# philres/ngmlr

Hardware: AMD Instinct MI355X
Metric: aligned Gbp/hour (PacBio 10kb synthetic, convex-gap SW hot path, host buffers in -> results out, CIGAR bit-exact) (higher is better)
Workload: dtype f32

## Files before the change

include/cvx_align.h:

```cpp
#ifndef CVX_ALIGN_H
#define CVX_ALIGN_H

#include <stdint.h>
#include <stddef.h>

#ifdef __cplusplus
extern "C" {
#endif

#define CVX_ABI_VERSION 9

enum {
	CVX_OK = 0,
	CVX_ERR_NO_DEVICE = -1,
	CVX_ERR_PARAMS = -2,
	CVX_ERR_ARG = -3,
	CVX_ERR_OOM = -4,
	CVX_ERR_HIP = -5,
	CVX_ERR_CAPACITY = -6
};

enum {
	CVX_TILE_OK = 0,
	CVX_TILE_INVALID_ROW0 = 1,
	CVX_TILE_INVALID_EDGE = 2,
	CVX_TILE_INVALID_LENGTH = 3,
	CVX_TILE_TOO_LARGE = 4,
	CVX_TILE_EMPTY = 5,
	CVX_TILE_UNSUPPORTED = -1
};

enum { CVX_OP_I = 1, CVX_OP_D = 2, CVX_OP_EQ = 7, CVX_OP_X = 8 };

typedef struct {
	float match;
	float mismatch;
	float gap_open;
	float gap_extend;
	float gap_extend_min;
	float gap_decay;
} cvx_params;

enum { CVX_CORRIDOR_ROWS = 0, CVX_CORRIDOR_AFFINE = 1, CVX_CORRIDOR_CONST = 2 };

typedef struct {
	const char *ref;
	const char *qry;
	const int32_t *row_offset;
	const int32_t *row_length;
	int32_t ref_len;
	int32_t qry_len;
	int32_t row_stride_bytes;
	int32_t corridor_kind;
	float corridor_k;
	float corridor_d;
	float corridor_right;
	int32_t corridor_offset;
	int32_t corridor_width;
	int32_t reserved;
} cvx_tile;

int cvx_corridor_fit(const int32_t *row_offset, const int32_t *row_length, int32_t row_stride_bytes, int32_t n_rows,
		int32_t ref_len, int32_t qry_len, cvx_tile *form);
int cvx_corridor_fit_batch(int32_t n_tiles, cvx_tile *tiles, int32_t n_threads, int32_t *n_fitted);

typedef struct {
	float score;
	int32_t status;
	int32_t best_ref_index;
	int32_t best_read_index;
	int32_t ref_position;
	int32_t qstart;
	int32_t qend;
	int32_t n_ops;
	uint64_t ops_begin;
	uint64_t cells;
} cvx_result;

typedef struct cvx_context *cvx_handle;
typedef struct cvx_batch_s *cvx_batch;
typedef struct cvx_batch_s *cvx_job;

typedef struct {
	float plan_ms;
	float fill_ms;
	float backtrack_ms;
	float total_ms;
	uint64_t cells;
	uint64_t active_cells;
	uint64_t dir_bytes;
	int32_t n_fill_launches;
	int32_t n_tiles_fast;
	int32_t n_tiles_redone;
	int32_t n_tiles_chained;
	uint64_t chain_task_ticks, chain_poll_ticks;
} cvx_timing;

enum { CVX_LAUNCH_WHOLE = 0, CVX_LAUNCH_GANG = 1, CVX_LAUNCH_CHAINED = 2, CVX_LAUNCH_CATCH_ALL = 3 };
typedef struct {
	int32_t slots_per_lane;
	int32_t waves;
	int32_t wrap16;
	int32_t n_tiles;
	float ms;
	int32_t kind;
	uint64_t cells;
	uint64_t active_cells;
	uint64_t alg_bytes;
	uint64_t read_bases;
} cvx_launch_info;

const char *cvx_last_error(void);
int cvx_abi_version(void);
int cvx_device_count(void);
const char *cvx_build_id(void);
const char *cvx_source_id(const char *family);
int cvx_device_synchronize(int device_id);

int cvx_create(int device_id, const cvx_params *params, uint64_t max_matrix_mb, cvx_handle *out);
enum { CVX_CREATE_SERVICE = 1, CVX_CREATE_SCALAR_TWIN = 2 };
typedef struct {
	int32_t hw_queues_env, hw_queues_set_by_library;
	int32_t blocking_sync, blocking_sync_why;
	int32_t service_streams;
	int32_t runtime_up_at_load;
	int32_t reserved[2];
} cvx_regime;
int cvx_runtime_regime(int device_id, cvx_regime *out);
int cvx_create_ex(int device_id, const cvx_params *params, uint64_t max_matrix_mb, uint32_t flags, cvx_handle *out);
void cvx_destroy(cvx_handle h);

int cvx_align_batch(cvx_handle h, int32_t n_tiles, const cvx_tile *tiles, cvx_result *results,
		uint32_t *ops_arena, uint64_t ops_capacity, uint64_t *ops_used);

int cvx_batch_upload(cvx_handle h, int32_t n_tiles, const cvx_tile *tiles, cvx_batch *out);
int cvx_batch_run(cvx_handle h, cvx_batch b);
int cvx_batch_timing(cvx_batch b, cvx_timing *t);
int cvx_batch_ops_total(cvx_batch b, uint64_t *n_ops);
int cvx_batch_launch_info(cvx_batch b, int32_t i, cvx_launch_info *info);
int cvx_batch_download(cvx_handle h, cvx_batch b, cvx_result *results,
		uint32_t *ops_arena, uint64_t ops_capacity, uint64_t *ops_used);
void cvx_batch_free(cvx_handle h, cvx_batch b);

int cvx_submit(cvx_handle h, int32_t n_tiles, const cvx_tile *tiles, cvx_job *out);
int cvx_wait(cvx_handle h, cvx_job job, const cvx_result **results, const uint32_t **ops, uint64_t *n_ops);
int cvx_job_poll(cvx_handle h, cvx_job job, int32_t *done);
int cvx_job_timing(cvx_job job, cvx_timing *t);
int cvx_job_launch_info(cvx_job job, int32_t i, cvx_launch_info *info);
void cvx_job_release(cvx_handle h, cvx_job job);

int cvx_host_alloc(uint64_t bytes, void **out);
void cvx_host_free(void *p);

int cvx_corridor_rows(cvx_handle h, const cvx_tile *tile, int32_t *offset, int32_t *length);

int cvx_pack_probe(int32_t n_tiles, const cvx_tile *tiles, int32_t iters, int32_t assume_page_locked, double *ms_per_iter, uint64_t *bytes_touched);

typedef struct cvx_genome_s *cvx_genome;
uint64_t cvx_genome_encoded_bytes(int32_t n, const uint64_t *lengths);
int cvx_genome_encode(int32_t n, const char *const *seqs, const uint64_t *lengths, uint8_t *bin_ref,
		uint64_t *n_nibbles, uint64_t *start_table, int32_t *n_starts);
int cvx_genome_upload(cvx_handle h, const uint8_t *bin_ref, uint64_t n_nibbles, const uint64_t *start_table,
		int32_t n_starts, cvx_genome *out);
void cvx_genome_free(cvx_handle h, cvx_genome g);
int cvx_genome_decode(cvx_handle h, cvx_genome g, int32_t n, const uint64_t *position, const int32_t *length,
		const uint64_t *out_offset, char *out);
int cvx_submit_windows(cvx_handle h, cvx_genome g, int32_t n_tiles, const cvx_tile *tiles,
		const uint64_t *ref_position, cvx_job *out);
int cvx_job_window_refs(cvx_handle h, cvx_job job, const char **refs);

typedef struct cvx_index_s *cvx_index;
typedef struct {
	uint64_t location;
	float score;
	int32_t reverse;
} cvx_candidate;
int cvx_index_upload(cvx_handle h, int32_t kmer_len, const void *ref_table_index, const uint32_t *ref_table, uint32_t n_locations,
		uint64_t unit_offset, cvx_index *out);
void cvx_index_free(cvx_handle h, cvx_index ix);
int cvx_index_build(const uint8_t *bin_ref, uint64_t n_nibbles, const uint64_t *start_table, const uint64_t *seq_lengths, int32_t n_seqs,
		int32_t kmer_len, int32_t ref_skip, int32_t bin_shift, void *ref_table_index, uint32_t *ref_table, uint64_t ref_table_capacity,
		uint64_t *n_locations);
#define CVX_INDEX_KEEP_RESIDENT 1u
int cvx_index_build_device(int32_t device_id, const uint8_t *bin_ref, uint64_t n_nibbles, const uint64_t *start_table, const uint64_t *seq_lengths,
		int32_t n_seqs, int32_t kmer_len, int32_t ref_skip, int32_t bin_shift, void *ref_table_index, uint32_t *ref_table,
		uint64_t ref_table_capacity, uint64_t *n_locations, uint32_t flags);
int cvx_search_batch(cvx_handle h, cvx_index ix, int32_t n, const char *const *seqs, const int32_t *lens,
		float sensitivity, float min_kmer_hits, int32_t bin_shift,
		int32_t *n_candidates, uint64_t *cand_begin, cvx_candidate *cands, uint64_t cand_capacity, uint64_t *cand_used);
int cvx_search_batch_ex(cvx_handle h, cvx_index ix, int32_t n, const char *const *seqs, const int32_t *lens,
		float sensitivity, float min_kmer_hits, int32_t bin_shift, int32_t first_bits,
		int32_t *n_candidates, uint64_t *cand_begin, cvx_candidate *cands, uint64_t cand_capacity, uint64_t *cand_used,
		float *max_hit, int32_t *kmer_misses);
int cvx_search_batch_arena(cvx_handle h, cvx_index ix, int32_t n, const uint8_t *arena, const uint64_t *offsets,
		float sensitivity, float min_kmer_hits, int32_t bin_shift, int32_t first_bits,
		int32_t *n_candidates, uint64_t *cand_begin, cvx_candidate *cands, uint64_t cand_capacity, uint64_t *cand_used,
		float *max_hit, int32_t *kmer_misses);

int cvx_search_last_attempts(cvx_handle h, int32_t n, int32_t *attempts);

int cvx_score_batch(cvx_handle h, int32_t n, const char *const *refs, const char *const *qrys, float *scores);
int cvx_score_kernel_ms(cvx_handle h, float *ms);
enum { CVX_STAGE_SCORE = 0, CVX_STAGE_DECODE = 1, CVX_STAGE_SEARCH = 2,
	CVX_STAGE_SCORE_WINDOWS = 3  };
int cvx_stage_kernel_ms(cvx_handle h, int32_t stage, float *ms);

typedef struct cvx_score_job_s *cvx_score_job;
int cvx_score_submit(cvx_handle h, int32_t n, const char *const *refs, const char *const *qrys, cvx_score_job *job);
int cvx_score_poll(cvx_score_job job);
int cvx_score_wait(cvx_score_job job, float *scores);

typedef struct { uint64_t position; int32_t buffer_len; int32_t read; int32_t reverse; } cvx_score_window;
int cvx_score_windows_submit(cvx_handle h, cvx_genome g, int32_t n_reads, const uint8_t *arena, const uint64_t *offsets,
		int32_t n, const cvx_score_window *pairs, cvx_score_job *job);
int cvx_score_windows(cvx_handle h, cvx_genome g, int32_t n_reads, const uint8_t *arena, const uint64_t *offsets,
		int32_t n, const cvx_score_window *pairs, float *scores, int32_t *status );
int cvx_stage_windows(cvx_handle h, cvx_genome g, int32_t n_reads, const uint8_t *arena, const uint64_t *offsets,
		int32_t n, const cvx_score_window *pairs, uint8_t *out, uint64_t cap, uint64_t *ref_off, uint64_t *qry_off,
		int32_t *status, uint64_t *used);
int cvx_stage_windows_host(const uint8_t *bin_ref, uint64_t n_nibbles, const uint64_t *start_table, int32_t n_starts,
		int32_t n_reads, const uint8_t *arena, const uint64_t *offsets, int32_t n, const cvx_score_window *pairs,
		uint8_t *out, uint64_t cap, uint64_t *ref_off, uint64_t *qry_off, int32_t *status, uint64_t *used);
int cvx_genome_concat_len(uint64_t n_nibbles, const uint64_t *start_table, int32_t n_starts, uint64_t *concat_len);

typedef struct {
	int32_t ret;
	float score;
	int32_t position_offset;
	int32_t qstart, qend;
	int32_t nm;
	float identity;
	int32_t alignment_length;
	int32_t cigar_op_count;
	int32_t sv_type;
	int32_t first_ref, first_read, last_ref, last_read;
	int32_t nm_count;
	int32_t cigar_len, md_len;
} cvx_alignment_text;

enum { CVX_FORMAT_SCALAR_TWIN = 1 };
enum { CVX_NOT_WRITTEN = -1 };
int cvx_format_alignment_ex(const cvx_result *r, const uint32_t *ops_arena,
		const char *ref, int32_t ref_len, int32_t qry_len,
		int32_t ext_qstart, int32_t ext_qend,
		char *cigar, int32_t cigar_cap, char *md, int32_t md_cap,
		int32_t *nm_triples, int32_t nm_cap, uint32_t flags, cvx_alignment_text *out);
int cvx_format_alignment(const cvx_result *r, const uint32_t *ops_arena,
		const char *ref, int32_t ref_len, int32_t qry_len,
		int32_t ext_qstart, int32_t ext_qend,
		char *cigar, int32_t cigar_cap, char *md, int32_t md_cap,
		int32_t *nm_triples, int32_t nm_cap, cvx_alignment_text *out);

typedef struct {
	char *cigar;
	char *md;
	int32_t *nm_triples;
	int32_t cigar_cap, md_cap, nm_cap;
	int32_t ext_qstart, ext_qend;
} cvx_text_buffers;

int cvx_format_batch(int32_t n, const cvx_result *results, const uint32_t *ops_arena,
		const cvx_tile *tiles, const cvx_text_buffers *bufs, cvx_alignment_text *out,
		int32_t n_threads);
int cvx_format_batch_ex(int32_t n, const cvx_result *results, const uint32_t *ops_arena,
		const cvx_tile *tiles, const cvx_text_buffers *bufs, cvx_alignment_text *out,
		int32_t n_threads, uint32_t flags);

int cvx_job_text(cvx_handle h, cvx_job job, const int32_t *ext_qstart, const int32_t *ext_qend,
		cvx_alignment_text *out, uint64_t *text_off, const char **text, uint64_t *text_bytes);

int cvx_job_nm_profile(cvx_handle h, cvx_job job, int32_t first, int32_t count, uint64_t *entry_off,
		int32_t *triples, uint64_t cap_entries, double *kernel_ms);
int cvx_job_nm_profile_resident(cvx_handle h, cvx_job job, int32_t first, int32_t count, uint64_t *entry_off,
		const int32_t **triples, double *kernel_ms);
int cvx_job_text_all(cvx_handle h, cvx_job job, const int32_t *ext_qstart, const int32_t *ext_qend,
		cvx_alignment_text *out, uint64_t *text_off, const char **text, uint64_t *text_bytes,
		uint64_t *nm_entry_off, const int32_t **triples);
int cvx_job_nm_sizes(cvx_handle h, cvx_job job, int32_t first, int32_t count, uint64_t *entry_off);

int cvx_nm_profile_ops(cvx_handle h, int32_t n, const cvx_result *results, const uint32_t *ops_arena, uint64_t ops_total,
		uint64_t *entry_off, int32_t *triples, uint64_t cap_entries);

typedef struct {
	int32_t ref_start, ref_stop;
	int32_t read_start, read_stop;
} cvx_nm_region;
typedef struct {
	int32_t open, distance;
	cvx_nm_region r;
} cvx_nm_open;

int cvx_job_nm_regions(cvx_handle h, cvx_job job, int32_t first, int32_t count, uint64_t *region_off,
		const cvx_nm_region **regions, cvx_nm_open *open, double *kernel_ms);
int cvx_nm_regions_ops(cvx_handle h, int32_t n, const cvx_result *results, const uint32_t *ops_arena, uint64_t ops_total,
		uint64_t *region_off, cvx_nm_region *regions, uint64_t cap_regions, cvx_nm_open *open);
int cvx_nm_regions_host(const int32_t *triples, int64_t n_entries, int64_t scan_len, cvx_nm_region *regions, int64_t cap,
		int64_t *n_regions, cvx_nm_open *open);

typedef struct {
	const char *ref_name;
	int32_t ref_name_len;
	uint32_t location;
	int32_t reverse;
	const char *cigar;
	int32_t mq, nm;
} cvx_sam_other;

typedef struct {
	const char *read_name;
	const char *seq;
	char *qual;
	int32_t read_length;
	int32_t flags;
	int32_t primary;
	int32_t reverse;
	const char *ref_name;
	int32_t ref_name_len;
	uint32_t location;
	int32_t mq;
	const char *cigar;
	const char *md;
	int32_t cigar_op_count;
	const char *mate_ref_name;
	int32_t mate_location;
	int32_t template_length;
	float score;
	int32_t nm;
	float identity;
	int32_t qstart, qend;
	int32_t sv_type;
	int32_t n_others;
	const cvx_sam_other *others;
	const char *rg_id;
	int32_t hard_clip;
	int32_t bam_cigar_fix;
	int32_t skip;
} cvx_sam_record;

typedef struct {
	const char *read_name, *seq;
	const char *qual;
	int32_t read_length, flags;
	const char *ref_name;
	int32_t ref_name_len;
	int32_t location;
	char mate_ref;
	int32_t mate_location, template_length;
	const char *rg_id;
} cvx_sam_unmapped;

int cvx_sam_record_text(cvx_sam_record *r, char *out, uint64_t cap, uint64_t *len);
int cvx_sam_unmapped_text(const cvx_sam_unmapped *r, char *out, uint64_t cap, uint64_t *len);

int cvx_sam_batch(int32_t n, cvx_sam_record *recs, char *out, uint64_t cap, uint64_t *offsets);

#ifdef __cplusplus
}
#endif
#endif
```

ngmlr_amd/capi.py:

```python
from __future__ import annotations

import ctypes as C
import os

HERE = os.path.dirname(os.path.abspath(__file__))
LIB_PATH = os.environ.get("CVX_LIB") or os.path.join(HERE, "libcvxalign.so")

CVX_OK = 0
CREATE_SERVICE, CREATE_SCALAR_TWIN = 1, 2
FORMAT_SCALAR_TWIN = 1
NOT_WRITTEN = -1
STAGE_SCORE, STAGE_DECODE, STAGE_SEARCH, STAGE_SCORE_WINDOWS = 0, 1, 2, 3
ERR_NAMES = {0: "CVX_OK", -1: "CVX_ERR_NO_DEVICE", -2: "CVX_ERR_PARAMS", -3: "CVX_ERR_ARG",
             -4: "CVX_ERR_OOM", -5: "CVX_ERR_HIP", -6: "CVX_ERR_CAPACITY"}
TILE_STATUS = {0: "ok", 1: "invalid-row0", 2: "invalid-edge", 3: "invalid-length", 4: "too-large",
               5: "empty", -1: "unsupported"}

EXPORTS = ("cvx_last_error", "cvx_abi_version", "cvx_source_id", "cvx_device_count", "cvx_device_synchronize", "cvx_create", "cvx_destroy",
           "cvx_align_batch", "cvx_batch_upload", "cvx_batch_run", "cvx_batch_timing",
           "cvx_batch_ops_total", "cvx_batch_launch_info", "cvx_batch_download", "cvx_batch_free",
           "cvx_submit", "cvx_wait", "cvx_job_timing", "cvx_job_launch_info", "cvx_job_release",
           "cvx_format_alignment", "cvx_format_batch", "cvx_score_batch",
           "cvx_genome_encoded_bytes", "cvx_genome_encode", "cvx_genome_upload", "cvx_genome_free",
           "cvx_genome_decode", "cvx_submit_windows", "cvx_job_text",
           "cvx_host_alloc", "cvx_host_free", "cvx_corridor_rows", "cvx_pack_probe", "cvx_build_id", "cvx_job_poll", "cvx_score_kernel_ms",
           "cvx_index_upload", "cvx_index_free", "cvx_search_batch", "cvx_search_batch_ex", "cvx_job_nm_profile", "cvx_job_nm_profile_resident", "cvx_job_text_all", "cvx_job_window_refs", "cvx_job_nm_sizes", "cvx_nm_profile_ops",
           "cvx_job_nm_regions", "cvx_nm_regions_ops", "cvx_nm_regions_host",
           "cvx_sam_record_text", "cvx_sam_unmapped_text", "cvx_sam_batch", "cvx_stage_kernel_ms", "cvx_search_last_attempts", "cvx_index_build", "cvx_index_build_device",
           "cvx_corridor_fit", "cvx_corridor_fit_batch", "cvx_create_ex", "cvx_runtime_regime", "cvx_search_batch_arena",
           "cvx_score_submit", "cvx_score_poll", "cvx_score_wait", "cvx_format_alignment_ex", "cvx_format_batch_ex",
           "cvx_score_windows_submit", "cvx_score_windows", "cvx_stage_windows", "cvx_stage_windows_host", "cvx_genome_concat_len")


class CvxParams(C.Structure):
    _fields_ = [("match", C.c_float), ("mismatch", C.c_float), ("gap_open", C.c_float),
                ("gap_extend", C.c_float), ("gap_extend_min", C.c_float), ("gap_decay", C.c_float)]


class CvxTile(C.Structure):
    _fields_ = [("ref", C.c_char_p), ("qry", C.c_char_p), ("row_offset", C.c_void_p),
                ("row_length", C.c_void_p), ("ref_len", C.c_int32), ("qry_len", C.c_int32),
                ("row_stride_bytes", C.c_int32), ("corridor_kind", C.c_int32),
                ("corridor_k", C.c_float), ("corridor_d", C.c_float), ("corridor_right", C.c_float),
                ("corridor_offset", C.c_int32), ("corridor_width", C.c_int32), ("reserved", C.c_int32)]


class CvxRegime(C.Structure):
    _fields_ = [("hw_queues_env", C.c_int32), ("hw_queues_set_by_library", C.c_int32), ("blocking_sync", C.c_int32),
                ("blocking_sync_why", C.c_int32), ("service_streams", C.c_int32), ("runtime_up_at_load", C.c_int32), ("reserved", C.c_int32 * 2)]


CORRIDOR_ROWS, CORRIDOR_AFFINE, CORRIDOR_CONST = 0, 1, 2
assert C.sizeof(CvxTile) == 72


class CvxResult(C.Structure):
    _fields_ = [("score", C.c_float), ("status", C.c_int32), ("best_ref_index", C.c_int32),
                ("best_read_index", C.c_int32), ("ref_position", C.c_int32), ("qstart", C.c_int32),
                ("qend", C.c_int32), ("n_ops", C.c_int32), ("ops_begin", C.c_uint64),
                ("cells", C.c_uint64)]


class CvxTiming(C.Structure):
    _fields_ = [("plan_ms", C.c_float), ("fill_ms", C.c_float), ("backtrack_ms", C.c_float),
                ("total_ms", C.c_float), ("cells", C.c_uint64), ("active_cells", C.c_uint64),
                ("dir_bytes", C.c_uint64), ("n_fill_launches", C.c_int32), ("n_tiles_fast", C.c_int32),
                ("n_tiles_redone", C.c_int32), ("n_tiles_chained", C.c_int32),
                ("chain_task_ticks", C.c_uint64), ("chain_poll_ticks", C.c_uint64)]


class CvxLaunchInfo(C.Structure):
    _fields_ = [("slots_per_lane", C.c_int32), ("waves", C.c_int32), ("wrap16", C.c_int32),
                ("n_tiles", C.c_int32), ("ms", C.c_float), ("kind", C.c_int32), ("cells", C.c_uint64),
                ("active_cells", C.c_uint64), ("alg_bytes", C.c_uint64), ("read_bases", C.c_uint64)]


class CvxAlignmentText(C.Structure):
    _fields_ = [("ret", C.c_int32), ("score", C.c_float), ("position_offset", C.c_int32),
                ("qstart", C.c_int32), ("qend", C.c_int32), ("nm", C.c_int32), ("identity", C.c_float),
                ("alignment_length", C.c_int32), ("cigar_op_count", C.c_int32), ("sv_type", C.c_int32),
                ("first_ref", C.c_int32), ("first_read", C.c_int32), ("last_ref", C.c_int32),
                ("last_read", C.c_int32), ("nm_count", C.c_int32), ("cigar_len", C.c_int32),
                ("md_len", C.c_int32)]


class CvxNmRegion(C.Structure):
    _fields_ = [("ref_start", C.c_int32), ("ref_stop", C.c_int32), ("read_start", C.c_int32), ("read_stop", C.c_int32)]


class CvxNmOpen(C.Structure):
    _fields_ = [("open", C.c_int32), ("distance", C.c_int32), ("r", CvxNmRegion)]


class CvxSamOther(C.Structure):
    _fields_ = [("ref_name", C.c_char_p), ("ref_name_len", C.c_int32), ("location", C.c_uint32), ("reverse", C.c_int32),
                ("cigar", C.c_char_p), ("mq", C.c_int32), ("nm", C.c_int32)]


class CvxSamRecord(C.Structure):
    _fields_ = [("read_name", C.c_char_p), ("seq", C.c_char_p), ("qual", C.c_void_p), ("read_length", C.c_int32),
                ("flags", C.c_int32), ("primary", C.c_int32), ("reverse", C.c_int32), ("ref_name", C.c_char_p),
                ("ref_name_len", C.c_int32), ("location", C.c_uint32), ("mq", C.c_int32), ("cigar", C.c_char_p),
                ("md", C.c_char_p), ("cigar_op_count", C.c_int32), ("mate_ref_name", C.c_char_p),
                ("mate_location", C.c_int32), ("template_length", C.c_int32), ("score", C.c_float), ("nm", C.c_int32),
                ("identity", C.c_float), ("qstart", C.c_int32), ("qend", C.c_int32), ("sv_type", C.c_int32),
                ("n_others", C.c_int32), ("others", C.POINTER(CvxSamOther)), ("rg_id", C.c_char_p),
                ("hard_clip", C.c_int32), ("bam_cigar_fix", C.c_int32), ("skip", C.c_int32)]


class CvxSamUnmapped(C.Structure):
    _fields_ = [("read_name", C.c_char_p), ("seq", C.c_char_p), ("qual", C.c_char_p), ("read_length", C.c_int32),
                ("flags", C.c_int32), ("ref_name", C.c_char_p), ("ref_name_len", C.c_int32), ("location", C.c_int32),
                ("mate_ref", C.c_char), ("mate_location", C.c_int32), ("template_length", C.c_int32), ("rg_id", C.c_char_p)]


class CvxTextBuffers(C.Structure):
    _fields_ = [("cigar", C.c_void_p), ("md", C.c_void_p), ("nm_triples", C.c_void_p),
                ("cigar_cap", C.c_int32), ("md_cap", C.c_int32), ("nm_cap", C.c_int32),
                ("ext_qstart", C.c_int32), ("ext_qend", C.c_int32)]


class CvxScoreWindow(C.Structure):
    _fields_ = [("position", C.c_uint64), ("buffer_len", C.c_int32), ("read", C.c_int32), ("reverse", C.c_int32)]


assert C.sizeof(CvxScoreWindow) == 24


class CvxError(RuntimeError):
    def __init__(self, code: int, msg: str):
        super().__init__("%s: %s" % (ERR_NAMES.get(code, str(code)), msg))
        self.code = code


_libs = {}


def load(path: str = None) -> C.CDLL:
    path = path or LIB_PATH
    if path in _libs:
        return _libs[path]
    if not os.path.exists(path):
        raise FileNotFoundError(
            "%s not built: run `python -c 'import __graft_entry__ as g; g.build()'` "
            "(the HIP path has no fallback)" % path)
    lib = C.CDLL(path)
    lib.cvx_last_error.restype = C.c_char_p
    lib.cvx_abi_version.restype = C.c_int
    lib.cvx_build_id.restype = C.c_char_p
    lib.cvx_source_id.restype = C.c_char_p
    lib.cvx_source_id.argtypes = [C.c_char_p]
    lib.cvx_device_count.restype = C.c_int
    lib.cvx_device_synchronize.argtypes = [C.c_int]
    lib.cvx_create.argtypes = [C.c_int, C.POINTER(CvxParams), C.c_uint64, C.POINTER(C.c_void_p)]
    lib.cvx_destroy.argtypes = [C.c_void_p]
    lib.cvx_destroy.restype = None
    lib.cvx_align_batch.argtypes = [C.c_void_p, C.c_int32, C.POINTER(CvxTile), C.POINTER(CvxResult),
                                    C.c_void_p, C.c_uint64, C.POINTER(C.c_uint64)]
    lib.cvx_batch_upload.argtypes = [C.c_void_p, C.c_int32, C.POINTER(CvxTile), C.POINTER(C.c_void_p)]
    lib.cvx_batch_run.argtypes = [C.c_void_p, C.c_void_p]
    lib.cvx_batch_timing.argtypes = [C.c_void_p, C.POINTER(CvxTiming)]
    lib.cvx_batch_launch_info.argtypes = [C.c_void_p, C.c_int32, C.POINTER(CvxLaunchInfo)]
    lib.cvx_batch_ops_total.argtypes = [C.c_void_p, C.POINTER(C.c_uint64)]
    lib.cvx_batch_download.argtypes = [C.c_void_p, C.c_void_p, C.POINTER(CvxResult), C.c_void_p,
                                       C.c_uint64, C.POINTER(C.c_uint64)]
    lib.cvx_batch_free.argtypes = [C.c_void_p, C.c_void_p]
    lib.cvx_batch_free.restype = None
    lib.cvx_submit.argtypes = [C.c_void_p, C.c_int32, C.POINTER(CvxTile), C.POINTER(C.c_void_p)]
    lib.cvx_wait.argtypes = [C.c_void_p, C.c_void_p, C.POINTER(C.POINTER(CvxResult)), C.POINTER(C.POINTER(C.c_uint32)),
                             C.POINTER(C.c_uint64)]
    lib.cvx_job_poll.argtypes = [C.c_void_p, C.c_void_p, C.POINTER(C.c_int32)]
    lib.cvx_job_timing.argtypes = [C.c_void_p, C.POINTER(CvxTiming)]
    lib.cvx_job_launch_info.argtypes = [C.c_void_p, C.c_int32, C.POINTER(CvxLaunchInfo)]
    lib.cvx_job_release.argtypes = [C.c_void_p, C.c_void_p]
    lib.cvx_job_release.restype = None
    lib.cvx_format_batch.argtypes = [C.c_int32, C.POINTER(CvxResult), C.c_void_p, C.POINTER(CvxTile),
                                     C.POINTER(CvxTextBuffers), C.POINTER(CvxAlignmentText), C.c_int32]
    lib.cvx_genome_encoded_bytes.restype = C.c_uint64
    lib.cvx_genome_encoded_bytes.argtypes = [C.c_int32, C.c_void_p]
    lib.cvx_genome_encode.argtypes = [C.c_int32, C.POINTER(C.c_char_p), C.c_void_p, C.c_void_p, C.POINTER(C.c_uint64),
                                      C.c_void_p, C.POINTER(C.c_int32)]
    lib.cvx_genome_upload.argtypes = [C.c_void_p, C.c_void_p, C.c_uint64, C.c_void_p, C.c_int32, C.POINTER(C.c_void_p)]
    lib.cvx_genome_free.argtypes = [C.c_void_p, C.c_void_p]
    lib.cvx_genome_free.restype = None
    lib.cvx_genome_decode.argtypes = [C.c_void_p, C.c_void_p, C.c_int32, C.c_void_p, C.c_void_p, C.c_void_p, C.c_void_p]
    lib.cvx_submit_windows.argtypes = [C.c_void_p, C.c_void_p, C.c_int32, C.POINTER(CvxTile), C.c_void_p, C.POINTER(C.c_void_p)]
    lib.cvx_job_text.argtypes = [C.c_void_p, C.c_void_p, C.c_void_p, C.c_void_p, C.POINTER(CvxAlignmentText), C.c_void_p,
                                 C.POINTER(C.c_char_p), C.POINTER(C.c_uint64)]
    lib.cvx_job_nm_profile.argtypes = [C.c_void_p, C.c_void_p, C.c_int32, C.c_int32, C.c_void_p, C.c_void_p, C.c_uint64, C.POINTER(C.c_double)]
    lib.cvx_job_nm_sizes.argtypes = [C.c_void_p, C.c_void_p, C.c_int32, C.c_int32, C.c_void_p]
    lib.cvx_job_nm_profile_resident.argtypes = [C.c_void_p, C.c_void_p, C.c_int32, C.c_int32, C.c_void_p, C.POINTER(C.c_void_p), C.POINTER(C.c_double)]
    lib.cvx_job_window_refs.argtypes = [C.c_void_p, C.c_void_p, C.c_void_p]
    lib.cvx_job_text_all.argtypes = [C.c_void_p, C.c_void_p, C.c_void_p, C.c_void_p, C.POINTER(CvxAlignmentText), C.c_void_p,
                                     C.POINTER(C.c_char_p), C.POINTER(C.c_uint64), C.c_void_p, C.POINTER(C.c_void_p)]
    lib.cvx_nm_profile_ops.argtypes = [C.c_void_p, C.c_int32, C.c_void_p, C.c_void_p, C.c_uint64, C.c_void_p, C.c_void_p, C.c_uint64]
    lib.cvx_job_nm_regions.argtypes = [C.c_void_p, C.c_void_p, C.c_int32, C.c_int32, C.c_void_p, C.POINTER(C.c_void_p), C.c_void_p, C.POINTER(C.c_double)]
    lib.cvx_nm_regions_ops.argtypes = [C.c_void_p, C.c_int32, C.c_void_p, C.c_void_p, C.c_uint64, C.c_void_p, C.c_void_p, C.c_uint64, C.c_void_p]
    lib.cvx_nm_regions_host.argtypes = [C.c_void_p, C.c_int64, C.c_int64, C.c_void_p, C.c_int64, C.POINTER(C.c_int64), C.c_void_p]
    lib.cvx_sam_record_text.argtypes = [C.POINTER(CvxSamRecord), C.c_void_p, C.c_uint64, C.POINTER(C.c_uint64)]
    lib.cvx_sam_unmapped_text.argtypes = [C.POINTER(CvxSamUnmapped), C.c_void_p, C.c_uint64, C.POINTER(C.c_uint64)]
    lib.cvx_sam_batch.argtypes = [C.c_int32, C.POINTER(CvxSamRecord), C.c_void_p, C.c_uint64, C.c_void_p]
    lib.cvx_host_alloc.argtypes = [C.c_uint64, C.POINTER(C.c_void_p)]
    lib.cvx_host_free.argtypes = [C.c_void_p]
    lib.cvx_host_free.restype = None
    lib.cvx_corridor_rows.argtypes = [C.c_void_p, C.POINTER(CvxTile), C.c_void_p, C.c_void_p]
    lib.cvx_pack_probe.argtypes = [C.c_int32, C.c_void_p, C.c_int32, C.c_int32, C.POINTER(C.c_double), C.POINTER(C.c_uint64)]
    lib.cvx_index_upload.argtypes = [C.c_void_p, C.c_int32, C.c_void_p, C.c_void_p, C.c_uint32, C.c_uint64, C.POINTER(C.c_void_p)]
    lib.cvx_index_free.argtypes = [C.c_void_p, C.c_void_p]
    lib.cvx_index_free.restype = None
    lib.cvx_search_batch.argtypes = [C.c_void_p, C.c_void_p, C.c_int32, C.POINTER(C.c_char_p), C.c_void_p, C.c_float, C.c_float, C.c_int32,
                                     C.c_void_p, C.c_void_p, C.c_void_p, C.c_uint64, C.POINTER(C.c_uint64)]
    lib.cvx_search_batch_ex.argtypes = [C.c_void_p, C.c_void_p, C.c_int32, C.POINTER(C.c_char_p), C.c_void_p, C.c_float, C.c_float, C.c_int32, C.c_int32,
                                        C.c_void_p, C.c_void_p, C.c_void_p, C.c_uint64, C.POINTER(C.c_uint64), C.c_void_p, C.c_void_p]
    lib.cvx_search_batch_arena.argtypes = [C.c_void_p, C.c_void_p, C.c_int32, C.c_void_p, C.c_void_p, C.c_float, C.c_float, C.c_int32, C.c_int32,
                                           C.c_void_p, C.c_void_p, C.c_void_p, C.c_uint64, C.POINTER(C.c_uint64), C.c_void_p, C.c_void_p]
    lib.cvx_score_kernel_ms.argtypes = [C.c_void_p, C.POINTER(C.c_float)]
    lib.cvx_stage_kernel_ms.argtypes = [C.c_void_p, C.c_int32, C.POINTER(C.c_float)]
    lib.cvx_search_last_attempts.argtypes = [C.c_void_p, C.c_int32, C.c_void_p]
    lib.cvx_index_build_device.argtypes = [C.c_int32, C.c_void_p, C.c_uint64, C.c_void_p, C.c_void_p, C.c_int32, C.c_int32, C.c_int32, C.c_int32,
                                           C.c_void_p, C.c_void_p, C.c_uint64, C.POINTER(C.c_uint64), C.c_uint32]
    lib.cvx_index_build.argtypes = [C.c_void_p, C.c_uint64, C.c_void_p, C.c_void_p, C.c_int32, C.c_int32, C.c_int32, C.c_int32,
                                    C.c_void_p, C.c_void_p, C.c_uint64, C.POINTER(C.c_uint64)]
    lib.cvx_runtime_regime.argtypes = [C.c_int, C.POINTER(CvxRegime)]
    lib.cvx_create_ex.argtypes = [C.c_int, C.POINTER(CvxParams), C.c_uint64, C.c_uint32, C.POINTER(C.c_void_p)]
    lib.cvx_corridor_fit_batch.argtypes = [C.c_int32, C.c_void_p, C.c_int32, C.POINTER(C.c_int32)]
    lib.cvx_corridor_fit.argtypes = [C.c_void_p, C.c_void_p, C.c_int32, C.c_int32, C.c_int32, C.c_int32, C.POINTER(CvxTile)]
    lib.cvx_score_batch.argtypes = [C.c_void_p, C.c_int32, C.POINTER(C.c_char_p), C.POINTER(C.c_char_p), C.c_void_p]
    lib.cvx_score_submit.argtypes = [C.c_void_p, C.c_int32, C.POINTER(C.c_char_p), C.POINTER(C.c_char_p), C.POINTER(C.c_void_p)]
    lib.cvx_score_poll.argtypes = [C.c_void_p]
    lib.cvx_score_wait.argtypes = [C.c_void_p, C.c_void_p]
    win_in = [C.c_int32, C.c_void_p, C.c_void_p, C.c_int32, C.c_void_p]
    win_out = [C.c_void_p, C.c_uint64, C.c_void_p, C.c_void_p, C.c_void_p, C.POINTER(C.c_uint64)]
    lib.cvx_score_windows_submit.argtypes = [C.c_void_p, C.c_void_p] + win_in + [C.POINTER(C.c_void_p)]
    lib.cvx_score_windows.argtypes = [C.c_void_p, C.c_void_p] + win_in + [C.c_void_p, C.c_void_p]
    lib.cvx_stage_windows.argtypes = [C.c_void_p, C.c_void_p] + win_in + win_out
    lib.cvx_stage_windows_host.argtypes = [C.c_void_p, C.c_uint64, C.c_void_p, C.c_int32] + win_in + win_out
    lib.cvx_genome_concat_len.argtypes = [C.c_uint64, C.c_void_p, C.c_int32, C.POINTER(C.c_uint64)]
    lib.cvx_format_alignment.argtypes = [C.POINTER(CvxResult), C.c_void_p, C.c_char_p, C.c_int32,
                                         C.c_int32, C.c_int32, C.c_int32, C.c_char_p, C.c_int32,
                                         C.c_char_p, C.c_int32, C.c_void_p, C.c_int32,
                                         C.POINTER(CvxAlignmentText)]
    lib.cvx_format_alignment_ex.argtypes = [C.POINTER(CvxResult), C.c_void_p, C.c_char_p, C.c_int32,
                                            C.c_int32, C.c_int32, C.c_int32, C.c_char_p, C.c_int32,
                                            C.c_char_p, C.c_int32, C.c_void_p, C.c_int32, C.c_uint32,
                                            C.POINTER(CvxAlignmentText)]
    lib.cvx_format_batch_ex.argtypes = [C.c_int32, C.POINTER(CvxResult), C.c_void_p, C.POINTER(CvxTile),
                                        C.POINTER(CvxTextBuffers), C.POINTER(CvxAlignmentText), C.c_int32, C.c_uint32]
    _libs[path] = lib
    return lib


def check(rc: int) -> None:
    if rc != CVX_OK:
        raise CvxError(rc, load().cvx_last_error().decode(errors="replace"))


def corridor_fit(row_offset, row_length, ref_len, qry_len, stride_bytes=4):
    import numpy as np
    lib = load()
    off = np.ascontiguousarray(row_offset, dtype=np.int32) if stride_bytes == 4 else row_offset
    ln = np.ascontiguousarray(row_length, dtype=np.int32) if stride_bytes == 4 else row_length
    n = len(off) if stride_bytes == 4 else qry_len
    form = CvxTile()
    rc = lib.cvx_corridor_fit(off.ctypes.data, ln.ctypes.data, stride_bytes, n, ref_len, qry_len, C.byref(form))
    if rc != CVX_OK:
        raise RuntimeError("cvx_corridor_fit: %s" % ERR_NAMES.get(rc, rc))
    return (form.corridor_kind, form.corridor_k, form.corridor_d, form.corridor_right, form.corridor_offset, form.corridor_width)
```

ngmlr_amd/csrc/cvx_fill_ring.inc:

```
template <int M, bool WRAP, int MODE, bool TAB = false, int G = 1>
__global__ void __launch_bounds__(64 * G) CVX_FILL_OCC(M, TAB && G == 1)
CVX_FILL_KERNEL(const FillArgs a) {
	constexpr bool TWIN = CVX_FILL_TWIN;
	constexpr int N = 64 * M * G;
	constexpr int NW = 64 * M;
	constexpr bool EXACT = (MODE != kFillTwoPhase);
	constexpr bool CHAIN = (MODE == kFillChain);
	constexpr bool GANG = G > 1;
	static_assert(!GANG || (!WRAP && !CHAIN), "gangs serve whole tiles with float runs");
	static_assert(!TAB || (!WRAP && MODE == kFillTwoPhase), "the penalty table serves the two-phase float-score instantiation only");
	typedef typename RunT<WRAP || TAB>::type run_t;
	const int tid = threadIdx.x;
	const int lane = GANG ? (tid & 63) : tid;
	const int wv = GANG ? __builtin_amdgcn_readfirstlane(tid >> 6) : 0;
	const float go = a.sp.go;
	const float gext = a.sp.ge, gem = a.sp.gem, decay = a.sp.decay;
	float vmat = a.sp.mat, vmis = a.sp.mis;
	asm volatile("" : "+v"(vmat), "+v"(vmis));

	__shared__ int4 s_rec[CHAIN ? 1 : M * G][64];
	__shared__ int s_besty[M][64 * G];
	__shared__ u64 s_gx[GANG ? G : 1][GANG ? kGangDepth : 1];
	__shared__ float s_gred[GANG ? G : 1][4];
	__shared__ int s_gfail[GANG ? G : 1];
	__shared__ BoundaryVal s_bnd[CHAIN ? kChainChunk : 1];
	__shared__ float s_pen[TAB ? kPenEntries : 1];

	int t;
	int task_id = 0, y0 = 0;
	u64 chain_t0 = 0ull, chain_polled = 0ull;
	ChainTask ct;
	if (CHAIN) {
		int tk = 0;
		if (lane == 0) tk = atomicAdd(a.chain_ticket, 1);
		task_id = __builtin_amdgcn_readfirstlane(tk);
		if (task_id >= a.list_n) return;
		ct = a.tasks[task_id];
		t = ct.tile;
		y0 = ct.y0;
		if (a.chain_prio) __builtin_amdgcn_s_setprio(3);
		chain_t0 = __builtin_amdgcn_s_memtime();
	} else {
		t = a.list[blockIdx.x];
		if (!GANG && a.chain_prio) { if (a.chain_prio >= 2) __builtin_amdgcn_s_setprio(2); else __builtin_amdgcn_s_setprio(1); }
#if CVX_FILL_PRIO
		if (blockIdx.x < (unsigned) (a.list_n >> 4)) __builtin_amdgcn_s_setprio(2);
#endif
		if (GANG && a.chain_prio) __builtin_amdgcn_s_setprio(2);
		if (MODE == kFillExact) {
			if (a.tout[t].pad != kPadRedo) return;
			if (tid == 0) atomicAdd(a.redo_count, 1);
		}
	}
	TileIn ti = a.tin[t];
	ti.ref_off = in_sgpr(ti.ref_off); ti.qry_off = in_sgpr(ti.qry_off); ti.W = in_sgpr(ti.W); ti.H = in_sgpr(ti.H);
	ti.row_off = in_sgpr((u64) ti.row_off);
	TileRun tr = a.trun[t];
	tr.dir_off = in_sgpr((u64) tr.dir_off); tr.r0 = in_sgpr(tr.r0); tr.nsteps = in_sgpr(tr.nsteps);
	RowView rv = row_view(a.rsrc[t], a.rows, ti.row_off, y0);
	rv.rows = in_sgpr(rv.rows); rv.fmt = in_sgpr(rv.fmt); rv.width = in_sgpr(rv.width);
	rv.k = in_sgpr(rv.k); rv.d = in_sgpr(rv.d); rv.right = in_sgpr(rv.right);
	const uint8_t *seq = a.seq;
	const int H = CHAIN ? ct.rows : ti.H, W = ti.W;
	const unsigned qry_off = ti.qry_off + (unsigned) y0;
	const int r0 = CHAIN ? ct.r0 : tr.r0;
	const int nsteps = CHAIN ? ct.nsteps : tr.nsteps;
	uint32_t *dirs = in_sgpr(a.dirs + (CHAIN ? ct.dir_off : tr.dir_off));
	float S[M];
	float Hc[M];
	float V[M];
	float dg[M];
	run_t drun[M];
	run_t irun[M];
	int cnt[M];
	int len[M];
	int qch[M];
	unsigned xa[M];
	unsigned cwn[M];
	float penp[M];
	constexpr bool LAZY = TAB && (CVX_FILL_TAB_LAZY != 0);
	float best[M];
	int best_r[M];
	float lbest = 0.0f;
	unsigned accA[M], accB[M];
	u64 mD[M];
	u64 mI[M];

	const unsigned ref_base = ti.ref_off - (unsigned) y0;
	auto make_rec = [&](const int yy) {
		int4 rec;
		rec.w = (int) (ref_base - (unsigned) yy);
		if (yy < H) {
			const RowDesc2 ol = row_at(rv, yy);
			const long long Ws = (long long) W;
			long long lo = ol.x > 0 ? ol.x : 0;
			long long hi = (long long) ol.x + (long long) ol.y;
			if (hi > Ws) hi = Ws;
			if (hi < lo) hi = lo;
			rec.x = yy + y0 + (int) lo;
			rec.y = (int) (hi - lo);
			rec.z = seq[qry_off + (unsigned) yy];
		} else {
			rec.x = yy + y0 + (1 << 30);
			rec.y = 0;
			rec.z = 0;
		}
		return rec;
	};
	auto take_row = [&](const int j, const int4 rec, const int rnext, const bool fetch_now) {
		cnt[j] = rnext - rec.x;
		len[j] = rec.y;
		qch[j] = rec.z;
		xa[j] = (unsigned) rec.w + (unsigned) rnext + 4u;
		if (fetch_now || cnt[j] > -4) cwn[j] = *reinterpret_cast<const unsigned *>(seq + (xa[j] - 4u));
	};
	constexpr int kStage = 16 * M;
	auto stage_rows = [&](const int Y, const int sY) {
		if (lane < kStage) {
			const int4 rec = make_rec(Y + lane);
			const int sl = sY + lane;
			s_rec[CHAIN ? 0 : wv * M + sl % M][sl / M] = rec;
		}
		__builtin_amdgcn_fence(__ATOMIC_ACQ_REL, "workgroup");
	};

	if (TAB) {
		for (int i = lane; i < kPenEntries; i += 64) s_pen[i] = fminf(gem, gext + (float) i * decay);
		__builtin_amdgcn_fence(__ATOMIC_ACQ_REL, "workgroup");
	}
#pragma unroll
	for (int j = 0; j < M; ++j) {
		s_besty[j][tid] = 0;
		S[j] = 0.0f; Hc[j] = go; V[j] = go; dg[j] = 0.0f;
		drun[j] = 0; irun[j] = 0;
		best[j] = 0.0f; best_r[j] = 0;
		penp[j] = gem;
		accA[j] = accB[j] = 0u;
		mD[j] = 0; mI[j] = 0;
		cwn[j] = 0u;
		take_row(j, make_rec(tid * M + j), r0, true);
	}
	int stage_next = N + wv * NW, stage_slot = 0;
	auto stage_advance = [&]() {
		stage_next += kStage;
		stage_slot += kStage;
		if (stage_slot >= NW) { stage_slot = 0; stage_next += N - NW; }
	};
	if (!CHAIN) {
		for (int c = 0; c < NW / kStage - 1; ++c) { stage_rows(stage_next, stage_slot); stage_advance(); }
	}

	int gang_failed = 0;
	if (GANG) {
		if (lane < kGangDepth) s_gx[wv][lane] = ~0ull;
		__syncthreads();
	}
	const int gang_pred = GANG ? (wv + G - 1) % G : 0;

	const int ngroups = (nsteps + 3) >> 2;
	int late = ngroups >> a.late_shift;
	if (late < a.late_min_groups) late = a.late_min_groups;
	const int gswitch = (EXACT || late >= ngroups) ? 0 : ngroups - late;
	int r = r0;

	const int out_slot = CHAIN ? (ct.rows - 1) : 0;
	const int out_lane = out_slot / M, out_j = out_slot % M;
	u64 *bnd_out = CHAIN ? reinterpret_cast<u64 *>(a.bnd + ct.bnd_out_off) : nullptr;
	u64 *bnd_in = CHAIN ? reinterpret_cast<u64 *>(a.bnd + ct.bnd_in_off) : nullptr;
	const unsigned epoch = a.bnd_epoch;
	int chain_failed = 0;
	BoundaryVal bcur;
	bcur.V = go; bcur.S = 0.0f; bcur.run = 0u; bcur.is_ins = 0u;
	u64 bpre = 0ull;

	auto group = [&](auto track_tag, const int g) {
		constexpr bool TRACK = decltype(track_tag)::value;
		if (CHAIN && (g & (kChainChunk / 4 - 1)) == 0) {
			const int x = (r - y0) + lane;
			const int idx = x - ct.bnd_lo;
			const bool mine = ct.prev >= 0 && lane < kChainChunk && idx >= 0 && idx < ct.bnd_len;
			u64 q = bpre;
			bool ok = !mine || (unsigned) (q >> 49) == epoch;
			int spins = 0;
			const bool must_poll = !chain_failed && ballot(!ok) != 0ull;
			const u64 poll_t0 = must_poll ? __builtin_amdgcn_s_memtime() : 0ull;
			while (!chain_failed && ballot(!ok) != 0ull) {
				if (!ok) {
					q = __hip_atomic_load(bnd_in + idx, __ATOMIC_RELAXED, __HIP_MEMORY_SCOPE_AGENT);
					ok = (unsigned) (q >> 49) == epoch;
				}
				if (ballot(!ok) == 0ull) break;
				if (++spins > (1 << 21)) { chain_failed = 1; break; }
				if (spins < 8) __builtin_amdgcn_s_sleep(2);
				else if (spins < 64) __builtin_amdgcn_s_sleep(32);
				else __builtin_amdgcn_s_sleep(127);
			}
			if (must_poll) chain_polled += __builtin_amdgcn_s_memtime() - poll_t0;
			BoundaryVal br;
			br.V = go; br.S = 0.0f; br.run = 0u; br.is_ins = 0u;
			if (mine && ok) {
				const unsigned meta = (unsigned) (q >> 32);
				const float sc = __uint_as_float((unsigned) q);
				const unsigned run16 = meta & 0xffffu;
				const bool ins = (meta >> 16) & 1u;
				const float runf = WRAP ? (float) (int) (short) run16 : (float) run16 - 1.0f;
				br.S = sc;
				br.run = WRAP ? (unsigned) (int) (short) run16 : __float_as_uint((float) run16);
				br.is_ins = ins ? 1u : 0u;
				br.V = ins ? gap_extend_value(sc, runf, gem, gext, decay) : sc + go;
			}
			if (lane < kChainChunk) s_bnd[lane] = br;
			__builtin_amdgcn_fence(__ATOMIC_ACQ_REL, "workgroup");
			bcur = s_bnd[0];
			const int idxn = idx + kChainChunk;
			bpre = 0ull;
			if (ct.prev >= 0 && lane < kChainChunk && idxn >= 0 && idxn < ct.bnd_len)
				bpre = __hip_atomic_load(bnd_in + idxn, __ATOMIC_RELAXED, __HIP_MEMORY_SCOPE_AGENT);
		}
		unsigned cw[M];
		const float misx = TWIN ? a.sp.misx : 0.0f;
#pragma unroll
		for (int j = 0; j < M; ++j) {
			cw[j] = cwn[j];
			cwn[j] = *reinterpret_cast<const unsigned *>(seq + xa[j]);
			xa[j] += 4u;
		}
		if (g != 0 && (g & 7) == 0) {
			uint32_t *d = dirs + (size_t) ((g >> 3) - 1) * (N * 2);
			const unsigned dl = (unsigned) tid * (M * 2);
#pragma unroll
			for (int j = 0; j < M; ++j) { d[dl + 2 * j] = accA[j]; d[dl + 2 * j + 1] = accB[j]; }
		}

#pragma unroll
		for (int i = 0; i < 4; ++i) {
			float p_E[M], p_O[M];
			auto offers = [&](const int j) {
				p_E[j] = fmaxf(S[j] + penp[j], S[j] * -0x1p100f);
				p_O[j] = S[j] + go;
			};
			if (LAZY) offers(M - 1);
			float uV0 = LAZY ? rot1_f(lanes(mI[M - 1]) ? p_E[M - 1] : p_O[M - 1]) : rot1_f(V[M - 1]);
			float uS0 = rot1_f(S[M - 1]);
			run_t uI0;
			if (WRAP || TAB) uI0 = (run_t) rot1_i((int) irun[M - 1]);
			else uI0 = (run_t) rot1_f((float) irun[M - 1]);
			u64 mIu0 = rot1_m(mI[M - 1]);
			u64 gq = 0ull;
			if (GANG && r != r0) gq = __hip_atomic_load(&s_gx[gang_pred][(r - r0 - 1) & (kGangDepth - 1)], __ATOMIC_RELAXED, __HIP_MEMORY_SCOPE_WORKGROUP);
			auto gang_take = [&]() {
				float sc = 0.0f, vv = go;
				unsigned run16 = 0u, ins = 0u;
				if (r != r0) {
					const unsigned want_tag = (unsigned) (r - r0 - 1) & 0x7fffu;
					int spins = 0;
					while (!gang_failed && (((unsigned) __builtin_amdgcn_readfirstlane((int) (gq >> 32))) >> 17) != want_tag) {
						if (++spins > (1 << 22)) { gang_failed = 1; break; }
#if CVX_GANG_SLEEP > 0
						__builtin_amdgcn_s_sleep(CVX_GANG_SLEEP);
#endif
						gq = __hip_atomic_load(&s_gx[gang_pred][(r - r0 - 1) & (kGangDepth - 1)], __ATOMIC_RELAXED, __HIP_MEMORY_SCOPE_WORKGROUP);
					}
					const unsigned meta = (unsigned) __builtin_amdgcn_readfirstlane((int) (gq >> 32));
					sc = __uint_as_float((unsigned) __builtin_amdgcn_readfirstlane((int) gq));
					run16 = meta & 0xffffu;
					ins = (meta >> 16) & 1u;
					vv = ins ? gap_extend_value(sc, (float) run16 - 1.0f, gem, gext, decay) : sc + go;
				}
				if (lane == 0) {
					uV0 = vv;
					uS0 = sc;
					uI0 = TAB ? (run_t) (int) (run16 << 2) : (run_t) (float) run16;
				}
				mIu0 = (mIu0 & ~1ull) | (u64) ins;
			};
			auto gang_give = [&]() {
				const unsigned run16 = TAB ? (((unsigned) (int) irun[M - 1]) >> 2) & 0xffffu : ((unsigned) (int) (float) irun[M - 1]) & 0xffffu;
				const unsigned meta = run16 | (unsigned) (((mI[M - 1] >> 63) & 1ull) << 16) | (((unsigned) (r - r0) & 0x7fffu) << 17);
				if (lane == 63)
					__hip_atomic_store(&s_gx[wv][(r - r0) & (kGangDepth - 1)], ((u64) meta << 32) | (u64) __float_as_uint(S[M - 1]), __ATOMIC_RELAXED, __HIP_MEMORY_SCOPE_WORKGROUP);
			};
			if (CHAIN) {
				const BoundaryVal br = bcur;
				bcur = s_bnd[((r - r0) + 1) & (kChainChunk - 1)];
				if (lane == 0) {
					uV0 = br.V;
					uS0 = br.S;
					uI0 = WRAP ? (run_t) (int) br.run : (run_t) __uint_as_float(br.run);
				}
				const int bit = __builtin_amdgcn_readfirstlane((int) br.is_ins);
				mIu0 = (mIu0 & ~1ull) | (u64) (bit & 1);
			}

			float p_lc[M], p_dc[M], p_uc[M], p_mx[M];
			u64 p_eL[M], p_eU[M], p_eG[M], p_act[M], p_isDl[M], p_isIu[M];
			u64 p_nD[M], p_nI[M], p_gap[M], p_cread[M];
			auto phase1 = [&](const int j, const float misx_) {
				float uV = (j > 0) ? V[j > 0 ? j - 1 : 0] : uV0;
				const run_t uI = (j > 0) ? irun[j > 0 ? j - 1 : 0] : uI0;
				const u64 mIu = (j > 0) ? mI[j > 0 ? j - 1 : 0] : mIu0;
				float lcv = Hc[j];
				if (LAZY) {
					if (j > 0) {
						offers(j > 0 ? j - 1 : 0);
						uV = lanes(mIu) ? p_E[j > 0 ? j - 1 : 0] : p_O[j > 0 ? j - 1 : 0];
					}
					lcv = lanes(mD[j]) ? p_E[j] : p_O[j];
				}
				const int refc = (int) ((cw[j] >> (8 * i)) & 0xffu);
				const bool eq = (refc == qch[j]);
				float mv = vmis;
				if (TWIN) mv = lanes(ballot(refc == 'x')) ? misx_ : vmis;
				const float diag_cell = dg[j] + (eq ? vmat : mv);
				float lc = lcv, dc = diag_cell, uc = uV;
				const float mx = fmaxf(fmaxf(fmaxf(lc, dc), uc), 0.0f);
				p_lc[j] = lc; p_dc[j] = dc; p_uc[j] = uc; p_mx[j] = mx;
				p_eL[j] = ballot(mx == lc);
				p_eU[j] = ballot(mx == uc);
				p_eG[j] = ballot(mx == dc);
				p_act[j] = ballot((unsigned) cnt[j] < (unsigned) len[j]);
				p_isDl[j] = WRAP ? ballot(drun[j] > 0) : mD[j];
				p_isIu[j] = WRAP ? ballot(uI > 0) : mIu;
			};
			auto phase2 = [&](const int j) {
				const u64 eL = p_eL[j], eU = p_eU[j], eG = p_eG[j], act = p_act[j], isDl = p_isDl[j], isIu = p_isIu[j];
				const u64 c2 = isIu & eU;
				const u64 nD = eL & (isDl | ~(c2 | eG)) & act;
				const u64 nI = ~nD & eU & (isIu | ~eG) & act;
				p_nD[j] = nD; p_nI[j] = nI;
				p_gap[j] = nD | nI;
				p_cread[j] = nI | (eG & ~nD);
			};
			auto phase3 = [&](const int j) {
				const float uS = (j > 0) ? S[j > 0 ? j - 1 : 0] : uS0;
				const run_t uI = (j > 0) ? irun[j > 0 ? j - 1 : 0] : uI0;
				const u64 nD = p_nD[j], nI = p_nI[j], isDl = p_isDl[j], isIu = p_isIu[j];
				const float mx = p_mx[j];
				const float sc = lanes(p_act[j]) ? mx : 0.0f;
				run_t nd, ni;
				float runf = 0.0f;
				float E;
				if (TAB) {
					const u64 extD = nD & isDl, extI = nI & isIu;
					const int t1 = lanes(extI) ? (int) uI : 4;
					const int ra = lanes(extD) ? (int) drun[j] : t1;
					nd = (run_t) (ra + 4);
					ni = nd;
					const float pen = *reinterpret_cast<const float *>(reinterpret_cast<const char *>(s_pen) + ra);
					if (LAZY) penp[j] = pen;
					E = fmaxf(sc + pen, sc * -0x1p100f);
				} else if (WRAP) {
					nd = lanes(nD) ? (lanes(isDl) ? (run_t) (short) ((int) drun[j] + 1) : (run_t) 1) : (run_t) 0;
					ni = lanes(nI) ? (lanes(isIu) ? (run_t) (short) ((int) uI + 1) : (run_t) 1) : (run_t) 0;
					runf = (float) (lanes(nD) ? nd : ni);
				} else {
					const u64 extD = nD & isDl, extI = nI & isIu;
					const float t1 = lanes(extI) ? (float) uI : 1.0f;
					runf = lanes(extD) ? (float) drun[j] : t1;
					nd = (run_t) (runf + 1.0f);
					ni = nd;
				}
				if (!TAB) E = gap_extend_value(sc, runf, gem, gext, decay);
				const float O = sc + go;

				dg[j] = uS;
				S[j] = sc;
				drun[j] = nd;
				irun[j] = ni;
				if (!LAZY) {
					V[j] = lanes(nI) ? E : O;
					Hc[j] = lanes(nD) ? E : O;
				}
				if (TRACK) {
					const u64 better = ballot(sc > best[j]);
					best[j] = lanes(better) ? mx : best[j];
					best_r[j] = lanes(better) ? r : best_r[j];
				} else if (i >= 2) {
					lbest = fmaxf(lbest, sc);
				}
				mD[j] = nD;
				mI[j] = nI;
				cnt[j] += 1;
				accA[j] = shl1_in(accA[j], p_gap[j]);
				accB[j] = shl1_in(accB[j], p_cread[j]);
			};
#if CVX_FILL_SCHED == 1
#pragma unroll
			for (int j = M - 1; j >= 0; --j) phase1(j, misx);
			__builtin_amdgcn_sched_barrier(0);
#pragma unroll
			for (int j = M - 1; j >= 0; --j) phase2(j);
			__builtin_amdgcn_sched_barrier(0);
#elif CVX_FILL_SCHED == 2
#pragma unroll
			for (int q = M; q >= -1; --q) {
				if (q < M && q >= 0) phase1(q, misx);
				if (q + 1 < M && q + 1 >= 0) phase2(q + 1);
				__builtin_amdgcn_sched_barrier(0);
			}
#endif
#pragma unroll
			for (int j = M - 1; j >= 0; --j) {
#if CVX_FILL_SCHED == 0 || CVX_FILL_SCHED == 3
				if (GANG && j == 0) gang_take();
				phase1(j, misx); phase2(j);
#endif
				phase3(j);
				if (GANG && j == M - 1) gang_give();
#if CVX_FILL_SCHED == 3
				__builtin_amdgcn_sched_barrier(0);
#endif
				if (CHAIN && j == out_j && ct.has_next) {
					if (lane == out_lane && (unsigned) (cnt[j] - 1) < (unsigned) len[j]) {
						const unsigned run16 = WRAP ? ((unsigned) (int) irun[j] & 0xffffu) : ((unsigned) (int) (float) irun[j] & 0xffffu);
						const unsigned meta = run16 | (unsigned) (((mI[j] >> out_lane) & 1ull) << 16) | (epoch << 17);
						__hip_atomic_store(bnd_out + (cnt[j] - 1), ((u64) meta << 32) | (u64) __float_as_uint(S[j]), __ATOMIC_RELAXED, __HIP_MEMORY_SCOPE_AGENT);
					}
				}
			}
			r += 1;
		}
		const bool stage_now = !CHAIN && (ballot(cnt[0] > len[0]) & 0x0001000100010001ull) != 0ull;
#pragma unroll
		for (int j = 0; j < M; ++j) {
			if (!CHAIN && cnt[j] > len[j]) {
				if (TRACK) {
					const int yy = (int) (ref_base - (xa[j] - (unsigned) r - 4u));
					if (best_r[j] >= r - cnt[j]) s_besty[j][tid] = yy;
				}
				take_row(j, s_rec[CHAIN ? 0 : wv * M + j][lane], r, false);
			}
		}
		if (TAB) {
#pragma unroll
			for (int j = 0; j < M; ++j) { const int c = min((int) drun[j], 4 * kPenClamp); drun[j] = (run_t) c; irun[j] = (run_t) c; }
		}
		if (stage_now) {
			stage_rows(stage_next, stage_slot);
			stage_advance();
		}
	};

	for (int g = 0; g < gswitch; ++g) group(BoolTag<false>(), g);
	for (int g = gswitch; g < ngroups; ++g) group(BoolTag<true>(), g);

	if (ngroups > 0) {
		const int done = ((ngroups - 1) & 7) + 1;
		const int sh = 32 - 4 * done;
		uint32_t *d = dirs + ((size_t) ((ngroups - 1) >> 3) * N + (size_t) tid * M) * 2;
#pragma unroll
		for (int j = 0; j < M; ++j) { d[2 * j] = sh ? accA[j] << sh : accA[j]; d[2 * j + 1] = sh ? accB[j] << sh : accB[j]; }
	}

	float b = -1.0f;
	int by = 0x7fffffff, bx = 0x7fffffff;
#pragma unroll
	for (int j = 0; j < M; ++j) {
		int vy = s_besty[j][tid];
		const int ycur = (int) (ref_base - (xa[j] - (unsigned) r - 4u));
		if (ycur < H && best_r[j] >= r - cnt[j]) vy = ycur;
		const float v = best[j];
		const int vx = best_r[j] - vy;
		if (v > 0.0f) {
			if (v > b || (v == b && (vy < by || (vy == by && vx < bx)))) { b = v; by = vy; bx = vx; }
		}
	}
	float be = lbest;
#pragma unroll
	for (int off = 32; off >= 1; off >>= 1) {
		const float ob = __shfl_xor(b, off, 64);
		const int oy = __shfl_xor(by, off, 64);
		const int ox = __shfl_xor(bx, off, 64);
		if (ob > b || (ob == b && (oy < by || (oy == by && ox < bx)))) { b = ob; by = oy; bx = ox; }
		if (!EXACT) be = fmaxf(be, __shfl_xor(be, off, 64));
	}
	if (CHAIN) {
		if (lane == 0) {
			ChainOut co;
			co.score = b;
			co.best_y = (b > -1.0f) ? by + y0 : 0;
			co.best_x = (b > -1.0f) ? bx - y0 : 0;
			co.failed = chain_failed;
			a.chain_out[ct.blk] = co;
			unsigned long long *ticks = reinterpret_cast<unsigned long long *>(a.redo_count + kCtrChainTicks);
			atomicAdd(ticks, (unsigned long long) (__builtin_amdgcn_s_memtime() - chain_t0));
			if (chain_polled) atomicAdd(ticks + 1, (unsigned long long) chain_polled);
		}
		return;
	}
	if (GANG) {
		if (lane == 0) {
			s_gred[wv][0] = b; s_gred[wv][1] = __int_as_float(by); s_gred[wv][2] = __int_as_float(bx);
			s_gred[wv][3] = EXACT ? 0.0f : be;
			s_gfail[wv] = gang_failed;
		}
		__syncthreads();
		if (wv != 0) return;
#pragma unroll
		for (int w = 1; w < G; ++w) {
			const float ob = s_gred[w][0];
			const int oy = __float_as_int(s_gred[w][1]), ox = __float_as_int(s_gred[w][2]);
			if (ob > b || (ob == b && (oy < by || (oy == by && ox < bx)))) { b = ob; by = oy; bx = ox; }
			if (!EXACT) be = fmaxf(be, s_gred[w][3]);
		}
	}
	if (lane == 0) {
		TileOut o;
		o.score = b;
		o.status = 0;
		o.best_x = (b > -1.0f) ? bx : 0;
		o.best_y = (b > -1.0f) ? by : 0;
		o.ref_position = 0; o.qstart = 0; o.qend = 0; o.n_ops = 0; o.ops_first = 0;
		o.pad = (!EXACT && gswitch > 0 && !(b > be + 2.0f * a.sp.mat + 1.0f)) ? kPadRedo : 0;
		if (GANG) {
			bool failed = gang_failed != 0;
			for (int w = 1; w < G; ++w) failed = failed || s_gfail[w] != 0;
			if (failed) { o.status = -1; o.pad = 0; }
		}
		a.tout[t] = o;
	}
}
```

ngmlr_amd/csrc/cvx_kernels.hip:

```cpp
#include <hip/hip_runtime.h>
#include <stdint.h>

#include "cvx_types.h"
#include "cvx_launch.h"

namespace cvx {

#define CVX_DEV __device__ __forceinline__

CVX_DEV int rot1_i(int v) {
	return __builtin_amdgcn_update_dpp(0, v, 0x13C, 0xf, 0xf, true);
}
CVX_DEV float rot1_f(float v) {
	return __int_as_float(rot1_i(__float_as_int(v)));
}


CVX_DEV void row_span(const int2 ol, int W, int y, int &gs, int &ge) {
	long long lo = ol.x > 0 ? ol.x : 0;
	long long hi = (long long) ol.x + (long long) ol.y;
	if (hi > W) hi = W;
	if (hi < lo) hi = lo;
	gs = (int) (lo + y);
	ge = (int) (hi + y);
}

template <int TPT>
__global__ void __launch_bounds__(256)
plan_kernel(const int2 *rows, const RowSrc *rsrc, const TileIn *tin, TilePlan *plan, int n_tiles, unsigned long long max_matrix_mb) {
	constexpr int TPB = 256 / TPT;
	const int sub = threadIdx.x / TPT;
	const int ltid = threadIdx.x % TPT;
	const int t = blockIdx.x * TPB + sub;
	const bool live = t < n_tiles;
	const TileIn ti = tin[live ? t : 0];
	const RowView rv = row_view(rsrc[live ? t : 0], reinterpret_cast<const RowDesc2 *>(rows), ti.row_off);
	auto row = [&](const int y) { const RowDesc2 q = row_at(rv, y); return make_int2(q.x, q.y); };
	const int H = live ? ti.H : 0, W = ti.W;

	__shared__ unsigned long long s_cells[TPB], s_active[TPB];
	__shared__ int s_need[TPB], s_flags[TPB], s_maxlen[TPB], s_rend[TPB], s_r0[TPB];
	if (ltid == 0) { s_cells[sub] = 0; s_active[sub] = 0; s_need[sub] = 1; s_flags[sub] = 0; s_maxlen[sub] = 0; s_rend[sub] = -0x7fffffff; s_r0[sub] = 0x7fffffff; }
	__syncthreads();

	unsigned long long cells = 0, active = 0;
	int need = 1, flags = 0, maxlen = 0, rendmax = -0x7fffffff, r0min = 0x7fffffff;
	for (int y = ltid; y < H; y += TPT) {
		const int2 ol = row(y);
		int gs, ge;
		row_span(ol, W, y, gs, ge);
		cells += (unsigned long long) (long long) ol.y;
		active += (unsigned long long) (ge - gs);
		if (ol.y > maxlen) maxlen = ol.y;
		if (ge > rendmax) rendmax = ge;
		if (gs < r0min) r0min = gs;
		if (y > 0) {
			int pgs, pge;
			row_span(row(y - 1), W, y - 1, pgs, pge);
			if (gs <= pgs) flags |= kPlanIrregular;
			if (ge < pge) flags |= kPlanIrregular;
		}
		const int lim = ge + kSwitchMargin;
		auto starts_before = [&](int yy) {
			int mgs, mge;
			row_span(row(yy), W, yy, mgs, mge);
			return mgs < lim;
		};
		int lo = y + 1, hi = H;
		int g = y + 1 + ((lim - gs) >> 1);
		g = g < lo ? lo : g;
		if (g < hi) {
			if (starts_before(g)) {
				lo = g + 1;
				for (int step = 1; lo < hi; step <<= 1) {
					const int p = (lo + step - 1 < hi) ? lo + step - 1 : hi - 1;
					if (starts_before(p)) lo = p + 1; else { hi = p; break; }
				}
			} else {
				hi = g;
				for (int step = 1; lo < hi; step <<= 1) {
					const int p = (hi - step > lo) ? hi - step : lo;
					if (starts_before(p)) { lo = p + 1; break; } else hi = p;
				}
			}
		}
		while (lo < hi) {
			const int mid = (lo + hi) >> 1;
			if (starts_before(mid)) lo = mid + 1; else hi = mid;
		}
		const int n = lo - y + 1;
		if (n > need) need = n;
		if (H > 32767) {
			long long lo_y = ol.x > 0 ? ol.x : 0;
			long long hi_y = (long long) ol.x + (long long) ol.y;
			if (hi_y > W) hi_y = W;
			if (hi_y < lo_y) hi_y = lo_y;
			int a = y + 1, b = H;
			while (a < b) {
				const int mid = (a + b) >> 1;
				const int2 om = row(mid);
				const long long lo_m = om.x > 0 ? om.x : 0;
				if (lo_m < hi_y) a = mid + 1; else b = mid;
			}
			if (a - y > maxlen) maxlen = a - y;
		}
	}
	if (H > 0) {
		atomicAdd(&s_cells[sub], cells);
		atomicAdd(&s_active[sub], active);
		atomicMax(&s_need[sub], need);
		atomicOr(&s_flags[sub], flags);
		atomicMax(&s_maxlen[sub], maxlen);
		atomicMax(&s_rend[sub], rendmax);
		atomicMin(&s_r0[sub], r0min);
	}
	__syncthreads();

	if (ltid == 0 && live) {
		TilePlan p;
		p.cells = s_cells[sub];
		p.active = s_active[sub];
		p.need = s_need[sub];
		int f = s_flags[sub];
		int r0 = 0, rend = 0;
		if (H > 0) { r0 = s_r0[sub]; rend = s_rend[sub]; }
		if (H <= 0 || s_active[sub] == 0) f |= kPlanEmpty;
		const float mb = (float) s_cells[sub] / 1000.0f / 1000.0f;
		if (!((unsigned long long) mb < max_matrix_mb)) f |= kPlanTooLarge;
		if (s_maxlen[sub] > 32767 || (H > 32767 && (f & kPlanIrregular))) f |= kPlanWrap16;
		p.r0 = r0;
		p.rend = rend;
		p.flags = f;
		plan[t] = p;
	}
}


__global__ void __launch_bounds__(64)
expand_rows_kernel(const RowSrc *rsrc, const TileIn *tin, const uint8_t *delta, const int2 *rowsx, int2 *rows, int n_tiles, int closed_forms) {
	const int t = blockIdx.x;
	if (t >= n_tiles) return;
	const int lane = threadIdx.x;
	const RowSrc rs = rsrc[t];
	const TileIn ti = tin[t];
	const int H = ti.H;
	int2 *out = rows + ti.row_off;
	if (rs.fmt == kRowsExplicit) {
		const int2 *src = rowsx + rs.src_off;
		for (int y = lane; y < H; y += 64) out[y] = src[y];
		return;
	}
	if ((rs.fmt == kRowsAffine || rs.fmt == kRowsConst) && !closed_forms) return;
	if (rs.fmt == kRowsAffine) {
		for (int y = lane; y < H; y += 64) out[y] = make_int2(affine_row_offset(y, rs.d, rs.k, rs.right), rs.width);
		return;
	}
	if (rs.fmt == kRowsConst) {
		for (int y = lane; y < H; y += 64) out[y] = make_int2(rs.off0, rs.width);
		return;
	}
	const int8_t *d = reinterpret_cast<const int8_t *>(delta + rs.src_off);
	int carry = rs.off0;
	for (int y0 = 0; y0 < H; y0 += 64) {
		const int y = y0 + lane;
		int v = (y < H && y > 0) ? (int) d[y] : 0;
#pragma unroll
		for (int k = 1; k < 64; k <<= 1) {
			const int u = __shfl_up(v, k, 64);
			if (lane >= k) v += u;
		}
		if (y < H) out[y] = make_int2(carry + v, rs.width);
		carry += __builtin_amdgcn_readlane(v, 63);
	}
}


typedef unsigned long long u64;

CVX_DEV u64 ballot(bool p) { return __builtin_amdgcn_ballot_w64(p); }
CVX_DEV int in_sgpr(int v) { v = __builtin_amdgcn_readfirstlane(v); asm volatile("" : "+s"(v)); return v; }
CVX_DEV float in_sgpr(float v) { return __int_as_float(in_sgpr(__float_as_int(v))); }
CVX_DEV unsigned in_sgpr(unsigned v) { return (unsigned) in_sgpr((int) v); }
CVX_DEV u64 in_sgpr(u64 u) { return ((u64) in_sgpr((unsigned) (u >> 32)) << 32) | (u64) in_sgpr((unsigned) u); }
template <typename T> CVX_DEV T *in_sgpr(T *p) {
	const u64 u = (u64) p;
	const unsigned lo = (unsigned) in_sgpr((int) (unsigned) u), hi = (unsigned) in_sgpr((int) (unsigned) (u >> 32));
	return (T *) (((u64) hi << 32) | (u64) lo);
}
CVX_DEV bool lanes(u64 m) { return __builtin_amdgcn_inverse_ballot_w64(m); }
CVX_DEV u64 rot1_m(u64 m) { return (m << 1) | (m >> 63); }
#ifndef CVX_FILL_ADDC_SGPR
#define CVX_FILL_ADDC_SGPR 1
#endif
CVX_DEV unsigned shl1_in(unsigned acc, u64 m) {
#if CVX_FILL_ADDC_SGPR
	u64 carry_out;
	asm volatile("v_addc_co_u32_e64 %0, %1, %0, %0, %2" : "+v"(acc), "=s"(carry_out) : "s"(m));
#else
	asm volatile("v_addc_co_u32_e64 %0, vcc, %0, %0, %1" : "+v"(acc) : "s"(m) : "vcc");
#endif
	return acc;
}


CVX_DEV void valid_bounds(const int off, const int width, int &minC, int &maxC) {
	minC = (int) ((float) off + 0.1f * (float) width);
	maxC = (int) ((float) (minC + width) - 0.1f * (float) width);
}

CVX_DEV unsigned plane_code(const unsigned wx, const unsigned wy, const int bit) {
	const unsigned px = (wx >> bit) & 1u, py = (wy >> bit) & 1u;
	return px ? (py ? 1u : 2u) : (py ? 3u : 0u);
}

template <bool CHAINED>
CVX_DEV void backtrack_walk(const int lane, const int H, const int N, const int r0, const int ops_cap,
		const RowView &rows, const uint2 *dirs, const ChainBlk *blk, const uint8_t *ref, const uint8_t *qry, int *ops, TileOut &o) {
	const int best_x = __builtin_amdgcn_readfirstlane(o.best_x);
	const int best_y = __builtin_amdgcn_readfirstlane(o.best_y);
	if (best_y <= 0) { o.status = 1; return; }

	const int qend = (H - best_y) - 1;
	int idx = ops_cap - 1;
	int elem = 4;
	int elem_len = qend;
	int consumed = qend;
	int x = best_x, y = best_y;
	int s = y % N;
	int status = 0;
	unsigned want = 3u;

	auto emit = [&](int cur, int n) {
		if (n <= 0) return;
		if (cur == elem) {
			elem_len += n;
		} else {
			if (elem != 4) { if (lane == 0) ops[idx] = (elem_len << 4) | elem; idx -= 1; }
			elem = cur;
			elem_len = n;
		}
	};

	int budget = 2 * (best_x + best_y) + 8;
	for (;;) {
		if (--budget < 0) { status = 3; break; }
		const int dx = (want != 1u) ? 1 : 0, dy = (want != 2u) ? 1 : 0;
		const int cx = x - lane * dx, cy = y - lane * dy;
		const bool inside = (cx >= 0 && cy >= 0);
		const int lx = cx > 0 ? cx : 0, ly = cy > 0 ? cy : 0;
		int sl = s - lane * dy;
		if (sl < 0) sl += N;
		const int tt = cx + cy - r0;
		const int ttc = tt > 0 ? tt : 0;
		const RowDesc2 ol = row_at(rows, ly);
		uint2 w;
		if (CHAINED) {
			const int gb = ly / N;
			const ChainBlk cb = blk[gb];
			int wr = (ttc >> 5) - cb.tblk0;
			wr = wr < 0 ? 0 : (wr >= cb.nblk32 ? cb.nblk32 - 1 : wr);
			w = dirs[cb.dir_off + (size_t) wr * N + (size_t) (ly - gb * N)];
		} else {
			w = dirs[(size_t) (ttc >> 5) * N + sl];
		}
		const int rc = ref[lx], qc = qry[ly];
		const u64 eqm = ballot(rc == qc);
		const bool in_row = inside && tt >= 0 && cx >= ol.x && cx < ol.x + ol.y;
		unsigned code = plane_code(w.x, w.y, 31 - (ttc & 31));
		if (!in_row) code = 0u;
		int minC, maxC;
		valid_bounds(ol.x, ol.y, minC, maxC);

		const u64 run = ballot(code == want);
		const int L = (~run == 0ull) ? 64 : __builtin_ctzll(~run);
		const u64 low = (L == 64) ? ~0ull : ((1ull << L) - 1ull);
		const u64 vp = ballot(cx > minC && cx < maxC);
		if ((~vp & low) != 0ull) { status = 2; break; }

		if (want == 3u) {
			int pos = 0;
			while (pos < L) {
				const int isq = (int) ((eqm >> pos) & 1ull);
				const u64 m = (isq ? ~eqm : eqm) >> pos;
				int rl = (m == 0ull) ? 64 - pos : __builtin_ctzll(m);
				if (rl > L - pos) rl = L - pos;
				emit(isq ? 7 : 8, rl);
				pos += rl;
			}
			x -= L; y -= L; consumed += L;
		} else if (want == 1u) {
			emit(1, L);
			y -= L; consumed += L;
		} else {
			emit(2, L);
			x -= L;
		}
		if (want != 2u) { s -= L; if (s < 0) s += N; }
		if (L == 64) continue;
		const unsigned nxt = (unsigned) __builtin_amdgcn_readlane((int) code, L);
		if (nxt == 0u) break;
		if (want != 3u) { want = nxt; continue; }

		const int tp = x + y - r0;
		if (nxt == 2u) {
			const unsigned wx = (unsigned) __builtin_amdgcn_readlane((int) w.x, L);
			const unsigned wy = (unsigned) __builtin_amdgcn_readlane((int) w.y, L);
			const int row_lo = max(__builtin_amdgcn_readlane(ol.x, L), 0);
			const int b0 = 31 - (tp & 31);
			const unsigned dm = (wx & ~wy) >> b0;
			int Ld = (~dm == 0u) ? 32 : __builtin_ctz(~dm);
			const int in_word = 32 - b0;
			const int in_rowc = x - row_lo + 1;
			if (Ld > in_rowc) Ld = in_rowc;
			const int rminC = __builtin_amdgcn_readlane(minC, L), rmaxC = __builtin_amdgcn_readlane(maxC, L);
			if (!(x - (Ld - 1) > rminC && x < rmaxC)) { status = 2; break; }
			emit(2, Ld);
			x -= Ld;
			if (Ld == in_rowc) break;
			if (Ld == in_word) { want = 2u; continue; }
			const unsigned c2 = plane_code(wx, wy, b0 + Ld);
			if (c2 == 0u) break;
			want = c2;
		} else {
			const int k = lane - L;
			const int tn = tp - k;
			const bool have = (k >= 0) && (cy >= 0) && (tn >= 0) && ((tn >> 5) == (ttc >> 5));
			const bool col_in = (x >= ol.x) && (x < ol.x + ol.y);
			unsigned c2 = plane_code(w.x, w.y, 31 - (tn & 31));
			if (!col_in) c2 = 0u;
			const u64 im = ballot(have && c2 == 1u) >> L;
			const int Li = (~im == 0ull) ? 64 : __builtin_ctzll(~im);
			const u64 ilow = (Li == 64) ? ~0ull : ((1ull << Li) - 1ull);
			const u64 vpi = ballot(x > minC && x < maxC) >> L;
			if ((~vpi & ilow) != 0ull) { status = 2; break; }
			emit(1, Li);
			y -= Li; consumed += Li;
			s -= Li; if (s < 0) s += N;
			const int e = L + Li;
			want = 1u;
			if (e < 64 && ((ballot(have) >> e) & 1ull) != 0ull) {
				const unsigned c3 = (unsigned) __builtin_amdgcn_readlane((int) c2, e);
				if (c3 == 0u) break;
				want = c3;
			}
		}
	}
	if (status == 0) {
		if (elem != 4) { if (lane == 0) ops[idx] = (elem_len << 4) | elem; idx -= 1; }
		consumed += (y + 1);
		o.ref_position = x + 1;
		o.qstart = y + 1;
		o.qend = qend;
		o.ops_first = idx + 1;
		o.n_ops = ops_cap - 1 - idx;
		if (H != consumed) status = 3;
	}
	o.status = status;
}

CVX_DEV void first_cell(const RowView &rows, int H, int W, int lane, int *fy, int *fx) {
	*fy = -1;
	*fx = 0;
	for (int y0 = 0; y0 < H; y0 += 64) {
		const int yy = y0 + lane;
		bool has = false;
		int lo_i = 0;
		if (yy < H) {
			const RowDesc2 ol = row_at(rows, yy);
			long long lo = ol.x > 0 ? ol.x : 0;
			long long hi = (long long) ol.x + (long long) ol.y;
			if (hi > W) hi = W;
			has = hi > lo;
			lo_i = (int) lo;
		}
		const unsigned long long m = __builtin_amdgcn_ballot_w64(has);
		if (m != 0ull) {
			const int l = __builtin_ctzll(m);
			*fy = y0 + l;
			*fx = __builtin_amdgcn_readlane(lo_i, l);
			return;
		}
	}
}


template <bool WRAP> struct RunT { typedef float type; };
template <> struct RunT<true> { typedef int type; };
template <bool B> struct BoolTag { static constexpr bool value = B; };

#ifndef CVX_FILL_WAVES_PER_EU
#define CVX_FILL_WAVES_PER_EU 6
#endif
#ifndef CVX_FILL_WAVES_M4
#define CVX_FILL_WAVES_M4 1
#endif
#ifndef CVX_FILL_WAVES_TAB
#define CVX_FILL_WAVES_TAB 7
#endif
#define CVX_FILL_OCC(M, SEVEN) __attribute__((amdgpu_waves_per_eu( \
		(M) == 3 ? ((SEVEN) ? CVX_FILL_WAVES_TAB : CVX_FILL_WAVES_PER_EU) : ((M) == 4 ? CVX_FILL_WAVES_M4 : 1), \
		(M) == 3 ? ((SEVEN) ? CVX_FILL_WAVES_TAB : CVX_FILL_WAVES_PER_EU) : ((M) == 4 && CVX_FILL_WAVES_M4 > 1 ? CVX_FILL_WAVES_M4 : 8))))

#ifndef CVX_FILL_TAB_LAZY
#define CVX_FILL_TAB_LAZY 1
#endif

#ifndef CVX_GANG_SLEEP
#define CVX_GANG_SLEEP 1
#endif

#ifndef CVX_FILL_SCHED
#define CVX_FILL_SCHED 0
#endif

#ifndef CVX_FILL_PRIO
#define CVX_FILL_PRIO 1
#endif

CVX_DEV float gap_extend_value(const float sc, const float runf, const float gem, const float gext, const float decay) {
	const float pen = fminf(gem, gext + runf * decay);
	return fmaxf(sc + pen, sc * -0x1p100f);
}

enum FillMode { kFillTwoPhase = 0, kFillExact = 1, kFillChain = 2 };

#define CVX_FILL_KERNEL fill_ring_kernel
#define CVX_FILL_TWIN false
#include "cvx_fill_ring.inc"
#undef CVX_FILL_KERNEL
#undef CVX_FILL_TWIN
#define CVX_FILL_KERNEL fill_ring_twin_kernel
#define CVX_FILL_TWIN true
#include "cvx_fill_ring.inc"
#undef CVX_FILL_KERNEL
#undef CVX_FILL_TWIN

CVX_DEV int rec_load(const void *rec, const int n_dwords, const int lane) {
	return lane < n_dwords ? reinterpret_cast<const int *>(rec)[lane] : 0;
}
CVX_DEV int fld(const int w, const int k) { return __builtin_amdgcn_readlane(w, k); }
CVX_DEV unsigned long long fld64(const int w, const int k) {
	return ((unsigned long long) (unsigned) fld(w, k + 1) << 32) | (unsigned) fld(w, k);
}

CVX_DEV void walk_tile(const BacktrackArgs &a, const int t, const int lane) {
	static_assert(sizeof(TileRun) == 48 && sizeof(TileIn) == 32 && sizeof(TileOut) == 40, "record layout");
	const int wr = rec_load(a.trun + t, 12, lane);
	const int wo = rec_load(a.tout + t, 10, lane);
	if (fld(wr, 8) != 0) return;
	TileOut o;
	o.score = __int_as_float(fld(wo, 0));
	o.status = fld(wo, 1);
	o.best_x = fld(wo, 2); o.best_y = fld(wo, 3);
	o.ref_position = 0; o.qstart = 0; o.qend = 0; o.n_ops = 0; o.ops_first = 0;
	o.pad = fld(wo, 9);
	if (o.status != 0 || o.pad != 0) return;
	const int wi = rec_load(a.tin + t, 8, lane);
	const int H = fld(wi, 3), W = fld(wi, 2);
	const RowView rows = row_view(a.rsrc[t], a.rows, fld64(wi, 4));
	if (!(o.score > 0.0f)) {
		int fy, fx;
		first_cell(rows, H, W, lane, &fy, &fx);
		if (fy < 0) {
			o.score = -1.0f; o.status = 5; o.pad = 1;
			if (lane == 0) a.tout[t] = o;
			return;
		}
		o.score = 0.0f; o.best_x = fx; o.best_y = fy;
	}
	const int cb0 = fld(wr, 10);
	if (cb0 >= 0)
		backtrack_walk<true>(lane, H, fld(wr, 4), fld(wr, 6), fld(wr, 5), rows,
				reinterpret_cast<const uint2 *>(a.dirs), a.chain_blk + cb0,
				a.seq + (unsigned) fld(wi, 0), a.seq + (unsigned) fld(wi, 1),
				a.ops + fld64(wr, 2), o);
	else
		backtrack_walk<false>(lane, H, fld(wr, 4), fld(wr, 6), fld(wr, 5), rows,
				reinterpret_cast<const uint2 *>(a.dirs + fld64(wr, 0)), nullptr,
				a.seq + (unsigned) fld(wi, 0), a.seq + (unsigned) fld(wi, 1),
				a.ops + fld64(wr, 2), o);
	o.pad = 1;
	if (lane == 0) a.tout[t] = o;
}


template <int G>
struct Group {
	int gl;
	int base;
	CVX_DEV unsigned ballot(bool p) const {
		const u64 b = __builtin_amdgcn_ballot_w64(p);
		return (unsigned) (b >> base) & (G == 32 ? 0xffffffffu : ((1u << (G & 31)) - 1u));
	}
	CVX_DEV int bcast(int v, int l) const { return __shfl(v, base + l, 64); }
};

template <int G>
CVX_DEV void backtrack_walk_grp(const Group<G> g, const bool has_tile, const bool chained, const int H, const int N, const int r0, const int ops_cap,
		const RowView &rows, const uint2 *dirs, const ChainBlk *blk, const uint8_t *ref, const uint8_t *qry, int *ops, TileOut &o) {
	const int gl = g.gl;
	const int best_x = o.best_x, best_y = o.best_y;
	bool act = has_tile;
	if (has_tile && best_y <= 0) { o.status = 1; act = false; }
	const bool walked = act;

	const int qend = (H - best_y) - 1;
	int idx = ops_cap - 1;
	int elem = 4;
	int elem_len = qend;
	int consumed = qend;
	int x = best_x, y = best_y;
	int s = act ? y % N : 0;
	int status = 0;
	unsigned want = 3u;
	int budget = 2 * (best_x + best_y) + 8;

	auto emit = [&](int cur, int n) {
		if (n <= 0) return;
		if (cur == elem) {
			elem_len += n;
		} else {
			if (elem != 4) { if (gl == 0) ops[idx] = (elem_len << 4) | elem; idx -= 1; }
			elem = cur;
			elem_len = n;
		}
	};
	int c_gb = -1;
	ChainBlk c_cb;
	c_cb.dir_off = 0; c_cb.tblk0 = 0; c_cb.nblk32 = 1;

	while (__builtin_amdgcn_ballot_w64(act) != 0ull) {
		if (act) {
			bool go_on = true;
			if (--budget < 0) { status = 3; go_on = false; }
			else {
				const int dx = (want != 1u) ? 1 : 0, dy = (want != 2u) ? 1 : 0;
				const int cx = x - gl * dx, cy = y - gl * dy;
				const bool inside = (cx >= 0 && cy >= 0);
				const int lx = cx > 0 ? cx : 0, ly = cy > 0 ? cy : 0;
				int sl = s - gl * dy;
				if (sl < 0) sl += N;
				const int tt = cx + cy - r0;
				const int ttc = tt > 0 ? tt : 0;
				const RowDesc2 ol = row_at(rows, ly);
				size_t widx = (size_t) (ttc >> 5) * N + sl;
				if (chained) {
					const int gb = ly / N;
					if (gb != c_gb) { c_cb = blk[gb]; c_gb = gb; }
					int wr = (ttc >> 5) - c_cb.tblk0;
					wr = wr < 0 ? 0 : (wr >= c_cb.nblk32 ? c_cb.nblk32 - 1 : wr);
					widx = c_cb.dir_off + (size_t) wr * N + (size_t) (ly - gb * N);
				}
				const uint2 w = dirs[widx];
				const int rc = ref[lx], qc = qry[ly];
				const unsigned eqm = g.ballot(rc == qc);
				const bool in_row = inside && tt >= 0 && cx >= ol.x && cx < ol.x + ol.y;
				unsigned code = plane_code(w.x, w.y, 31 - (ttc & 31));
				if (!in_row) code = 0u;
				int minC, maxC;
				valid_bounds(ol.x, ol.y, minC, maxC);

				const unsigned full = (G == 32) ? 0xffffffffu : ((1u << (G & 31)) - 1u);
				const unsigned run = g.ballot(code == want);
				const int L = (run == full) ? G : __builtin_ctz(~run);
				const unsigned low = (L == G) ? full : ((1u << L) - 1u);
				const unsigned vp = g.ballot(cx > minC && cx < maxC);
				if ((~vp & low) != 0u) { status = 2; go_on = false; }
				else {
					if (want == 3u) {
						if (L > 0) {
							const unsigned e = eqm & low;
							const unsigned starts = (((e ^ (e << 1)) & low) & ~1u) | 1u;
							const int k = __builtin_popcount(starts);
							const int op0 = (e & 1u) ? 7 : 8;
							if (k == 1) {
								emit(op0, L);
							} else {
								const unsigned after0 = starts & ~1u;
								int len0 = __builtin_ctz(after0);
								int w0 = 0;
								if (op0 == elem) len0 += elem_len;
								else if (elem != 4) { if (gl == 0) ops[idx] = (elem_len << 4) | elem; w0 = 1; }
								const bool is_start = gl < L && ((starts >> gl) & 1u) != 0u;
								const int j = __builtin_popcount(starts & ((1u << gl) - 1u));
								const unsigned rest = (starts >> gl) >> 1;
								int mylen = rest ? __builtin_ctz(rest) + 1 : L - gl;
								if (gl == 0) mylen = len0;
								const int myop = ((e >> gl) & 1u) ? 7 : 8;
								if (is_start && j < k - 1) ops[idx - w0 - j] = (mylen << 4) | myop;
								idx -= w0 + (k - 1);
								const int lastpos = 31 - __builtin_clz(starts);
								elem = ((e >> lastpos) & 1u) ? 7 : 8;
								elem_len = L - lastpos;
							}
						}
						x -= L; y -= L; consumed += L;
					} else if (want == 1u) {
						emit(1, L);
						y -= L; consumed += L;
					} else {
						emit(2, L);
						x -= L;
					}
					if (want != 2u) { s -= L; if (s < 0) s += N; }
					if (L < G) {
						const unsigned nxt = (unsigned) g.bcast((int) code, L);
						if (nxt == 0u) go_on = false;
						else if (want != 3u) want = nxt;
						else {
							const int tp = x + y - r0;
							if (nxt == 2u) {
								const unsigned wx = (unsigned) g.bcast((int) w.x, L);
								const unsigned wy = (unsigned) g.bcast((int) w.y, L);
								const int row_lo = max(g.bcast(ol.x, L), 0);
								const int b0 = 31 - (tp & 31);
								const unsigned dm = (wx & ~wy) >> b0;
								int Ld = (~dm == 0u) ? 32 : __builtin_ctz(~dm);
								const int in_word = 32 - b0;
								const int in_rowc = x - row_lo + 1;
								if (Ld > in_rowc) Ld = in_rowc;
								const int rminC = g.bcast(minC, L), rmaxC = g.bcast(maxC, L);
								if (!(x - (Ld - 1) > rminC && x < rmaxC)) { status = 2; go_on = false; }
								else {
									emit(2, Ld);
									x -= Ld;
									if (Ld == in_rowc) go_on = false;
									else if (Ld == in_word) want = 2u;
									else {
										const unsigned c2 = plane_code(wx, wy, b0 + Ld);
										if (c2 == 0u) go_on = false; else want = c2;
									}
								}
							} else {
								const int k = gl - L;
								const int tn = tp - k;
								const bool have = (k >= 0) && (cy >= 0) && (tn >= 0) && ((tn >> 5) == (ttc >> 5));
								const bool col_in = (x >= ol.x) && (x < ol.x + ol.y);
								unsigned c2 = plane_code(w.x, w.y, 31 - (tn & 31));
								if (!col_in) c2 = 0u;
								const unsigned im = g.ballot(have && c2 == 1u) >> L;
								const int Li = (~im == 0u) ? 32 : __builtin_ctz(~im);
								const unsigned ilow = (Li >= 32) ? 0xffffffffu : ((1u << Li) - 1u);
								const unsigned vpi = g.ballot(x > minC && x < maxC) >> L;
								if ((~vpi & ilow) != 0u) { status = 2; go_on = false; }
								else {
									emit(1, Li);
									y -= Li; consumed += Li;
									s -= Li; if (s < 0) s += N;
									const int en = L + Li;
									want = 1u;
									const unsigned hv = g.ballot(have);
									const int c3i = g.bcast((int) c2, en < G ? en : 0);
									if (en < G && ((hv >> en) & 1u) != 0u) {
										if (c3i == 0) go_on = false; else want = (unsigned) c3i;
									}
								}
							}
						}
					}
				}
			}
			if (!go_on) act = false;
		}
	}
	if (walked) {
		if (status == 0) {
			if (elem != 4) { if (gl == 0) ops[idx] = (elem_len << 4) | elem; idx -= 1; }
			consumed += (y + 1);
			o.ref_position = x + 1;
			o.qstart = y + 1;
			o.qend = qend;
			o.ops_first = idx + 1;
			o.n_ops = ops_cap - 1 - idx;
			if (H != consumed) status = 3;
		}
		o.status = status;
	}
}

template <int G>
__global__ void __launch_bounds__(64)
backtrack_grp_kernel(const BacktrackArgs a, const int32_t *order, const int n_order) {
	const int lane = threadIdx.x;
	Group<G> g;
	g.gl = lane & (G - 1);
	g.base = lane & ~(G - 1);
	const int q = blockIdx.x * (64 / G) + lane / G;
	bool has = q < n_order;
	const int t = has ? order[q] : 0;
	TileOut o;
	o.score = -1.0f; o.status = 0; o.best_x = 0; o.best_y = 0;
	o.ref_position = 0; o.qstart = 0; o.qend = 0; o.n_ops = 0; o.ops_first = 0; o.pad = 0;
	TileRun tr;
	TileIn ti;
	tr.skip = 1; tr.ring = 64; tr.r0 = 0; tr.ops_cap = 8; tr.dir_off = 0; tr.ops_off = 0; tr.chain_blk0 = -1;
	ti.H = 0; ti.W = 0; ti.row_off = 0; ti.ref_off = 0; ti.qry_off = 0;
	if (has) {
		tr = a.trun[t];
		o = a.tout[t];
		ti = a.tin[t];
		if (tr.skip != 0 || o.status != 0 || o.pad != 0) has = false;
	}
	const int H = ti.H, W = ti.W;
	const RowView rows = row_view(a.rsrc[t], a.rows, ti.row_off);
	bool dead = false;
	if (__builtin_amdgcn_ballot_w64(has && !(o.score > 0.0f)) != 0ull) {
		if (has && !(o.score > 0.0f)) {
			int fy = -1, fx = 0;
			bool searching = true;
			for (int y0 = 0; __builtin_amdgcn_ballot_w64(searching && y0 < H) != 0ull; y0 += G) {
				if (searching && y0 < H) {
					const int yy = y0 + g.gl;
					bool hc = false;
					int lo_i = 0;
					if (yy < H) {
						const RowDesc2 ol = row_at(rows, yy);
						long long lo = ol.x > 0 ? ol.x : 0;
						long long hi = (long long) ol.x + (long long) ol.y;
						if (hi > W) hi = W;
						hc = hi > lo;
						lo_i = (int) lo;
					}
					const unsigned m = g.ballot(hc);
					const int l = m ? __builtin_ctz(m) : 0;
					const int fxl = g.bcast(lo_i, l);
					if (m != 0u) { fy = y0 + l; fx = fxl; searching = false; }
				}
			}
			if (fy < 0) { dead = true; has = false; }
			else { o.score = 0.0f; o.best_x = fx; o.best_y = fy; }
		}
	}
	const bool chained = tr.chain_blk0 >= 0;
	int *ops = a.ops + tr.ops_off;
	const uint8_t *ref = a.seq + ti.ref_off, *qry = a.seq + ti.qry_off;
	const uint2 *dirs = reinterpret_cast<const uint2 *>(chained ? a.dirs : a.dirs + tr.dir_off);
	backtrack_walk_grp<G>(g, has, chained, H, tr.ring, tr.r0, tr.ops_cap, rows, dirs,
			a.chain_blk + (chained ? tr.chain_blk0 : 0), ref, qry, ops, o);
	if (dead) { o.score = -1.0f; o.status = 5; }
	if ((has || dead) && g.gl == 0) { o.pad = 1; a.tout[t] = o; }
}

__global__ void __launch_bounds__(64)
backtrack_kernel(const BacktrackArgs a, const int32_t *order, const int n_order) {
	if ((int) blockIdx.x >= n_order) return;
	const int t = order ? order[blockIdx.x] : (int) blockIdx.x;
	walk_tile(a, t, threadIdx.x);
}

__global__ void __launch_bounds__(256)
finalize_kernel(const TileOut *tout, const TilePlan *plan, uint64_t *dst_off, ResultRec *res,
		BatchSummary *sum, int32_t *counters, int n_tiles, unsigned long long dense_cap) {
	constexpr int T = 256;
	__shared__ unsigned long long s_part[T];
	const int tid = threadIdx.x;
	const int per = (n_tiles + T - 1) / T;
	const int t0 = min(n_tiles, tid * per), t1 = min(n_tiles, t0 + per);
	unsigned long long mine = 0;
	for (int t = t0; t < t1; ++t) {
		const TileOut o = tout[t];
		if (o.status == 0 && o.n_ops > 0) mine += (unsigned long long) o.n_ops;
	}
	s_part[tid] = mine;
	__syncthreads();
	for (int d = 1; d < T; d <<= 1) {
		const unsigned long long v = (tid >= d) ? s_part[tid - d] : 0ull;
		__syncthreads();
		s_part[tid] += v;
		__syncthreads();
	}
	unsigned long long off = s_part[tid] - mine;
	int n_valid = 0;
	for (int t = t0; t < t1; ++t) {
		const TileOut o = tout[t];
		ResultRec r;
		r.score = o.score;
		r.status = o.status;
		r.best_x = o.best_x; r.best_y = o.best_y;
		r.ref_position = o.ref_position; r.qstart = o.qstart; r.qend = o.qend;
		r.n_ops = (o.status == 0) ? o.n_ops : 0;
		r.ops_begin = off;
		r.cells = plan[t].cells;
		res[t] = r;
		dst_off[t] = off;
		if (o.status == 0) { n_valid += 1; if (o.n_ops > 0) off += (unsigned long long) o.n_ops; }
	}
	__shared__ int s_valid;
	if (tid == 0) s_valid = 0;
	__syncthreads();
	if (n_valid) atomicAdd(&s_valid, n_valid);
	__syncthreads();
	if (tid == T - 1) {
		BatchSummary b;
		b.ops_total = s_part[T - 1];
		b.dense_cap = dense_cap;
		b.n_valid = s_valid;
		b.n_redone = counters ? counters[0] : 0;
		b.chain_task_ticks = counters ? reinterpret_cast<const unsigned long long *>(counters + kCtrChainTicks)[0] : 0ull;
		b.chain_poll_ticks = counters ? reinterpret_cast<const unsigned long long *>(counters + kCtrChainTicks)[1] : 0ull;
		*sum = b;
	}
	__syncthreads();
	if (counters && tid < 64) counters[tid] = 0;
}

__global__ void __launch_bounds__(256)
compact_ops_kernel(const int32_t *regions, const TileRun *trun, const TileOut *tout,
		const uint64_t *dst_off, uint32_t *dense, int n_tiles, unsigned long long dense_cap) {
	const int t = blockIdx.x;
	if (t >= n_tiles) return;
	const TileOut o = tout[t];
	if (o.status != 0 || o.n_ops <= 0) return;
	const unsigned long long d0 = dst_off[t];
	if (d0 + (unsigned long long) o.n_ops > dense_cap) return;
	const int32_t *src = regions + trun[t].ops_off + o.ops_first;
	uint32_t *dst = dense + d0;
	for (int i = threadIdx.x; i < o.n_ops; i += blockDim.x) dst[i] = (uint32_t) src[i];
}


__global__ void __launch_bounds__(64)
chain_reduce_kernel(const int32_t *tiles, int n_tiles, const TileRun *trun, const ChainOut *cout, TileOut *tout) {
	const int q = blockIdx.x;
	if (q >= n_tiles) return;
	const int t = tiles[q];
	const TileRun tr = trun[t];
	const int lane = threadIdx.x;
	float b = -1.0f;
	int by = 0x7fffffff, bx = 0x7fffffff, failed = 0;
	for (int g = lane; g < tr.chain_nblk; g += 64) {
		const ChainOut c = cout[tr.chain_blk0 + g];
		failed |= c.failed;
		if (c.score > b) { b = c.score; by = c.best_y; bx = c.best_x; }
	}
#pragma unroll
	for (int off = 32; off >= 1; off >>= 1) {
		const float ob = __shfl_xor(b, off, 64);
		const int oy = __shfl_xor(by, off, 64);
		const int ox = __shfl_xor(bx, off, 64);
		failed |= __shfl_xor(failed, off, 64);
		if (ob > b || (ob == b && (oy < by || (oy == by && ox < bx)))) { b = ob; by = oy; bx = ox; }
	}
	if (lane == 0) {
		TileOut o;
		o.score = b;
		o.status = failed ? -1 : 0;
		o.best_x = (b > -1.0f) ? bx : 0;
		o.best_y = (b > -1.0f) ? by : 0;
		o.ref_position = 0; o.qstart = 0; o.qend = 0; o.n_ops = 0; o.ops_first = 0;
		o.pad = 0;
		tout[t] = o;
	}
}

template <int G>
static hipError_t launch_fill_gang(const FillArgs &a, int mode, hipStream_t st) {
	if (mode == kFillExact) hipLaunchKernelGGL((fill_ring_kernel<3, false, kFillExact, false, G>), dim3(a.list_n), dim3(64 * G), 0, st, a);
	else if (a.pen_table) hipLaunchKernelGGL((fill_ring_kernel<3, false, kFillTwoPhase, true, G>), dim3(a.list_n), dim3(64 * G), 0, st, a);
	else hipLaunchKernelGGL((fill_ring_kernel<3, false, kFillTwoPhase, false, G>), dim3(a.list_n), dim3(64 * G), 0, st, a);
	return hipGetLastError();
}

template <int M, bool WRAP>
static hipError_t launch_fill_twin_t(const FillArgs &a, int mode, size_t pad_lds, hipStream_t st) {
	if (mode == kFillChain) {
		if constexpr (M == 1 || M == 2 || M == 4) hipLaunchKernelGGL((fill_ring_twin_kernel<M, WRAP, kFillChain>), dim3(a.list_n), dim3(64), pad_lds, st, a);
		else return hipErrorInvalidValue;
	} else if (mode == kFillExact) hipLaunchKernelGGL((fill_ring_twin_kernel<M, WRAP, kFillExact>), dim3(a.list_n), dim3(64), 0, st, a);
	else if (!WRAP && a.pen_table) hipLaunchKernelGGL((fill_ring_twin_kernel<M, false, kFillTwoPhase, true>), dim3(a.list_n), dim3(64), 0, st, a);
	else hipLaunchKernelGGL((fill_ring_twin_kernel<M, WRAP, kFillTwoPhase>), dim3(a.list_n), dim3(64), 0, st, a);
	return hipGetLastError();
}

template <int M, bool WRAP>
static hipError_t launch_fill_t(const FillArgs &a, int mode, size_t pad_lds, hipStream_t st) {
	if (a.twin) return launch_fill_twin_t<M, WRAP>(a, mode, pad_lds, st);
	if (mode == kFillChain) {
		if constexpr (M == 1 || M == 2 || M == 4) hipLaunchKernelGGL((fill_ring_kernel<M, WRAP, kFillChain>), dim3(a.list_n), dim3(64), pad_lds, st, a);
		else return hipErrorInvalidValue;
	} else if (mode == kFillExact) hipLaunchKernelGGL((fill_ring_kernel<M, WRAP, kFillExact>), dim3(a.list_n), dim3(64), 0, st, a);
	else if (!WRAP && a.pen_table) hipLaunchKernelGGL((fill_ring_kernel<M, false, kFillTwoPhase, true>), dim3(a.list_n), dim3(64), 0, st, a);
	else hipLaunchKernelGGL((fill_ring_kernel<M, WRAP, kFillTwoPhase>), dim3(a.list_n), dim3(64), 0, st, a);
	return hipGetLastError();
}

template <int M>
static hipError_t launch_fill_w(const FillArgs &a, bool wrap, int mode, size_t pad_lds, hipStream_t st) {
	return wrap ? launch_fill_t<M, true>(a, mode, pad_lds, st) : launch_fill_t<M, false>(a, mode, pad_lds, st);
}

hipError_t launch_fill(int m, int gang, bool wrap, int mode, const FillArgs &a, size_t pad_lds, hipStream_t st) {
	if (a.list_n <= 0) return hipSuccess;
	if (gang > 1) {
		if (m != 3 || wrap || mode == kFillChain || a.twin) return hipErrorInvalidValue;
		return gang == 2 ? launch_fill_gang<2>(a, mode, st) : gang == 3 ? launch_fill_gang<3>(a, mode, st) : hipErrorInvalidValue;
	}
	switch (m) {
	case 1: return launch_fill_w<1>(a, wrap, mode, pad_lds, st);
	case 2: return launch_fill_w<2>(a, wrap, mode, pad_lds, st);
	case 3: return launch_fill_w<3>(a, wrap, mode, pad_lds, st);
	case 4: return launch_fill_w<4>(a, wrap, mode, pad_lds, st);
	default: return hipErrorInvalidValue;
	}
}

hipError_t launch_chain_reduce(const int32_t *tiles, int n_tiles, const TileRun *trun, const ChainOut *cout, TileOut *tout, hipStream_t st) {
	if (n_tiles <= 0) return hipSuccess;
	hipLaunchKernelGGL(chain_reduce_kernel, dim3(n_tiles), dim3(64), 0, st, tiles, n_tiles, trun, cout, tout);
	return hipGetLastError();
}

hipError_t launch_expand_rows(const RowSrc *rsrc, const TileIn *tin, const uint8_t *delta, const RowDesc *rowsx, RowDesc *rows,
		int n_tiles, bool closed_forms, hipStream_t st) {
	if (n_tiles <= 0) return hipSuccess;
	hipLaunchKernelGGL(expand_rows_kernel, dim3(n_tiles), dim3(64), 0, st, rsrc, tin, delta,
			reinterpret_cast<const int2 *>(rowsx), reinterpret_cast<int2 *>(rows), n_tiles, closed_forms ? 1 : 0);
	return hipGetLastError();
}

hipError_t launch_plan(const RowDesc *rows, const RowSrc *rsrc, const TileIn *tin, TilePlan *plan, int n_tiles, uint64_t rows_per_tile,
		unsigned long long max_matrix_mb, hipStream_t st) {
	if (n_tiles <= 0) return hipSuccess;
	if (rows_per_tile >= 1024)
		hipLaunchKernelGGL(plan_kernel<256>, dim3(n_tiles), dim3(256), 0, st,
				reinterpret_cast<const int2 *>(rows), rsrc, tin, plan, n_tiles, max_matrix_mb);
	else
		hipLaunchKernelGGL(plan_kernel<64>, dim3((n_tiles + 3) / 4), dim3(256), 0, st,
				reinterpret_cast<const int2 *>(rows), rsrc, tin, plan, n_tiles, max_matrix_mb);
	return hipGetLastError();
}

hipError_t launch_backtrack(const BacktrackArgs &a, const int32_t *order, int n_order, int group, hipStream_t st) {
	if (a.n_tiles <= 0) return hipSuccess;
	if (group == 16 && order != nullptr) {
		if (n_order <= 0) return hipSuccess;
		hipLaunchKernelGGL(backtrack_grp_kernel<16>, dim3((n_order + 3) / 4), dim3(64), 0, st, a, order, n_order);
	} else if (group == 4 && order != nullptr) {
		if (n_order <= 0) return hipSuccess;
		hipLaunchKernelGGL(backtrack_grp_kernel<4>, dim3((n_order + 15) / 16), dim3(64), 0, st, a, order, n_order);
	} else if (group == 8 && order != nullptr) {
		if (n_order <= 0) return hipSuccess;
		hipLaunchKernelGGL(backtrack_grp_kernel<8>, dim3((n_order + 7) / 8), dim3(64), 0, st, a, order, n_order);
	} else if (group == 32 && order != nullptr) {
		if (n_order <= 0) return hipSuccess;
		hipLaunchKernelGGL(backtrack_grp_kernel<32>, dim3((n_order + 1) / 2), dim3(64), 0, st, a, order, n_order);
	} else {
		const int nb = order != nullptr ? n_order : a.n_tiles;
		if (nb <= 0) return hipSuccess;
		hipLaunchKernelGGL(backtrack_kernel, dim3(nb), dim3(64), 0, st, a, order, nb);
	}
	return hipGetLastError();
}

hipError_t launch_finalize(const TileOut *tout, const TilePlan *plan, uint64_t *dst_off, ResultRec *res,
		BatchSummary *sum, int32_t *counters, int n_tiles, uint64_t dense_cap, hipStream_t st) {
	hipLaunchKernelGGL(finalize_kernel, dim3(1), dim3(256), 0, st, tout, plan, dst_off, res, sum, counters,
			n_tiles, (unsigned long long) dense_cap);
	return hipGetLastError();
}

hipError_t launch_compact(const int32_t *regions, const TileRun *trun, const TileOut *tout,
		const uint64_t *dst_off, uint32_t *dense, int n_tiles, uint64_t dense_cap, hipStream_t st) {
	if (n_tiles <= 0) return hipSuccess;
	hipLaunchKernelGGL(compact_ops_kernel, dim3(n_tiles), dim3(256), 0, st, regions, trun, tout, dst_off, dense, n_tiles,
			(unsigned long long) dense_cap);
	return hipGetLastError();
}

}
```

ngmlr_amd/csrc/cvx_launch.h:

```cpp
#ifndef CVX_LAUNCH_H
#define CVX_LAUNCH_H

#include <hip/hip_runtime_api.h>
#include <stdint.h>

#include "cvx_types.h"

namespace cvx {

hipError_t launch_fill(int m, int gang, bool wrap, int mode, const FillArgs &a, size_t pad_lds, hipStream_t st);
hipError_t launch_chain_reduce(const int32_t *tiles, int n_tiles, const TileRun *trun, const ChainOut *cout, TileOut *tout, hipStream_t st);
struct ScorePair {
	uint64_t ref_off, qry_off;
	uint64_t scratch_off;
	int32_t ref_len, qry_len;
};
hipError_t launch_score(const uint8_t *seq, const ScorePair *pairs, int32_t *scratch, float *out, int n, int max_ref_len, hipStream_t st);
hipError_t launch_score_diag(const uint8_t *seq, const ScorePair *pairs, float *out, int n, hipStream_t st);

struct SearchCandidate {
	uint64_t location;
	float score;
	int32_t reverse;
};
struct SearchArgs {
	const uint2 *rows;
	const uint32_t *locs;
	unsigned long long unit_offset;
	int32_t k;
	const uint8_t *seq;
	const uint64_t *seq_off;
	const int32_t *seq_len;
	int32_t n;
	unsigned long long *events;
	const uint64_t *list_off;
	uint32_t *rlist;
	uint32_t *undo;
	SearchCandidate *cand;
	int32_t *n_cand;
	float *max_hit;
	int32_t *kmer_misses;
	const int32_t *work;
	int32_t n_work;
	int32_t bits;
	float hpoc_factor;
	uint64_t *keys;
	float *scores;
	float sensitivity, min_hits;
	int32_t bin_shift;
	const uint64_t *cand_off;
};
static const int kSearchWaveLog2Min = 9, kSearchWaveLog2Max = 12, kSearchWaveLog2Default = 11;
static const int kSearchWaveSeq = 4096;
static inline int search_wave_entries(const int log2s) { return (3 << log2s) / 4; }
static inline int search_wave_log2(const unsigned long long votes) {
	for (int l = kSearchWaveLog2Min; l < kSearchWaveLog2Max; ++l) if (votes <= (unsigned long long) search_wave_entries(l)) return l;
	return kSearchWaveLog2Max;
}
static const int kSearchNeedsHbm = -2;
size_t search_wave_lds_bytes(int log2s, int seq_cap, bool slot8);
hipError_t launch_search_count(const SearchArgs &a, hipStream_t st);
hipError_t launch_search(const SearchArgs &a, hipStream_t st);
hipError_t launch_search_wave(const SearchArgs &a, int log2s, int seq_cap, bool slot8, hipStream_t st);
hipError_t launch_search_wave_hbm(const SearchArgs &a, int n_tables, unsigned int *ticket, hipStream_t st);
hipError_t launch_search_compact(const SearchCandidate *sparse, const uint64_t *src_off, const int32_t *n_cand, const uint64_t *dst_begin,
		SearchCandidate *dense, int n, hipStream_t st);

hipError_t launch_decode_windows(const uint8_t *bin, const uint64_t *starts, int n_starts,
		const WindowDesc *win, int n, uint8_t *dst, hipStream_t st);

hipError_t launch_text_size(const TextArgs &a, hipStream_t st);
hipError_t launch_text_write(const TextArgs &a, hipStream_t st);
hipError_t launch_nm_offsets(const TextArgs &a, int first, int count, unsigned long long *len, unsigned long long *off, unsigned long long *total, hipStream_t st);
hipError_t launch_nm_profile(const TextArgs &a, int first, int count, const unsigned long long *off, int32_t *triples, hipStream_t st);

size_t generic_scratch_bytes(int ring);
hipError_t launch_fill_generic(const FillArgs &a, bool sse_variant, uint8_t *scratch, const uint64_t *scratch_off, hipStream_t st);
hipError_t launch_expand_rows(const RowSrc *rsrc, const TileIn *tin, const uint8_t *delta, const RowDesc *rowsx, RowDesc *rows,
		int n_tiles, bool closed_forms, hipStream_t st);
hipError_t launch_plan(const RowDesc *rows, const RowSrc *rsrc, const TileIn *tin, TilePlan *plan, int n_tiles, uint64_t rows_per_tile,
		unsigned long long max_matrix_mb, hipStream_t st);
hipError_t launch_backtrack(const BacktrackArgs &a, const int32_t *order, int n_order, int group, hipStream_t st);
hipError_t launch_finalize(const TileOut *tout, const TilePlan *plan, uint64_t *dst_off, ResultRec *res,
		BatchSummary *sum, int32_t *counters, int n_tiles, uint64_t dense_cap, hipStream_t st);
hipError_t launch_compact(const int32_t *regions, const TileRun *trun, const TileOut *tout,
		const uint64_t *dst_off, uint32_t *dense, int n_tiles, uint64_t dense_cap, hipStream_t st);

}
#endif
```

ngmlr_amd/csrc/cvx_rt_align.cpp:

```cpp
#include <algorithm>
#include <atomic>
#include <chrono>
#include <cstdio>
#include <cstdlib>
#include <cstring>
#include <new>
#include <string>
#include <vector>

#include "cvx_rt.h"

namespace {

static const size_t kPoolBatches = 8;

cvx_batch_s *acquire_batch(cvx_context *h) {
	if (!h->pool.empty()) {
		cvx_batch_s *b = h->pool.back();
		h->pool.pop_back();
		return b;
	}
	return new (std::nothrow) cvx_batch_s();
}

void recycle_batch(cvx_context *h, cvx_batch_s *b) {
	const bool failed = b->state == kFailed;
	b->state = kEmpty;
	b->in_flight = false;
	b->have_ops = false;
	b->have_refs = false;
	b->text_done = false;
	b->fail_rc = CVX_OK;
	b->fail_msg.clear();
	if (h) {
		auto it = std::find(h->live.begin(), h->live.end(), b);
		if (it != h->live.end()) h->live.erase(it);
	}
	if (h && !failed && h->pool.size() < kPoolBatches) { h->pool.push_back(b); return; }
	b->release();
	delete b;
}

void discard_batch(cvx_context *h, cvx_batch_s *b) {
	(void) hipDeviceSynchronize();
	if (h) {
		auto it = std::find(h->pending.begin(), h->pending.end(), b);
		if (it != h->pending.end()) h->pending.erase(it);
		it = std::find(h->live.begin(), h->live.end(), b);
		if (it != h->live.end()) h->live.erase(it);
	}
	b->release();
	delete b;
}

int fail_job(cvx_batch_s *b, int rc) {
	(void) hipDeviceSynchronize();
	b->state = kFailed;
	b->fail_rc = rc;
	b->fail_msg = g_err;
	return rc;
}

int stage_upload(cvx_context *h, cvx_batch_s *b, int32_t n, const cvx_tile *tiles,
		const cvx_genome_s *genome = nullptr, const uint64_t *ref_position = nullptr) {
	RC_TRY(ensure_streams(h));
	UploadLayout L;
	std::vector<TileIn> tin;
	int bad = -1;
	const bool windows = genome != nullptr;
	const int lrc = upload_layout(n, tiles, tin, L, &bad, windows);
	if (lrc == kLayoutMalformed) { set_err("tile %d malformed", bad); return CVX_ERR_ARG; }
	if (lrc == kLayoutTooLarge) {
		set_err("%llu sequence bytes exceed one batch (4 GiB); split the batch", (unsigned long long) L.seq_total);
		return CVX_ERR_ARG;
	}
	b->n = n;
	b->state = kEmpty;
	b->have_ops = false;
	b->have_refs = false;
	b->text_done = false;
	b->ops_total = 0;
	b->seq_total = L.seq_total;
	b->n_rows = L.n_rows;
	memset(&b->timing, 0, sizeof(b->timing));
	RC_TRY(b->make_events());
	const size_t n1 = (size_t) std::max(n, 1);
	const size_t rows1 = (size_t) std::max<uint64_t>(L.arena_rows, 1);
	RC_TRY(b->h_delta.ensure((size_t) L.delta_total + 256));
	RC_TRY(b->h_rsrc.ensure(n1 * sizeof(RowSrc)));
	RC_TRY(b->d_delta.ensure((size_t) L.delta_total + 256));
	RC_TRY(b->d_rsrc.ensure(n1));
	RC_TRY(b->h_tin.ensure(n1 * sizeof(TileIn)));
	RC_TRY(b->h_plan.ensure(n1 * sizeof(TilePlan)));
	RC_TRY(b->h_res.ensure(n1 * sizeof(ResultRec) + sizeof(BatchSummary)));
	RC_TRY(b->d_seq.ensure((size_t) L.seq_total + 256));
	RC_TRY(b->d_rows.ensure(rows1));
	RC_TRY(b->d_tin.ensure(n1));
	RC_TRY(b->d_plan.ensure(n1));
	RC_TRY(b->d_trun.ensure(n1));
	RC_TRY(b->d_tout.ensure(n1));
	RC_TRY(b->d_dstoff.ensure(n1));
	RC_TRY(b->d_lists.ensure(2 * n1));
	if (b->d_counters.cap < 64) {
		RC_TRY(b->d_counters.ensure(64));
		HIP_TRY(hipMemset(b->d_counters.p, 0, b->d_counters.cap * sizeof(int32_t)));
	}
	RC_TRY(b->d_res.ensure(n1 * sizeof(ResultRec) + sizeof(BatchSummary)));
	if (n) memcpy(b->h_tin.p, tin.data(), (size_t) n * sizeof(TileIn));

	const bool qry_pinned = L.qry_contig && in_pinned_block(tiles[0].qry, L.qry_bytes + 4);
	const bool ref_pinned = L.ref_contig && in_pinned_block(tiles[0].ref, L.ref_bytes + 4);
	UploadSchedule sch;
	build_upload_schedule(L, tin, n, qry_pinned, ref_pinned, std::min(h->pack_threads, PackPool::get().size()), sch);
	b->zero_copy_bytes = sch.zero_copy_bytes;
	if (sch.pack_seq) RC_TRY(b->h_seq.ensure((size_t) L.seq_total + 256));
	uint8_t *hseq = b->h_seq.as<uint8_t>();
	uint8_t *hdelta = b->h_delta.as<uint8_t>();
	if (sch.pack_seq) upload_zero_pads(L, hseq);
	if (sch.zero_bytes) {
		RC_TRY(b->h_zero.ensure((size_t) sch.zero_bytes));
		if (b->zero_cap != b->h_zero.cap) { memset(b->h_zero.p, 0, b->h_zero.cap); b->zero_cap = b->h_zero.cap; }
	}
	hipStream_t st = h->s_io;
	const void *const from[] = { hseq, hdelta, b->h_zero.p, n ? tiles[0].qry : nullptr, n ? tiles[0].ref : nullptr };
	auto issue = [&](size_t r0, size_t r1) -> int {
		for (size_t r = r0; r < r1; ++r) {
			const UploadCopy &c = sch.copies[r];
			uint8_t *dst = (c.dst == kToSeq ? b->d_seq.p : b->d_delta.p) + c.dst_off;
			if (c.src == kClearOnDevice) HIP_TRY(hipMemsetAsync(dst, 0, (size_t) c.len, st));
			else HIP_TRY(hipMemcpyAsync(dst, static_cast<const uint8_t *>(from[c.src]) + c.src_off, (size_t) c.len, hipMemcpyHostToDevice, st));
		}
		return CVX_OK;
	};
	RC_TRY(issue(0, sch.n_leading));
	std::vector<RowOverflow> overflow;
	for (const UploadPiece &pc : sch.pieces) {
		upload_pack_piece(sch, pc, tiles, tin, L, hseq, hdelta, overflow);
		RC_TRY(issue(pc.rec0, pc.rec1));
	}
	if (n) HIP_TRY(hipMemcpyAsync(b->d_tin.p, b->h_tin.p, (size_t) n * sizeof(TileIn), hipMemcpyHostToDevice, st));
	if (n) {
		const uint64_t n_x = misfit_rows(overflow);
		b->n_rowsx = n_x;
		if (n_x) {
			RC_TRY(b->h_rowsx.ensure((size_t) n_x * sizeof(RowDesc)));
			RC_TRY(b->d_rowsx.ensure((size_t) n_x));
			RowDesc *hx = b->h_rowsx.as<RowDesc>();
			place_misfits(overflow, tin, L.rsrc, hx);
			HIP_TRY(hipMemcpyAsync(b->d_rowsx.p, hx, (size_t) n_x * sizeof(RowDesc), hipMemcpyHostToDevice, st));
		}
		memcpy(b->h_rsrc.p, L.rsrc.data(), (size_t) n * sizeof(RowSrc));
		HIP_TRY(hipMemcpyAsync(b->d_rsrc.p, b->h_rsrc.p, (size_t) n * sizeof(RowSrc), hipMemcpyHostToDevice, st));
		if (L.arena_rows) HIP_TRY(launch_expand_rows(b->d_rsrc.p, b->d_tin.p, b->d_delta.p, b->d_rowsx.p, b->d_rows.p, n, false, st));
	}
	if (windows && n) {
		RC_TRY(b->h_win.ensure((size_t) n * sizeof(WindowDesc)));
		RC_TRY(b->d_win.ensure((size_t) n));
		WindowDesc *hw = b->h_win.as<WindowDesc>();
		for (int i = 0; i < n; ++i) {
			hw[i].position = ref_position[i];
			hw[i].dst_off = tin[(size_t) i].ref_off;
			hw[i].n_chars = tiles[i].ref_len;
		}
		HIP_TRY(hipMemcpyAsync(b->d_win.p, hw, (size_t) n * sizeof(WindowDesc), hipMemcpyHostToDevice, st));
		RC_TRY(issue(sch.n_staged, sch.copies.size()));
		HIP_TRY(launch_decode_windows(genome->d_bin.p, genome->d_starts.p, genome->n_starts, b->d_win.p, n, b->d_seq.p, st));
		RC_TRY(b->h_refs.ensure((size_t) L.ref_bytes + 64));
		HIP_TRY(hipMemcpyAsync(b->h_refs.p, b->d_seq.p + L.ref_base, (size_t) L.ref_bytes, hipMemcpyDeviceToHost, st));
		b->refs_base = L.ref_base;
		b->have_refs = true;
	}
	b->state = kUploaded;
	return CVX_OK;
}

int stage_plan(cvx_context *h, cvx_batch_s *b, hipStream_t st) {
	const int n = b->n;
	HIP_TRY(hipEventRecord(b->ev[0], st));
	if (n) {
		HIP_TRY(launch_plan(b->d_rows.p, b->d_rsrc.p, b->d_tin.p, b->d_plan.p, n, b->n_rows / (uint64_t) n, h->max_matrix_mb, st));
		HIP_TRY(hipMemcpyAsync(b->h_plan.p, b->d_plan.p, (size_t) n * sizeof(TilePlan), hipMemcpyDeviceToHost, st));
	}
	HIP_TRY(hipEventRecord(b->ev[1], st));
	HIP_TRY(hipEventRecord(b->ev_in, st));
	b->state = kPlanned;
	return CVX_OK;
}

void kernel_args(const cvx_context *h, const cvx_batch_s *b, const ChainBlk *chain_blk, FillArgs &a, BacktrackArgs &ba) {
	a.seq = ba.seq = b->d_seq.p;
	a.rows = ba.rows = reinterpret_cast<const RowDesc2 *>(b->d_rows.p);
	a.rsrc = ba.rsrc = b->d_rsrc.p;
	a.tin = ba.tin = b->d_tin.p;
	a.trun = ba.trun = b->d_trun.p;
	a.tout = ba.tout = b->d_tout.p;
	ba.dirs = a.dirs = b->d_dirs.p;
	a.ops = ba.ops = b->d_regions.p;
	a.list = nullptr; a.list_n = 0;
	a.redo_count = b->d_counters.p;
	a.late_min_groups = h->tune_late_min;
	a.late_shift = h->tune_late_shift;
	a.pen_table = h->tune_pen_table;
	a.tasks = nullptr; a.chain_ticket = nullptr; a.bnd = nullptr; a.chain_out = nullptr; a.bnd_epoch = 0; a.chain_prio = 0;
	a.sp = h->sp;
	a.twin = h->scalar_twin ? 1 : 0;
	ba.chain_blk = chain_blk;
	ba.n_tiles = b->n;
}

int issue_walk(cvx_batch_s *b, const BacktrackArgs &ba, const WalkPlan &w, size_t at, int count, hipStream_t ws, hipStream_t side) {
	if (count <= 0) return CVX_OK;
	const int32_t *list = b->d_lists.p + at;
	const bool fork = w.n_long > 0 && side != nullptr;
	if (fork) {
		HIP_TRY(hipEventRecord(b->ev_bt0, ws));
		HIP_TRY(hipStreamWaitEvent(side, b->ev_bt0, 0));
	}
	if (w.n_long > 0) HIP_TRY(launch_backtrack(ba, list, w.n_long, w.long_lanes, fork ? side : ws));
	if (fork) HIP_TRY(hipEventRecord(b->ev_bt1, side));
	HIP_TRY(launch_backtrack(ba, list + w.n_long, count - w.n_long, w.bulk_lanes, ws));
	if (fork) HIP_TRY(hipStreamWaitEvent(ws, b->ev_bt1, 0));
	return CVX_OK;
}

int upload_chain(cvx_batch_s *b, const HostPlan &hp, const ComputeSchedule &sch, hipStream_t st) {
	RC_TRY(b->h_chain.ensure(sch.chain_bytes));
	uint8_t *hc = b->h_chain.as<uint8_t>();
	for (size_t c = 0; c < hp.chain_tasks.size(); ++c)
		if (!hp.chain_tasks[c].empty()) memcpy(hc + sch.chain_task_off[c], hp.chain_tasks[c].data(), hp.chain_tasks[c].size() * sizeof(ChainTask));
	memcpy(hc + sch.chain_blk_off, hp.chain_blk.data(), hp.chain_blk.size() * sizeof(ChainBlk));
	for (size_t c = 0; c < hp.chain_tiles.size(); ++c)
		if (!hp.chain_tiles[c].empty()) memcpy(hc + sch.chain_tile_off[c], hp.chain_tiles[c].data(), hp.chain_tiles[c].size() * sizeof(int32_t));
	RC_TRY(b->d_chain.ensure(sch.chain_bytes));
	RC_TRY(b->d_chain_out.ensure(hp.chain_blk.size()));
	{
		const size_t had = b->d_bnd.cap;
		RC_TRY(b->d_bnd.ensure((size_t) hp.bnd_recs + 64));
		if (b->d_bnd.cap != had || b->bnd_epoch >= kBndEpochMax) {
			HIP_TRY(hipMemsetAsync(b->d_bnd.p, 0, b->d_bnd.cap * sizeof(BoundaryRec), st));
			b->bnd_epoch = 0;
		}
		b->bnd_epoch += 1;
	}
	HIP_TRY(hipMemcpyAsync(b->d_chain.p, hc, sch.chain_bytes, hipMemcpyHostToDevice, st));
	return CVX_OK;
}

int stage_compute(cvx_context *h, cvx_batch_s *b, bool streaming = false) {
	const int n = b->n;
	if (h->test_fail_compute > 0 && --h->test_fail_compute == 0) {
		set_err("stage_compute: failure injected by CVX_TUNE_FAIL_COMPUTE");
		return CVX_ERR_OOM;
	}
	const bool second = streaming && n > 0 && n < kSmallJobTiles && !h->single_lane && ((h->small_jobs++ & 1u) != 0u);
	hipStream_t const S_main = second ? h->s_main2 : h->s_main;
	hipStream_t const S_post = second ? h->s_post2 : h->s_post;
	hipStream_t const *S_aux = second ? h->aux2 : h->aux;
	b->s_run = S_main;
	hipStream_t st = S_main;
	HIP_TRY(hipEventSynchronize(b->ev_in));
	b->launches.clear();
	b->ops_total = 0;
	b->have_ops = false;
	if (n == 0) {
		HIP_TRY(hipEventRecord(b->ev[4], st));
		hipStream_t ps = h->overlap_post ? S_post : S_main;
		HIP_TRY(hipStreamWaitEvent(ps, b->ev[4], 0));
		HIP_TRY(hipEventRecord(b->ev[2], ps));
		HIP_TRY(hipEventRecord(b->ev[3], ps));
		HIP_TRY(hipEventRecord(b->ev_res, ps));
		b->state = kComputed;
		return CVX_OK;
	}

	HostPlan hp;
	PlanTuning tune;
	tune.min_slots = h->tune_min_slots; tune.max_slots = h->tune_max_slots; tune.force_wrap = h->tune_force_wrap; tune.chain_m = h->tune_chain_m;
	tune.force_generic = h->force_generic ? 1 : 0;
	tune.long_steps = h->tune_long_steps; tune.small_batch = h->tune_small_batch; tune.long_need = h->tune_long_need;
	tune.no_gangs = h->tune_gangs ? 0 : 1;
	const RowSrc *rsrc = b->h_rsrc.as<RowSrc>();
	host_plan_rows(n, b->plan(), b->tin(), [&](int i, std::vector<RowDesc> &tmp) -> const RowDesc * {
		tmp.resize((size_t) std::max(b->tin()[(size_t) i].H, 1));
		expand_rows_host(rsrc[(size_t) i], b->tin()[(size_t) i].H, b->h_delta.as<uint8_t>(), b->h_rowsx.as<RowDesc>(), tmp.data());
		return tmp.data();
	}, true, tune, hp);
	const std::vector<int32_t> &generic = hp.generic;
	RC_TRY(b->d_dirs.ensure((size_t) hp.dir_dwords + 64));
	RC_TRY(b->d_regions.ensure((size_t) hp.ops_ints + 64));
	b->dense_cap = std::min<uint64_t>(hp.ops_ints, hp.ops_ints / 3 + 64ull * (uint64_t) n);
	RC_TRY(b->d_dense.ensure((size_t) b->dense_cap + 64));
	b->dense_cap = std::max<uint64_t>(b->dense_cap, b->d_dense.cap - 64);

	RC_TRY(b->h_trun.ensure((size_t) n * sizeof(TileRun)));
	RC_TRY(b->h_tout.ensure((size_t) n * sizeof(TileOut)));
	RC_TRY(b->h_lists.ensure((size_t) 2 * n * sizeof(int32_t) + 64));
	ScheduleTuning stune;
	stune.exact_steps = h->tune_exact_steps; stune.bt_group = h->bt_group; stune.bt_per_class = h->bt_per_class; stune.overlap_post = h->overlap_post;
	stune.wide_prio = h->tune_wide_prio; stune.gang_prio = h->tune_gang_prio; stune.chain_prio = h->tune_chain_prio; stune.chain_lds_kb = h->tune_chain_lds_kb;
	ComputeSchedule sch;
	build_schedule(hp, b->plan(), b->tin(), n, b->n_rows, h->num_cus, stune, b->h_lists.as<int32_t>(), sch);
	memcpy(b->h_trun.p, hp.trun.data(), (size_t) n * sizeof(TileRun));
	memcpy(b->h_tout.p, hp.tout.data(), (size_t) n * sizeof(TileOut));
	if (!generic.empty()) {
		RC_TRY(b->h_goff.ensure((generic.size() + 1) * sizeof(uint64_t)));
		uint64_t *goff = b->h_goff.as<uint64_t>();
		goff[0] = 0;
		for (size_t g = 0; g < generic.size(); ++g)
			goff[g + 1] = goff[g] + (uint64_t) generic_scratch_bytes(hp.trun[(size_t) generic[g]].ring);
		RC_TRY(b->d_gscratch.ensure((size_t) goff[generic.size()] + 256));
		RC_TRY(b->d_gscratch_off.ensure(generic.size() + 1));
		HIP_TRY(hipMemcpyAsync(b->d_gscratch_off.p, goff, (generic.size() + 1) * sizeof(uint64_t), hipMemcpyHostToDevice, st));
	}
	if (hp.n_chained) RC_TRY(upload_chain(b, hp, sch, st));
	HIP_TRY(hipMemcpyAsync(b->d_trun.p, b->h_trun.p, (size_t) n * sizeof(TileRun), hipMemcpyHostToDevice, st));
	HIP_TRY(hipMemcpyAsync(b->d_tout.p, b->h_tout.p, (size_t) n * sizeof(TileOut), hipMemcpyHostToDevice, st));
	if (sch.n_listed) HIP_TRY(hipMemcpyAsync(b->d_lists.p, b->h_lists.p, sch.n_listed * sizeof(int32_t), hipMemcpyHostToDevice, st));
	HIP_TRY(hipEventRecord(b->ev[4], st));

	FillArgs fa;
	BacktrackArgs ba;
	kernel_args(h, b, hp.n_chained ? reinterpret_cast<const ChainBlk *>(b->d_chain.p + sch.chain_blk_off) : nullptr, fa, ba);
	static_assert(kAuxStreams == 2, "StreamSlot names two side streams");
	hipStream_t fill_streams[kStreamSlots];
	fill_streams[kOnSide0] = S_aux[0]; fill_streams[kOnPost] = S_post; fill_streams[kOnMain] = st; fill_streams[kOnSide1] = S_aux[1];
	const int launches = (int) sch.launches.size();
	while (b->lev.size() < (size_t) launches * kLevPerLaunch) {
		hipEvent_t e;
		HIP_TRY(hipEventCreate(&e));
		b->lev.push_back(e);
	}
	for (int i = 0; i < launches; ++i) {
		const FillLaunch &L = sch.launches[(size_t) i];
		const hipStream_t ls = fill_streams[L.stream];
		const hipEvent_t *le = &b->lev[(size_t) i * kLevPerLaunch];
		const bool wrap = L.wrap != 0;
		b->launches.push_back(L.info);
		HIP_TRY(hipStreamWaitEvent(ls, b->ev[4], 0));
		HIP_TRY(hipEventRecord(le[kLevStart], ls));
		FillArgs a = fa;
		a.chain_prio = L.prio;
		if (L.kind == CVX_LAUNCH_CHAINED) {
			a.list_n = L.count;
			a.tasks = reinterpret_cast<const ChainTask *>(b->d_chain.p + sch.chain_task_off[L.slot]);
			a.chain_ticket = b->d_counters.p + 8 + L.slot;
			a.bnd = b->d_bnd.p;
			a.bnd_epoch = b->bnd_epoch;
			a.chain_out = b->d_chain_out.p;
			HIP_TRY(launch_fill(L.m, 1, wrap, kModeChain, a, L.pad_lds, ls));
			HIP_TRY(launch_chain_reduce(reinterpret_cast<const int32_t *>(b->d_chain.p + sch.chain_tile_off[L.slot]), L.info.n_tiles,
					b->d_trun.p, b->d_chain_out.p, b->d_tout.p, ls));
			HIP_TRY(hipEventRecord(le[kLevTwoPhase], ls));
		} else if (L.kind == CVX_LAUNCH_CATCH_ALL) {
			a.list = b->d_lists.p + L.list_off;
			a.list_n = L.count;
			HIP_TRY(launch_fill_generic(a, h->sse_variant, b->d_gscratch.p, b->d_gscratch_off.p, ls));
			HIP_TRY(hipEventRecord(le[kLevTwoPhase], ls));
		} else {
			a.list = b->d_lists.p + L.list_off;
			a.list_n = L.n_direct;
			if (a.list_n > 0) HIP_TRY(launch_fill(L.m, L.gang, wrap, kModeExact, a, 0, ls));
			a.list += L.n_direct;
			a.list_n = L.count - L.n_direct;
			if (a.list_n > 0) HIP_TRY(launch_fill(L.m, L.gang, wrap, kModeTwoPhase, a, 0, ls));
			HIP_TRY(hipEventRecord(le[kLevTwoPhase], ls));
			if (a.list_n > 0) HIP_TRY(launch_fill(L.m, L.gang, wrap, kModeExact, a, 0, ls));
		}
		HIP_TRY(hipEventRecord(le[kLevExact], ls));
		if (sch.per_class) RC_TRY(issue_walk(b, ba, L.walk, L.bt_off, L.bt_count, ls, nullptr));
		HIP_TRY(hipEventRecord(le[kLevWalked], ls));
	}
	st = h->overlap_post ? S_post : S_main;
	HIP_TRY(hipStreamWaitEvent(st, b->ev[4], 0));
	for (int i = 0; i < launches; ++i) HIP_TRY(hipStreamWaitEvent(st, b->lev[(size_t) i * kLevPerLaunch + kLevWalked], 0));
	HIP_TRY(hipEventRecord(b->ev[2], st));

	if (!sch.per_class) RC_TRY(issue_walk(b, ba, sch.walk, sch.bt_begin, sch.n_walk, st, S_aux[0]));
	ResultRec *d_rec = reinterpret_cast<ResultRec *>(b->d_res.p);
	BatchSummary *d_sum = reinterpret_cast<BatchSummary *>(b->d_res.p + (size_t) n * sizeof(ResultRec));
	HIP_TRY(launch_finalize(b->d_tout.p, b->d_plan.p, b->d_dstoff.p, d_rec, d_sum, b->d_counters.p, n, b->dense_cap, st));
	HIP_TRY(launch_compact(b->d_regions.p, b->d_trun.p, b->d_tout.p, b->d_dstoff.p, b->d_dense.p, n, b->dense_cap, st));
	HIP_TRY(hipEventRecord(b->ev[3], st));
	HIP_TRY(hipMemcpyAsync(b->h_res.p, b->d_res.p, (size_t) n * sizeof(ResultRec) + sizeof(BatchSummary), hipMemcpyDeviceToHost, st));
	HIP_TRY(hipEventRecord(b->ev_res, st));

	b->timing.cells = hp.cells;
	b->timing.active_cells = hp.active;
	b->timing.dir_bytes = hp.dir_dwords * 4;
	b->timing.n_fill_launches = launches;
	b->timing.n_tiles_fast = hp.n_fast;
	b->timing.n_tiles_chained = hp.n_chained;
	b->state = kComputed;
	return CVX_OK;
}

int stage_results(cvx_context *h, cvx_batch_s *b) {
	(void) h;
	if (b->state < kComputed) { set_err("internal: results requested from a batch whose kernels were never queued (state %d)", b->state); return CVX_ERR_ARG; }
	HIP_TRY(hipEventSynchronize(b->ev_res));
	if (b->n == 0) { b->ops_total = 0; b->state = kFinished; return CVX_OK; }
	const BatchSummary *s = b->summary();
	b->ops_total = s->ops_total;
	const int launches = b->timing.n_fill_launches;
	for (int i = 0; i < launches; ++i) b->launches[(size_t) i].ms = ev_ms(b->lev[(size_t) i * kLevPerLaunch + kLevStart], b->lev[(size_t) i * kLevPerLaunch + kLevTwoPhase]);
	b->timing.plan_ms = ev_ms(b->ev[0], b->ev[1]);
	float fill_end = 0.0f;
	for (int i = 0; i < launches; ++i) fill_end = std::max(fill_end, ev_ms(b->ev[4], b->lev[(size_t) i * kLevPerLaunch + kLevExact]));
	if (launches == 0) fill_end = ev_ms(b->ev[4], b->ev[2]);
	b->timing.fill_ms = fill_end;
	b->timing.backtrack_ms = std::max(0.0f, ev_ms(b->ev[4], b->ev[3]) - fill_end);
	b->timing.total_ms = b->timing.plan_ms + ev_ms(b->ev[4], b->ev[3]);
	b->timing.n_tiles_redone = s->n_redone;
	b->timing.chain_task_ticks = s->chain_task_ticks;
	b->timing.chain_poll_ticks = s->chain_poll_ticks;
	b->state = kFinished;
	return CVX_OK;
}

int stage_ops(cvx_context *h, cvx_batch_s *b) {
	if (b->have_ops) return CVX_OK;
	if (b->ops_total > b->dense_cap) {
		const uint64_t cap = b->ops_total;
		RC_TRY(b->d_dense.ensure((size_t) cap + 64));
		b->dense_cap = b->d_dense.cap - 64;
		hipStream_t ps = b->s_run ? b->s_run : h->s_main;
		HIP_TRY(launch_compact(b->d_regions.p, b->d_trun.p, b->d_tout.p, b->d_dstoff.p, b->d_dense.p, b->n, b->dense_cap, ps));
		HIP_TRY(hipStreamSynchronize(ps));
	}
	if (b->ops_total) {
		RC_TRY(b->h_ops.ensure((size_t) b->ops_total * sizeof(uint32_t)));
		HIP_TRY(hipMemcpyAsync(b->h_ops.p, b->d_dense.p, (size_t) b->ops_total * sizeof(uint32_t), hipMemcpyDeviceToHost, h->s_io));
		HIP_TRY(hipStreamSynchronize(h->s_io));
	}
	b->have_ops = true;
	return CVX_OK;
}

int pump(cvx_context *h, bool block, const cvx_batch_s *upto) {
	while (!h->pending.empty()) {
		cvx_batch_s *b = h->pending.front();
		if (!block) {
			hipError_t q = hipEventQuery(b->ev_in);
			if (q == hipErrorNotReady) { (void) hipGetLastError(); break; }
			if (q != hipSuccess) { set_err("hipEventQuery: %s", hipGetErrorString(q)); h->pending.erase(h->pending.begin()); (void) fail_job(b, CVX_ERR_HIP); continue; }
		}
		h->pending.erase(h->pending.begin());
		const int rc = stage_compute(h, b, true);
		if (rc != CVX_OK) (void) fail_job(b, rc);
		if (upto && b == upto) break;
	}
	return CVX_OK;
}

}

extern "C" {


int cvx_batch_upload(cvx_handle h, int32_t n, const cvx_tile *tiles, cvx_batch *out) {
	ABI_GUARD_BEGIN
	if (!h || !out || n < 0 || (n > 0 && !tiles)) { set_err("cvx_batch_upload: bad argument"); return CVX_ERR_ARG; }
	*out = nullptr;
	HIP_TRY(hipSetDevice(h->device));
	cvx_batch_s *b = acquire_batch(h);
	if (!b) return CVX_ERR_OOM;
	int rc = stage_upload(h, b, n, tiles);
	if (rc == CVX_OK) {
		hipError_t e = hipStreamSynchronize(h->s_io);
		if (e != hipSuccess) { set_err("upload copy failed: %s", hipGetErrorString(e)); rc = CVX_ERR_HIP; }
	}
	if (rc != CVX_OK) { discard_batch(h, b); return rc; }
	*out = b;
	return CVX_OK;
	ABI_GUARD_END
}

int cvx_batch_run(cvx_handle h, cvx_batch b) {
	ABI_GUARD_BEGIN
	if (!h || !b || b->state < kUploaded) { set_err("cvx_batch_run: NULL argument / batch not uploaded"); return CVX_ERR_ARG; }
	HIP_TRY(hipSetDevice(h->device));
	RC_TRY(stage_plan(h, b, h->s_main));
	RC_TRY(stage_compute(h, b));
	RC_TRY(stage_results(h, b));
	HIP_TRY(hipStreamSynchronize(h->s_main));
	HIP_TRY(hipStreamSynchronize(h->s_post));
	return CVX_OK;
	ABI_GUARD_END
}

int cvx_batch_timing(cvx_batch b, cvx_timing *t) {
	ABI_GUARD_BEGIN
	if (!b || !t) { set_err("cvx_batch_timing: NULL argument"); return CVX_ERR_ARG; }
	*t = b->timing;
	return CVX_OK;
	ABI_GUARD_END
}

int cvx_batch_launch_info(cvx_batch b, int32_t i, cvx_launch_info *info) {
	ABI_GUARD_BEGIN
	if (!b || !info || b->state < kFinished || i < 0 || (size_t) i >= b->launches.size()) { set_err("cvx_batch_launch_info: bad index"); return CVX_ERR_ARG; }
	*info = b->launches[(size_t) i];
	return CVX_OK;
	ABI_GUARD_END
}

int cvx_batch_ops_total(cvx_batch b, uint64_t *n_ops) {
	ABI_GUARD_BEGIN
	if (!b || !n_ops || b->state < kFinished) { set_err("cvx_batch_ops_total: batch not run"); return CVX_ERR_ARG; }
	*n_ops = b->ops_total;
	return CVX_OK;
	ABI_GUARD_END
}

int cvx_batch_download(cvx_handle h, cvx_batch b, cvx_result *results, uint32_t *ops_arena,
		uint64_t ops_capacity, uint64_t *ops_used) {
	ABI_GUARD_BEGIN
	if (!h || !b || b->state < kFinished || (b->n > 0 && !results)) { set_err("cvx_batch_download: bad argument / batch not run"); return CVX_ERR_ARG; }
	HIP_TRY(hipSetDevice(h->device));
	if (ops_used) *ops_used = b->ops_total;
	static_assert(sizeof(cvx_result) == sizeof(ResultRec), "ResultRec mirrors cvx_result");
	if (b->n) memcpy(results, b->res(), (size_t) b->n * sizeof(cvx_result));
	if (b->ops_total > ops_capacity) {
		set_err("cvx_batch_download: ops arena too small (%llu needed, %llu given)",
				(unsigned long long) b->ops_total, (unsigned long long) ops_capacity);
		return CVX_ERR_CAPACITY;
	}
	if (b->ops_total) {
		if (!ops_arena) { set_err("cvx_batch_download: NULL ops arena"); return CVX_ERR_ARG; }
		RC_TRY(stage_ops(h, b));
		memcpy(ops_arena, b->h_ops.p, (size_t) b->ops_total * sizeof(uint32_t));
	}
	return CVX_OK;
	ABI_GUARD_END
}

void cvx_batch_free(cvx_handle h, cvx_batch b) {
	ABI_GUARD_BEGIN
	if (!b) return;
	if (h) (void) hipSetDevice(h->device);
	recycle_batch(h, b);
	ABI_GUARD_END_VOID
}

int cvx_align_batch(cvx_handle h, int32_t n, const cvx_tile *tiles, cvx_result *results,
		uint32_t *ops_arena, uint64_t ops_capacity, uint64_t *ops_used) {
	ABI_GUARD_BEGIN
	cvx_job j = nullptr;
	int rc = cvx_submit(h, n, tiles, &j);
	if (rc != CVX_OK) return rc;
	const cvx_result *res = nullptr;
	const uint32_t *ops = nullptr;
	uint64_t n_ops = 0;
	rc = cvx_wait(h, j, &res, &ops, &n_ops);
	if (rc == CVX_OK) {
		if (ops_used) *ops_used = n_ops;
		if (n && results) memcpy(results, res, (size_t) n * sizeof(cvx_result));
		if (n && !results) { set_err("cvx_align_batch: NULL results"); rc = CVX_ERR_ARG; }
		else if (n_ops > ops_capacity) {
			set_err("cvx_align_batch: ops arena too small (%llu needed, %llu given)",
					(unsigned long long) n_ops, (unsigned long long) ops_capacity);
			rc = CVX_ERR_CAPACITY;
		} else if (n_ops) {
			if (!ops_arena) { set_err("cvx_align_batch: NULL ops arena"); rc = CVX_ERR_ARG; }
			else memcpy(ops_arena, ops, (size_t) n_ops * sizeof(uint32_t));
		}
		cvx_job_release(h, j);
	}
	return rc;
	ABI_GUARD_END
}


static int submit_common(cvx_handle h, int32_t n, const cvx_tile *tiles, const cvx_genome_s *genome, const uint64_t *ref_position, cvx_job *out) {
	if (!h || !out || n < 0 || (n > 0 && !tiles) || (genome && n > 0 && !ref_position)) { set_err("cvx_submit: bad argument"); return CVX_ERR_ARG; }
	*out = nullptr;
	if (genome && genome->device != h->device) { set_err("cvx_submit_windows: the genome lives on device %d, the handle on %d", genome->device, h->device); return CVX_ERR_ARG; }
	HIP_TRY(hipSetDevice(h->device));
	static const bool trace = getenv("CVX_SUBMIT_TRACE") != nullptr;
	const auto t0 = std::chrono::steady_clock::now();
	if (h->live.empty() && !g_deferred.empty()) g_deferred.drain();
	(void) pump(h, false, nullptr);
	const auto t1 = std::chrono::steady_clock::now();
	cvx_batch_s *b = acquire_batch(h);
	if (!b) return CVX_ERR_OOM;
	b->bind(h->marks);
	const auto t2 = std::chrono::steady_clock::now();
	int rc = stage_upload(h, b, n, tiles, genome, ref_position);
	const auto t3 = std::chrono::steady_clock::now();
	if (rc == CVX_OK) rc = stage_plan(h, b, h->s_io);
	if (rc != CVX_OK) { discard_batch(h, b); return rc; }
	b->in_flight = true;
	h->pending.push_back(b);
	h->live.push_back(b);
	const auto t4 = std::chrono::steady_clock::now();
	(void) pump(h, false, nullptr);
	if (trace) {
		const auto t5 = std::chrono::steady_clock::now();
		auto ms = [](std::chrono::steady_clock::time_point a, std::chrono::steady_clock::time_point c) { return std::chrono::duration<double, std::milli>(c - a).count(); };
		if (ms(t0, t5) > 5.0) fprintf(stderr, "cvx_submit: %d tiles in %.2f ms: pump %.2f, batch slot %.2f, upload stage %.2f, plan stage %.2f, pump %.2f\n", n, ms(t0, t5), ms(t0, t1), ms(t1, t2), ms(t2, t3), ms(t3, t4), ms(t4, t5));
	}
	*out = b;
	return CVX_OK;
}

int cvx_submit(cvx_handle h, int32_t n, const cvx_tile *tiles, cvx_job *out) {
	ABI_GUARD_BEGIN return submit_common(h, n, tiles, nullptr, nullptr, out); ABI_GUARD_END
}

int cvx_submit_windows(cvx_handle h, cvx_genome g, int32_t n, const cvx_tile *tiles, const uint64_t *ref_position, cvx_job *out) {
	ABI_GUARD_BEGIN
	if (!g) { set_err("cvx_submit_windows: NULL genome"); return CVX_ERR_ARG; }
	return submit_common(h, n, tiles, g, ref_position, out);
	ABI_GUARD_END
}

int cvx_wait(cvx_handle h, cvx_job j, const cvx_result **results, const uint32_t **ops, uint64_t *n_ops) {
	ABI_GUARD_BEGIN
	if (!h || !j || !j->in_flight) { set_err("cvx_wait: not a submitted job"); return CVX_ERR_ARG; }
	HIP_TRY(hipSetDevice(h->device));
	if (j->state != kFailed && j->state < kComputed) (void) pump(h, true, j);
	if (j->state != kFailed && j->state < kFinished) { const int rc = stage_results(h, j); if (rc != CVX_OK) (void) fail_job(j, rc); }
	if (j->state != kFailed) { const int rc = stage_ops(h, j); if (rc != CVX_OK) (void) fail_job(j, rc); }
	if (j->state == kFailed) { g_err = j->fail_msg; return j->fail_rc; }
	(void) pump(h, false, nullptr);
	if (results) *results = reinterpret_cast<const cvx_result *>(j->res());
	if (ops) *ops = j->h_ops.as<uint32_t>();
	if (n_ops) *n_ops = j->ops_total;
	return CVX_OK;
	ABI_GUARD_END
}

int cvx_job_window_refs(cvx_handle h, cvx_job j, const char **refs) {
	ABI_GUARD_BEGIN
	if (!h || !j || !refs || j->state < kFinished) { set_err("cvx_job_window_refs: job not finished (call cvx_wait first)"); return CVX_ERR_ARG; }
	if (!j->have_refs) { set_err("cvx_job_window_refs: not a job of cvx_submit_windows"); return CVX_ERR_ARG; }
	const char *base = j->h_refs.as<char>();
	const TileIn *tin = j->tin();
	for (int i = 0; i < j->n; ++i) refs[i] = base + (tin[i].ref_off - j->refs_base);
	return CVX_OK;
	ABI_GUARD_END
}

int cvx_job_poll(cvx_handle h, cvx_job j, int32_t *done) {
	ABI_GUARD_BEGIN
	if (!h || !j || !j->in_flight || !done) { set_err("cvx_job_poll: not a submitted job"); return CVX_ERR_ARG; }
	HIP_TRY(hipSetDevice(h->device));
	(void) pump(h, false, nullptr);
	*done = 0;
	if (j->state == kFailed || j->state >= kFinished) { *done = 1; return CVX_OK; }
	if (j->state >= kComputed) {
		hipError_t q = hipEventQuery(j->ev_res);
		if (q == hipSuccess) *done = 1;
		else if (q == hipErrorNotReady) (void) hipGetLastError();
		else { set_err("hipEventQuery: %s", hipGetErrorString(q)); return CVX_ERR_HIP; }
	}
	return CVX_OK;
	ABI_GUARD_END
}

int cvx_job_timing(cvx_job j, cvx_timing *t) { ABI_GUARD_BEGIN return cvx_batch_timing(j, t); ABI_GUARD_END }
int cvx_job_launch_info(cvx_job j, int32_t i, cvx_launch_info *info) { ABI_GUARD_BEGIN return cvx_batch_launch_info(j, i, info); ABI_GUARD_END }

void cvx_job_release(cvx_handle h, cvx_job j) {
	ABI_GUARD_BEGIN
	if (!j) return;
	if (h) {
		(void) hipSetDevice(h->device);
		auto it = std::find(h->pending.begin(), h->pending.end(), j);
		if (it != h->pending.end()) h->pending.erase(it);
		if ((j->state >= kPlanned && j->state < kFinished) || j->state == kFailed) (void) hipDeviceSynchronize();
	}
	recycle_batch(h, j);
	ABI_GUARD_END_VOID
}


int cvx_corridor_rows(cvx_handle h, const cvx_tile *tile, int32_t *offset, int32_t *length) {
	ABI_GUARD_BEGIN
	if (!h || !tile || tile->qry_len < 0 || (tile->qry_len > 0 && (!offset || !length))) { set_err("cvx_corridor_rows: bad argument"); return CVX_ERR_ARG; }
	const int H = tile->qry_len;
	if (H == 0) return CVX_OK;
	if (tile->corridor_kind == CVX_CORRIDOR_ROWS) {
		if (!tile->row_offset || !tile->row_length || (tile->row_stride_bytes & 3) || tile->row_stride_bytes < 4) { set_err("cvx_corridor_rows: bad row arrays"); return CVX_ERR_ARG; }
		for (int y = 0; y < H; ++y) {
			memcpy(&offset[y], (const char *) tile->row_offset + (size_t) y * (size_t) tile->row_stride_bytes, 4);
			memcpy(&length[y], (const char *) tile->row_length + (size_t) y * (size_t) tile->row_stride_bytes, 4);
		}
		return CVX_OK;
	}
	cvx_tile t = *tile;
	static const char dummy[1] = {0};
	t.ref = t.qry = dummy;
	t.ref_len = 0;
	std::vector<TileIn> tin;
	UploadLayout L;
	int bad = -1;
	{
		cvx_tile probe = t;
		if (upload_layout(1, &probe, tin, L, &bad, false) != kLayoutOk) { set_err("cvx_corridor_rows: malformed corridor descriptor"); return CVX_ERR_ARG; }
	}
	HIP_TRY(hipSetDevice(h->device));
	RowSrc rs = L.rsrc[0];
	TileIn ti;
	memset(&ti, 0, sizeof(ti));
	ti.H = H;
	DevBuf<RowSrc> d_rs;
	DevBuf<TileIn> d_ti;
	DevBuf<RowDesc> d_rows;
	int rc = d_rs.ensure(1);
	if (rc == CVX_OK) rc = d_ti.ensure(1);
	if (rc == CVX_OK) rc = d_rows.ensure((size_t) H);
	std::vector<RowDesc> rows((size_t) H);
	hipError_t e = hipSuccess;
	if (rc == CVX_OK) {
		e = hipMemcpy(d_rs.p, &rs, sizeof(rs), hipMemcpyHostToDevice);
		if (e == hipSuccess) e = hipMemcpy(d_ti.p, &ti, sizeof(ti), hipMemcpyHostToDevice);
		if (e == hipSuccess) e = launch_expand_rows(d_rs.p, d_ti.p, nullptr, nullptr, d_rows.p, 1, true, h->s_main);
		if (e == hipSuccess) e = hipStreamSynchronize(h->s_main);
		if (e == hipSuccess) e = hipMemcpy(rows.data(), d_rows.p, (size_t) H * sizeof(RowDesc), hipMemcpyDeviceToHost);
	}
	d_rs.release(); d_ti.release(); d_rows.release();
	if (rc != CVX_OK) return rc;
	if (e != hipSuccess) { set_err("cvx_corridor_rows: %s", hipGetErrorString(e)); return CVX_ERR_HIP; }
	for (int y = 0; y < H; ++y) { offset[y] = rows[(size_t) y].off; length[y] = rows[(size_t) y].len; }
	return CVX_OK;
	ABI_GUARD_END
}

int cvx_pack_probe(int32_t n, const cvx_tile *tiles, int32_t iters, int32_t assume_page_locked, double *ms_per_iter, uint64_t *bytes_touched) {
	ABI_GUARD_BEGIN
	if (n < 0 || (n > 0 && !tiles) || iters <= 0 || !ms_per_iter) { set_err("cvx_pack_probe: bad argument"); return CVX_ERR_ARG; }
	std::vector<uint8_t> hseq, hdelta;
	uint64_t touched = 0;
	const auto c0 = std::chrono::steady_clock::now();
	for (int it = 0; it < iters; ++it) {
		UploadLayout L;
		std::vector<TileIn> tin;
		int bad = -1;
		const int lrc = upload_layout(n, tiles, tin, L, &bad, false);
		if (lrc != kLayoutOk) { set_err("cvx_pack_probe: tile %d malformed / batch too large", bad); return CVX_ERR_ARG; }
		UploadSchedule sch;
		build_upload_schedule(L, tin, n, assume_page_locked != 0, assume_page_locked != 0, PackPool::get().size(), sch);
		if (hseq.size() < L.seq_total + 256) hseq.resize((size_t) L.seq_total + 256);
		if (hdelta.size() < L.delta_total + 256) hdelta.resize((size_t) L.delta_total + 256);
		std::vector<RowOverflow> overflow;
		for (const UploadPiece &pc : sch.pieces) upload_pack_piece(sch, pc, tiles, tin, L, hseq.data(), hdelta.data(), overflow);
		touched = 2 * ((sch.zc_qry ? 0 : L.qry_bytes) + (sch.zc_ref ? 0 : L.ref_bytes)) + L.delta_total * 9ull + (uint64_t) n * (sizeof(TileIn) + sizeof(RowSrc) + sizeof(cvx_tile));
	}
	const double dt = std::chrono::duration<double>(std::chrono::steady_clock::now() - c0).count();
	*ms_per_iter = dt * 1e3 / iters;
	if (bytes_touched) *bytes_touched = touched;
	return CVX_OK;
	ABI_GUARD_END
}

}
```

ngmlr_amd/csrc/cvx_types.h:

```cpp
#ifndef CVX_TYPES_H
#define CVX_TYPES_H

#include <stdint.h>

namespace cvx {

struct RowDesc2 { int32_t x, y; };
struct RowDesc { int32_t off, len; };

static const int kSwitchMargin = 4;
static const int kRingMax = 4096;
static const int kLateMinGroups = 128;
static const int kLateShift = 5;
static const int kPadRedo = 2;
static const int kPenEntries = 64;
static const int kPenClamp = kPenEntries - 8;
static const int kGangDepth = 8;
static const int kChainChunk = 16;

struct ScoreParams {
	float mat, mis, go, ge, gem, decay;
	float misx;
};

enum RowFormat { kRowsDelta8 = 0, kRowsExplicit = 1, kRowsAffine = 2, kRowsConst = 3 };
struct RowSrc {
	uint64_t src_off;
	int32_t off0;
	int32_t width;
	int32_t fmt;
	float k, d, right;
};

#if defined(__HIPCC__)
__host__ __device__
#endif
inline int32_t affine_row_offset(int y, float d, float k, float right) {
	const float a = (float) y - d;
	const float q = a / k;
	const float r = q - right;
	return (int32_t) r;
}

#if defined(__HIPCC__)
struct RowView {
	const RowDesc2 *rows;
	int32_t fmt;
	int32_t width;
	int32_t y0;
	float k, d, right;
};
__device__ __forceinline__ RowView row_view(const RowSrc &rs, const RowDesc2 *arena, const uint64_t row_off, const int y0 = 0) {
	RowView v;
	v.rows = arena + row_off + y0;
	v.fmt = rs.fmt; v.width = rs.width; v.y0 = y0;
	v.k = rs.k; v.d = rs.d;
	v.right = rs.fmt == kRowsConst ? __int_as_float(rs.off0) : rs.right;
	return v;
}
__device__ __forceinline__ RowDesc2 row_at(const RowView &v, const int y) {
	RowDesc2 r;
	if (v.fmt == kRowsAffine || v.fmt == kRowsConst) {
		r.x = v.fmt == kRowsConst ? __float_as_int(v.right) : affine_row_offset(y + v.y0, v.d, v.k, v.right);
		r.y = v.width;
	} else {
		r = v.rows[y];
	}
	return r;
}
#endif

struct TileIn {
	uint32_t ref_off;
	uint32_t qry_off;
	int32_t W, H;
	uint64_t row_off;
	uint64_t reserved;
};

enum PlanFlags {
	kPlanIrregular = 1,
	kPlanEmpty = 2,
	kPlanTooLarge = 4,
	kPlanWrap16 = 8
};

struct TilePlan {
	int32_t r0;
	int32_t rend;
	int32_t need;
	int32_t flags;
	uint64_t cells;
	uint64_t active;
};

struct TileRun {
	uint64_t dir_off;
	uint64_t ops_off;
	int32_t ring;
	int32_t ops_cap;
	int32_t r0;
	int32_t nsteps;
	int32_t skip;
	int32_t mnw;
	int32_t chain_blk0;
	int32_t chain_nblk;
};

struct ChainBlk {
	uint64_t dir_off;
	int32_t tblk0;
	int32_t nblk32;
};

struct ChainTask {
	int32_t tile;
	int32_t y0;
	int32_t rows;
	int32_t r0;
	int32_t nsteps;
	int32_t blk;
	int32_t prev;
	int32_t bnd_lo;
	int32_t bnd_len;
	int32_t has_next;
	uint64_t dir_off;
	uint64_t bnd_in_off;
	uint64_t bnd_out_off;
};

struct BoundaryRec {
	uint32_t s_bits;
	uint32_t meta;
};
static const uint32_t kBndEpochMax = 32767;

struct BoundaryVal {
	float V, S;
	uint32_t run;
	uint32_t is_ins;
};

struct ChainOut {
	float score;
	int32_t best_x, best_y;
	int32_t failed;
};

struct TileOut {
	float score;
	int32_t status;
	int32_t best_x, best_y;
	int32_t ref_position, qstart, qend;
	int32_t n_ops;
	int32_t ops_first;
	int32_t pad;
};

struct ResultRec {
	float score;
	int32_t status;
	int32_t best_x, best_y;
	int32_t ref_position, qstart, qend;
	int32_t n_ops;
	uint64_t ops_begin;
	uint64_t cells;
};

struct BatchSummary {
	uint64_t ops_total;
	uint64_t dense_cap;
	int32_t n_valid;
	int32_t n_redone;
	uint64_t chain_task_ticks, chain_poll_ticks;
};
static const int kCtrChainTicks = 16;

struct WindowDesc {
	uint64_t position;
	uint64_t dst_off;
	int64_t n_chars;
};

struct TextRec {
	int32_t ret;
	float score;
	int32_t position_offset, qstart, qend, nm;
	float identity;
	int32_t alignment_length, cigar_op_count, sv_type;
	int32_t first_ref, first_read, last_ref, last_read;
	int32_t nm_count, cigar_len, md_len;
};

struct TextArgs {
	const uint8_t *seq;
	const TileIn *tin;
	const TileRun *trun;
	const TileOut *tout;
	const int32_t *ops;
	const int32_t *ext_qstart;
	const int32_t *ext_qend;
	TextRec *recs;
	unsigned long long *text_len;
	unsigned long long *text_off;
	unsigned long long *text_total;
	uint8_t *text;
	int32_t n_tiles;
};

struct FillArgs {
	const uint8_t *seq;
	const RowDesc2 *rows;
	const RowSrc *rsrc;
	const TileIn *tin;
	const TileRun *trun;
	TileOut *tout;
	uint32_t *dirs;
	const int32_t *list;
	int32_t list_n;
	int32_t *redo_count;
	const ChainTask *tasks;
	int32_t *chain_ticket;
	BoundaryRec *bnd;
	uint32_t bnd_epoch;
	int32_t chain_prio;
	ChainOut *chain_out;
	int32_t late_min_groups;
	int32_t late_shift;
	int32_t pen_table;
	int32_t *ops;
	ScoreParams sp;
	int32_t twin;
};

struct BacktrackArgs {
	const ChainBlk *chain_blk;
	const uint8_t *seq;
	const RowDesc2 *rows;
	const RowSrc *rsrc;
	const TileIn *tin;
	const TileRun *trun;
	TileOut *tout;
	const uint32_t *dirs;
	int32_t *ops;
	int32_t n_tiles;
};

}

#endif
```

Before: 16070.

## Parallelize finalize scan, stage plan rows in shared memory, clamp runs less often

Replaces the single-block finalize kernel with a three-kernel multi-block scan: per-block sums, a carry scan, then a write pass. The plan kernel now precomputes row spans into a shared-memory ring per strip, so the forward searches read shared memory instead of recomputing row descriptors. The penalty run clamp moves from every row to each direction-word flush, with the penalty table enlarged to cover the longer reachable runs. The change also adds batch summary and plan query API functions, and the extra launches add small fixed overhead for small batches.

```diff
diff --git a/include/cvx_align.h b/include/cvx_align.h
--- a/include/cvx_align.h
+++ b/include/cvx_align.h
@@ -137,6 +137,12 @@
 int cvx_batch_run(cvx_handle h, cvx_batch b);
 int cvx_batch_timing(cvx_batch b, cvx_timing *t);
 int cvx_batch_ops_total(cvx_batch b, uint64_t *n_ops);
+int cvx_batch_summary(cvx_batch b, uint64_t *ops_total, int32_t *n_valid, int32_t *n_redone);
+typedef struct cvx_tile_plan {
+	int32_t r0, rend, need, flags;
+	uint64_t cells, active;
+} cvx_tile_plan;
+int cvx_batch_plan(cvx_batch b, int32_t first, int32_t count, cvx_tile_plan *out);
 int cvx_batch_launch_info(cvx_batch b, int32_t i, cvx_launch_info *info);
 int cvx_batch_download(cvx_handle h, cvx_batch b, cvx_result *results,
 		uint32_t *ops_arena, uint64_t ops_capacity, uint64_t *ops_used);
diff --git a/ngmlr_amd/capi.py b/ngmlr_amd/capi.py
--- a/ngmlr_amd/capi.py
+++ b/ngmlr_amd/capi.py
@@ -18,7 +18,7 @@
 
 EXPORTS = ("cvx_last_error", "cvx_abi_version", "cvx_source_id", "cvx_device_count", "cvx_device_synchronize", "cvx_create", "cvx_destroy",
            "cvx_align_batch", "cvx_batch_upload", "cvx_batch_run", "cvx_batch_timing",
-           "cvx_batch_ops_total", "cvx_batch_launch_info", "cvx_batch_download", "cvx_batch_free",
+           "cvx_batch_ops_total", "cvx_batch_summary", "cvx_batch_plan", "cvx_batch_launch_info", "cvx_batch_download", "cvx_batch_free",
            "cvx_submit", "cvx_wait", "cvx_job_timing", "cvx_job_launch_info", "cvx_job_release",
            "cvx_format_alignment", "cvx_format_batch", "cvx_score_batch",
            "cvx_genome_encoded_bytes", "cvx_genome_encode", "cvx_genome_upload", "cvx_genome_free",
@@ -162,6 +162,8 @@
     lib.cvx_batch_timing.argtypes = [C.c_void_p, C.POINTER(CvxTiming)]
     lib.cvx_batch_launch_info.argtypes = [C.c_void_p, C.c_int32, C.POINTER(CvxLaunchInfo)]
     lib.cvx_batch_ops_total.argtypes = [C.c_void_p, C.POINTER(C.c_uint64)]
+    lib.cvx_batch_summary.argtypes = [C.c_void_p, C.POINTER(C.c_uint64), C.POINTER(C.c_int32), C.POINTER(C.c_int32)]
+    lib.cvx_batch_plan.argtypes = [C.c_void_p, C.c_int32, C.c_int32, C.c_void_p]
     lib.cvx_batch_download.argtypes = [C.c_void_p, C.c_void_p, C.POINTER(CvxResult), C.c_void_p,
                                        C.c_uint64, C.POINTER(C.c_uint64)]
     lib.cvx_batch_free.argtypes = [C.c_void_p, C.c_void_p]
diff --git a/ngmlr_amd/csrc/cvx_fill_ring.inc b/ngmlr_amd/csrc/cvx_fill_ring.inc
--- a/ngmlr_amd/csrc/cvx_fill_ring.inc
+++ b/ngmlr_amd/csrc/cvx_fill_ring.inc
@@ -230,6 +230,11 @@
 			const unsigned dl = (unsigned) tid * (M * 2);
 #pragma unroll
 			for (int j = 0; j < M; ++j) { d[dl + 2 * j] = accA[j]; d[dl + 2 * j + 1] = accB[j]; }
+			if (TAB) {
+				static_assert(kPenClampSteps == 32, "the run registers are clamped where the direction words are flushed");
+#pragma unroll
+				for (int j = 0; j < M; ++j) { const int c = min((int) drun[j], 4 * kPenClamp); drun[j] = (run_t) c; irun[j] = (run_t) c; }
+			}
 		}
 
 #pragma unroll
@@ -270,7 +275,7 @@
 				if (lane == 0) {
 					uV0 = vv;
 					uS0 = sc;
-					uI0 = TAB ? (run_t) (int) (run16 << 2) : (run_t) (float) run16;
+					uI0 = TAB ? (run_t) (int) ((run16 < (unsigned) kPenClamp ? run16 : (unsigned) kPenClamp) << 2) : (run_t) (float) run16;
 				}
 				mIu0 = (mIu0 & ~1ull) | (u64) ins;
 			};
@@ -431,10 +436,6 @@
 				take_row(j, s_rec[CHAIN ? 0 : wv * M + j][lane], r, false);
 			}
 		}
-		if (TAB) {
-#pragma unroll
-			for (int j = 0; j < M; ++j) { const int c = min((int) drun[j], 4 * kPenClamp); drun[j] = (run_t) c; irun[j] = (run_t) c; }
-		}
 		if (stage_now) {
 			stage_rows(stage_next, stage_slot);
 			stage_advance();
diff --git a/ngmlr_amd/csrc/cvx_kernels.hip b/ngmlr_amd/csrc/cvx_kernels.hip
--- a/ngmlr_amd/csrc/cvx_kernels.hip
+++ b/ngmlr_amd/csrc/cvx_kernels.hip
@@ -3,6 +3,7 @@
 
 #include "cvx_types.h"
 #include "cvx_launch.h"
+#include "cvx_plan_logic.h"
 
 namespace cvx {
 
@@ -15,15 +16,6 @@
 	return __int_as_float(rot1_i(__float_as_int(v)));
 }
 
-
-CVX_DEV void row_span(const int2 ol, int W, int y, int &gs, int &ge) {
-	long long lo = ol.x > 0 ? ol.x : 0;
-	long long hi = (long long) ol.x + (long long) ol.y;
-	if (hi > W) hi = W;
-	if (hi < lo) hi = lo;
-	gs = (int) (lo + y);
-	ge = (int) (hi + y);
-}
 
 template <int TPT>
 __global__ void __launch_bounds__(256)
@@ -34,8 +26,11 @@
 	const int t = blockIdx.x * TPB + sub;
 	const bool live = t < n_tiles;
 	const TileIn ti = tin[live ? t : 0];
-	const RowView rv = row_view(rsrc[live ? t : 0], reinterpret_cast<const RowDesc2 *>(rows), ti.row_off);
-	auto row = [&](const int y) { const RowDesc2 q = row_at(rv, y); return make_int2(q.x, q.y); };
+	const RowSrc rs = rsrc[live ? t : 0];
+	PlanRows pr;
+	pr.rows = reinterpret_cast<const RowDesc2 *>(rows) + ti.row_off;
+	pr.fmt = rs.fmt; pr.width = rs.width; pr.off0 = rs.off0;
+	pr.k = rs.k; pr.d = rs.d; pr.right = rs.right;
 	const int H = live ? ti.H : 0, W = ti.W;
 
 	__shared__ unsigned long long s_cells[TPB], s_active[TPB];
@@ -43,95 +38,38 @@
 	if (ltid == 0) { s_cells[sub] = 0; s_active[sub] = 0; s_need[sub] = 1; s_flags[sub] = 0; s_maxlen[sub] = 0; s_rend[sub] = -0x7fffffff; s_r0[sub] = 0x7fffffff; }
 	__syncthreads();
 
-	unsigned long long cells = 0, active = 0;
-	int need = 1, flags = 0, maxlen = 0, rendmax = -0x7fffffff, r0min = 0x7fffffff;
-	for (int y = ltid; y < H; y += TPT) {
-		const int2 ol = row(y);
-		int gs, ge;
-		row_span(ol, W, y, gs, ge);
-		cells += (unsigned long long) (long long) ol.y;
-		active += (unsigned long long) (ge - gs);
-		if (ol.y > maxlen) maxlen = ol.y;
-		if (ge > rendmax) rendmax = ge;
-		if (gs < r0min) r0min = gs;
-		if (y > 0) {
-			int pgs, pge;
-			row_span(row(y - 1), W, y - 1, pgs, pge);
-			if (gs <= pgs) flags |= kPlanIrregular;
-			if (ge < pge) flags |= kPlanIrregular;
-		}
-		const int lim = ge + kSwitchMargin;
-		auto starts_before = [&](int yy) {
-			int mgs, mge;
-			row_span(row(yy), W, yy, mgs, mge);
-			return mgs < lim;
-		};
-		int lo = y + 1, hi = H;
-		int g = y + 1 + ((lim - gs) >> 1);
-		g = g < lo ? lo : g;
-		if (g < hi) {
-			if (starts_before(g)) {
-				lo = g + 1;
-				for (int step = 1; lo < hi; step <<= 1) {
-					const int p = (lo + step - 1 < hi) ? lo + step - 1 : hi - 1;
-					if (starts_before(p)) lo = p + 1; else { hi = p; break; }
-				}
-			} else {
-				hi = g;
-				for (int step = 1; lo < hi; step <<= 1) {
-					const int p = (hi - step > lo) ? hi - step : lo;
-					if (starts_before(p)) { lo = p + 1; break; } else hi = p;
-				}
-			}
-		}
-		while (lo < hi) {
-			const int mid = (lo + hi) >> 1;
-			if (starts_before(mid)) lo = mid + 1; else hi = mid;
-		}
-		const int n = lo - y + 1;
-		if (n > need) need = n;
-		if (H > 32767) {
-			long long lo_y = ol.x > 0 ? ol.x : 0;
-			long long hi_y = (long long) ol.x + (long long) ol.y;
-			if (hi_y > W) hi_y = W;
-			if (hi_y < lo_y) hi_y = lo_y;
-			int a = y + 1, b = H;
-			while (a < b) {
-				const int mid = (a + b) >> 1;
-				const int2 om = row(mid);
-				const long long lo_m = om.x > 0 ? om.x : 0;
-				if (lo_m < hi_y) a = mid + 1; else b = mid;
-			}
-			if (a - y > maxlen) maxlen = a - y;
-		}
+	PlanAcc acc = plan_acc_init();
+	if constexpr (TPT == 256) {
+		__shared__ int s_gs[kPlanCap], s_ge[kPlanCap];
+		int staged = 0;
+		for (int Y = 0; Y < H; Y += kPlanStrip) {
+			const int end = plan_strip_staged(Y, H);
+			__syncthreads();
+			for (int r = staged + ltid; r < end; r += TPT) plan_stage_row(pr, W, r, s_gs, s_ge);
+			staged = end;
+			__syncthreads();
+			const int yend = min(H, Y + kPlanStrip);
+			for (int y = Y + ltid; y < yend; y += TPT) plan_row_staged(acc, pr, W, H, y, staged, s_gs, s_ge);
+		}
+	} else {
+		for (int y = ltid; y < H; y += TPT) plan_row_ondemand(acc, pr, W, H, y);
 	}
 	if (H > 0) {
-		atomicAdd(&s_cells[sub], cells);
-		atomicAdd(&s_active[sub], active);
-		atomicMax(&s_need[sub], need);
-		atomicOr(&s_flags[sub], flags);
-		atomicMax(&s_maxlen[sub], maxlen);
-		atomicMax(&s_rend[sub], rendmax);
-		atomicMin(&s_r0[sub], r0min);
+		atomicAdd(&s_cells[sub], acc.cells);
+		atomicAdd(&s_active[sub], acc.active);
+		atomicMax(&s_need[sub], acc.need);
+		atomicOr(&s_flags[sub], acc.flags);
+		atomicMax(&s_maxlen[sub], acc.maxlen);
+		atomicMax(&s_rend[sub], acc.rendmax);
+		atomicMin(&s_r0[sub], acc.r0min);
 	}
 	__syncthreads();
 
 	if (ltid == 0 && live) {
-		TilePlan p;
-		p.cells = s_cells[sub];
-		p.active = s_active[sub];
-		p.need = s_need[sub];
-		int f = s_flags[sub];
-		int r0 = 0, rend = 0;
-		if (H > 0) { r0 = s_r0[sub]; rend = s_rend[sub]; }
-		if (H <= 0 || s_active[sub] == 0) f |= kPlanEmpty;
-		const float mb = (float) s_cells[sub] / 1000.0f / 1000.0f;
-		if (!((unsigned long long) mb < max_matrix_mb)) f |= kPlanTooLarge;
-		if (s_maxlen[sub] > 32767 || (H > 32767 && (f & kPlanIrregular))) f |= kPlanWrap16;
-		p.r0 = r0;
-		p.rend = rend;
-		p.flags = f;
-		plan[t] = p;
+		PlanAcc all;
+		all.cells = s_cells[sub]; all.active = s_active[sub]; all.need = s_need[sub]; all.flags = s_flags[sub];
+		all.maxlen = s_maxlen[sub]; all.rendmax = s_rend[sub]; all.r0min = s_r0[sub];
+		plan[t] = plan_finish(all, H, max_matrix_mb);
 	}
 }
 
@@ -748,60 +686,97 @@
 	walk_tile(a, t, threadIdx.x);
 }
 
-__global__ void __launch_bounds__(256)
-finalize_kernel(const TileOut *tout, const TilePlan *plan, uint64_t *dst_off, ResultRec *res,
-		BatchSummary *sum, int32_t *counters, int n_tiles, unsigned long long dense_cap) {
-	constexpr int T = 256;
-	__shared__ unsigned long long s_part[T];
+CVX_DEV unsigned long long finalize_block_scan(unsigned long long v, unsigned long long *s_wave, unsigned long long &total) {
+	const int tid = threadIdx.x, lane = tid & 63, w = tid >> 6;
+#pragma unroll
+	for (int k = 1; k < 64; k <<= 1) {
+		const unsigned long long u = __shfl_up(v, k, 64);
+		if (lane >= k) v += u;
+	}
+	__syncthreads();
+	if (lane == 63) s_wave[w] = v;
+	__syncthreads();
+	unsigned long long before = 0, all = 0;
+#pragma unroll
+	for (int i = 0; i < kFinalizeTile / 64; ++i) {
+		const unsigned long long x = s_wave[i];
+		if (i < w) before += x;
+		all += x;
+	}
+	total = all;
+	return v + before;
+}
+
+__global__ void __launch_bounds__(kFinalizeTile)
+finalize_sum_kernel(const TileOut *tout, unsigned long long *part, int n_tiles, int nblk) {
+	__shared__ unsigned long long s_wave[kFinalizeTile / 64];
+	const int t = blockIdx.x * kFinalizeTile + threadIdx.x;
+	unsigned long long ops = 0, valid = 0;
+	if (t < n_tiles) {
+		const int status = tout[t].status, n_ops = tout[t].n_ops;
+		if (status == 0) { valid = 1; if (n_ops > 0) ops = (unsigned long long) n_ops; }
+	}
+	unsigned long long total;
+	finalize_block_scan(ops | (valid << 40), s_wave, total);
+	if (threadIdx.x == 0) {
+		part[blockIdx.x] = total & ((1ull << 40) - 1);
+		part[nblk + blockIdx.x] = total >> 40;
+	}
+}
+
+__global__ void __launch_bounds__(kFinalizeTile)
+finalize_scan_kernel(unsigned long long *part, int nblk, BatchSummary *sum, int32_t *counters, unsigned long long dense_cap) {
+	__shared__ unsigned long long s_wave[kFinalizeTile / 64];
 	const int tid = threadIdx.x;
-	const int per = (n_tiles + T - 1) / T;
-	const int t0 = min(n_tiles, tid * per), t1 = min(n_tiles, t0 + per);
-	unsigned long long mine = 0;
-	for (int t = t0; t < t1; ++t) {
-		const TileOut o = tout[t];
-		if (o.status == 0 && o.n_ops > 0) mine += (unsigned long long) o.n_ops;
-	}
-	s_part[tid] = mine;
-	__syncthreads();
-	for (int d = 1; d < T; d <<= 1) {
-		const unsigned long long v = (tid >= d) ? s_part[tid - d] : 0ull;
-		__syncthreads();
-		s_part[tid] += v;
-		__syncthreads();
-	}
-	unsigned long long off = s_part[tid] - mine;
-	int n_valid = 0;
-	for (int t = t0; t < t1; ++t) {
-		const TileOut o = tout[t];
-		ResultRec r;
-		r.score = o.score;
-		r.status = o.status;
-		r.best_x = o.best_x; r.best_y = o.best_y;
-		r.ref_position = o.ref_position; r.qstart = o.qstart; r.qend = o.qend;
-		r.n_ops = (o.status == 0) ? o.n_ops : 0;
-		r.ops_begin = off;
-		r.cells = plan[t].cells;
-		res[t] = r;
-		dst_off[t] = off;
-		if (o.status == 0) { n_valid += 1; if (o.n_ops > 0) off += (unsigned long long) o.n_ops; }
-	}
-	__shared__ int s_valid;
-	if (tid == 0) s_valid = 0;
-	__syncthreads();
-	if (n_valid) atomicAdd(&s_valid, n_valid);
-	__syncthreads();
-	if (tid == T - 1) {
-		BatchSummary b;
-		b.ops_total = s_part[T - 1];
-		b.dense_cap = dense_cap;
-		b.n_valid = s_valid;
-		b.n_redone = counters ? counters[0] : 0;
-		b.chain_task_ticks = counters ? reinterpret_cast<const unsigned long long *>(counters + kCtrChainTicks)[0] : 0ull;
-		b.chain_poll_ticks = counters ? reinterpret_cast<const unsigned long long *>(counters + kCtrChainTicks)[1] : 0ull;
-		*sum = b;
+	unsigned long long carry = 0, valid = 0;
+	for (int b0 = 0; b0 < nblk; b0 += kFinalizeTile) {
+		const int b = b0 + tid;
+		const unsigned long long mine = b < nblk ? part[b] : 0ull;
+		unsigned long long total;
+		const unsigned long long incl = finalize_block_scan(mine, s_wave, total);
+		if (b < nblk) part[b] = carry + incl - mine;
+		carry += total;
+		finalize_block_scan(b < nblk ? part[nblk + b] : 0ull, s_wave, total);
+		valid += total;
+	}
+	if (tid == 0) {
+		BatchSummary s;
+		s.ops_total = carry;
+		s.dense_cap = dense_cap;
+		s.n_valid = (int32_t) valid;
+		s.n_redone = counters ? counters[0] : 0;
+		s.chain_task_ticks = counters ? reinterpret_cast<const unsigned long long *>(counters + kCtrChainTicks)[0] : 0ull;
+		s.chain_poll_ticks = counters ? reinterpret_cast<const unsigned long long *>(counters + kCtrChainTicks)[1] : 0ull;
+		*sum = s;
 	}
 	__syncthreads();
 	if (counters && tid < 64) counters[tid] = 0;
+}
+
+__global__ void __launch_bounds__(kFinalizeTile)
+finalize_write_kernel(const TileOut *tout, const TilePlan *plan, const unsigned long long *part, uint64_t *dst_off, ResultRec *res, int n_tiles) {
+	__shared__ unsigned long long s_wave[kFinalizeTile / 64];
+	const int t = blockIdx.x * kFinalizeTile + threadIdx.x;
+	const bool live = t < n_tiles;
+	TileOut o;
+	unsigned long long ops = 0;
+	if (live) {
+		o = tout[t];
+		if (o.status == 0 && o.n_ops > 0) ops = (unsigned long long) o.n_ops;
+	}
+	unsigned long long total;
+	const unsigned long long off = part[blockIdx.x] + finalize_block_scan(ops, s_wave, total) - ops;
+	if (!live) return;
+	ResultRec r;
+	r.score = o.score;
+	r.status = o.status;
+	r.best_x = o.best_x; r.best_y = o.best_y;
+	r.ref_position = o.ref_position; r.qstart = o.qstart; r.qend = o.qend;
+	r.n_ops = (o.status == 0) ? o.n_ops : 0;
+	r.ops_begin = off;
+	r.cells = plan[t].cells;
+	res[t] = r;
+	dst_off[t] = off;
 }
 
 __global__ void __launch_bounds__(256)
@@ -952,10 +927,13 @@
 	return hipGetLastError();
 }
 
-hipError_t launch_finalize(const TileOut *tout, const TilePlan *plan, uint64_t *dst_off, ResultRec *res,
+hipError_t launch_finalize(const TileOut *tout, const TilePlan *plan, uint64_t *dst_off, uint64_t *part, ResultRec *res,
 		BatchSummary *sum, int32_t *counters, int n_tiles, uint64_t dense_cap, hipStream_t st) {
-	hipLaunchKernelGGL(finalize_kernel, dim3(1), dim3(256), 0, st, tout, plan, dst_off, res, sum, counters,
-			n_tiles, (unsigned long long) dense_cap);
+	const int nblk = finalize_blocks(n_tiles);
+	unsigned long long *p = reinterpret_cast<unsigned long long *>(part);
+	if (nblk > 0) hipLaunchKernelGGL(finalize_sum_kernel, dim3(nblk), dim3(kFinalizeTile), 0, st, tout, p, n_tiles, nblk);
+	hipLaunchKernelGGL(finalize_scan_kernel, dim3(1), dim3(kFinalizeTile), 0, st, p, nblk, sum, counters, (unsigned long long) dense_cap);
+	if (nblk > 0) hipLaunchKernelGGL(finalize_write_kernel, dim3(nblk), dim3(kFinalizeTile), 0, st, tout, plan, p, dst_off, res, n_tiles);
 	return hipGetLastError();
 }
 
diff --git a/ngmlr_amd/csrc/cvx_launch.h b/ngmlr_amd/csrc/cvx_launch.h
--- a/ngmlr_amd/csrc/cvx_launch.h
+++ b/ngmlr_amd/csrc/cvx_launch.h
@@ -81,7 +81,9 @@
 hipError_t launch_plan(const RowDesc *rows, const RowSrc *rsrc, const TileIn *tin, TilePlan *plan, int n_tiles, uint64_t rows_per_tile,
 		unsigned long long max_matrix_mb, hipStream_t st);
 hipError_t launch_backtrack(const BacktrackArgs &a, const int32_t *order, int n_order, int group, hipStream_t st);
-hipError_t launch_finalize(const TileOut *tout, const TilePlan *plan, uint64_t *dst_off, ResultRec *res,
+static const int kFinalizeTile = 256;
+inline int finalize_blocks(int n_tiles) { return n_tiles > 0 ? (n_tiles + kFinalizeTile - 1) / kFinalizeTile : 0; }
+hipError_t launch_finalize(const TileOut *tout, const TilePlan *plan, uint64_t *dst_off, uint64_t *part, ResultRec *res,
 		BatchSummary *sum, int32_t *counters, int n_tiles, uint64_t dense_cap, hipStream_t st);
 hipError_t launch_compact(const int32_t *regions, const TileRun *trun, const TileOut *tout,
 		const uint64_t *dst_off, uint32_t *dense, int n_tiles, uint64_t dense_cap, hipStream_t st);
diff --git a/ngmlr_amd/csrc/cvx_plan_logic.h b/ngmlr_amd/csrc/cvx_plan_logic.h
--- /dev/null
+++ b/ngmlr_amd/csrc/cvx_plan_logic.h
@@ -0,0 +1,260 @@
+#ifndef CVX_PLAN_LOGIC_H
+#define CVX_PLAN_LOGIC_H
+
+#include <stdint.h>
+
+#include "cvx_types.h"
+
+#if defined(__HIPCC__)
+#define CVX_HD __host__ __device__ inline
+#else
+#define CVX_HD inline
+#endif
+
+namespace cvx {
+
+static const int kPlanStrip = 1536;
+static const int kPlanAhead = 511;
+static const int kPlanCap = 2048;
+static_assert(kPlanCap == kPlanStrip + kPlanAhead + 1 && (kPlanCap & (kPlanCap - 1)) == 0, "ring = strip + stretch behind it + the row above");
+
+struct PlanRows {
+	const RowDesc2 *rows;
+	int32_t fmt, width, off0;
+	float k, d, right;
+};
+
+CVX_HD RowDesc2 plan_row_at(const PlanRows &p, const int y) {
+	RowDesc2 r;
+	if (p.fmt == kRowsAffine || p.fmt == kRowsConst) {
+		r.x = p.fmt == kRowsConst ? p.off0 : affine_row_offset(y, p.d, p.k, p.right);
+		r.y = p.width;
+	} else {
+		r = p.rows[y];
+	}
+	return r;
+}
+CVX_HD int32_t plan_row_len(const PlanRows &p, const int y) {
+	return (p.fmt == kRowsAffine || p.fmt == kRowsConst) ? p.width : p.rows[y].y;
+}
+
+CVX_HD void plan_row_span(const RowDesc2 ol, const int W, const int y, int &gs, int &ge) {
+	long long lo = ol.x > 0 ? ol.x : 0;
+	long long hi = (long long) ol.x + (long long) ol.y;
+	if (hi > W) hi = W;
+	if (hi < lo) hi = lo;
+	gs = (int) (lo + y);
+	ge = (int) (hi + y);
+}
+
+struct PlanAcc {
+	unsigned long long cells, active;
+	int need, flags, maxlen, rendmax, r0min;
+};
+CVX_HD PlanAcc plan_acc_init() {
+	PlanAcc a;
+	a.cells = 0; a.active = 0; a.need = 1; a.flags = 0; a.maxlen = 0; a.rendmax = -0x7fffffff; a.r0min = 0x7fffffff;
+	return a;
+}
+
+template <typename Pred>
+CVX_HD int plan_first_row_at(const int y, const int gs, const int lim, const int H, Pred starts_before) {
+	int lo = y + 1, hi = H;
+	int g = y + 1 + ((lim - gs) >> 1);
+	g = g < lo ? lo : g;
+	if (g < hi) {
+		if (starts_before(g)) {
+			lo = g + 1;
+			for (int step = 1; lo < hi; step <<= 1) {
+				const int p = (lo + step - 1 < hi) ? lo + step - 1 : hi - 1;
+				if (starts_before(p)) lo = p + 1; else { hi = p; break; }
+			}
+		} else {
+			hi = g;
+			for (int step = 1; lo < hi; step <<= 1) {
+				const int p = (hi - step > lo) ? hi - step : lo;
+				if (starts_before(p)) { lo = p + 1; break; } else hi = p;
+			}
+		}
+	}
+	while (lo < hi) {
+		const int mid = (lo + hi) >> 1;
+		if (starts_before(mid)) lo = mid + 1; else hi = mid;
+	}
+	return lo;
+}
+
+CVX_HD int plan_insertion_extent(const PlanRows &p, const int W, const int H, const int y) {
+	const RowDesc2 ol = plan_row_at(p, y);
+	long long lo_y = ol.x > 0 ? ol.x : 0;
+	long long hi_y = (long long) ol.x + (long long) ol.y;
+	if (hi_y > W) hi_y = W;
+	if (hi_y < lo_y) hi_y = lo_y;
+	int a = y + 1, b = H;
+	while (a < b) {
+		const int mid = (a + b) >> 1;
+		const RowDesc2 om = plan_row_at(p, mid);
+		const long long lo_m = om.x > 0 ? om.x : 0;
+		if (lo_m < hi_y) a = mid + 1; else b = mid;
+	}
+	return a - y;
+}
+
+template <typename Pred>
+CVX_HD void plan_row_common(PlanAcc &a, const PlanRows &p, const int W, const int H, const int y, const int len,
+		const int gs, const int ge, const int pgs, const int pge, const int lim, Pred starts_before) {
+	a.cells += (unsigned long long) (long long) len;
+	a.active += (unsigned long long) (ge - gs);
+	if (len > a.maxlen) a.maxlen = len;
+	if (ge > a.rendmax) a.rendmax = ge;
+	if (gs < a.r0min) a.r0min = gs;
+	if (y > 0) {
+		if (gs <= pgs) a.flags |= kPlanIrregular;
+		if (ge < pge) a.flags |= kPlanIrregular;
+	}
+	const int n = plan_first_row_at(y, gs, lim, H, starts_before) - y + 1;
+	if (n > a.need) a.need = n;
+	if (H > 32767) {
+		const int ext = plan_insertion_extent(p, W, H, y);
+		if (ext > a.maxlen) a.maxlen = ext;
+	}
+}
+
+CVX_HD void plan_row_ondemand(PlanAcc &a, const PlanRows &p, const int W, const int H, const int y) {
+	const RowDesc2 ol = plan_row_at(p, y);
+	int gs, ge, pgs = 0, pge = 0;
+	plan_row_span(ol, W, y, gs, ge);
+	if (y > 0) plan_row_span(plan_row_at(p, y - 1), W, y - 1, pgs, pge);
+	const int lim = ge + kSwitchMargin;
+	plan_row_common(a, p, W, H, y, ol.y, gs, ge, pgs, pge, lim, [&](const int yy) {
+		int mgs, mge;
+		plan_row_span(plan_row_at(p, yy), W, yy, mgs, mge);
+		return mgs < lim;
+	});
+}
+
+CVX_HD void plan_stage_row(const PlanRows &p, const int W, const int r, int *ring_gs, int *ring_ge) {
+	int gs, ge;
+	plan_row_span(plan_row_at(p, r), W, r, gs, ge);
+	ring_gs[r & (kPlanCap - 1)] = gs;
+	ring_ge[r & (kPlanCap - 1)] = ge;
+}
+CVX_HD void plan_row_staged(PlanAcc &a, const PlanRows &p, const int W, const int H, const int y, const int staged,
+		const int *ring_gs, const int *ring_ge) {
+	const int gs = ring_gs[y & (kPlanCap - 1)], ge = ring_ge[y & (kPlanCap - 1)];
+	const int pgs = y > 0 ? ring_gs[(y - 1) & (kPlanCap - 1)] : 0, pge = y > 0 ? ring_ge[(y - 1) & (kPlanCap - 1)] : 0;
+	const int lim = ge + kSwitchMargin;
+	plan_row_common(a, p, W, H, y, plan_row_len(p, y), gs, ge, pgs, pge, lim, [&](const int yy) {
+		if (yy < staged) return ring_gs[yy & (kPlanCap - 1)] < lim;
+		int mgs, mge;
+		plan_row_span(plan_row_at(p, yy), W, yy, mgs, mge);
+		return mgs < lim;
+	});
+}
+CVX_HD int plan_strip_staged(const int Y, const int H) {
+	const long long e = (long long) Y + kPlanStrip + kPlanAhead;
+	return e < H ? (int) e : H;
+}
+
+CVX_HD TilePlan plan_finish(const PlanAcc &a, const int H, const unsigned long long max_matrix_mb) {
+	TilePlan p;
+	p.cells = a.cells;
+	p.active = a.active;
+	p.need = a.need;
+	int f = a.flags;
+	int r0 = 0, rend = 0;
+	if (H > 0) { r0 = a.r0min; rend = a.rendmax; }
+	if (H <= 0 || a.active == 0) f |= kPlanEmpty;
+	const float mb = (float) a.cells / 1000.0f / 1000.0f;
+	if (!((unsigned long long) mb < max_matrix_mb)) f |= kPlanTooLarge;
+	if (a.maxlen > 32767 || (H > 32767 && (f & kPlanIrregular))) f |= kPlanWrap16;
+	p.r0 = r0;
+	p.rend = rend;
+	p.flags = f;
+	return p;
+}
+
+#if !defined(__HIP_DEVICE_COMPILE__)
+
+inline TilePlan plan_tile_strips(const PlanRows &p, const int W, const int H, const unsigned long long max_matrix_mb) {
+	static thread_local int ring_gs[kPlanCap], ring_ge[kPlanCap];
+	PlanAcc a = plan_acc_init();
+	int staged = 0;
+	for (int Y = 0; Y < H; Y += kPlanStrip) {
+		const int end = plan_strip_staged(Y, H);
+		for (int r = staged; r < end; ++r) plan_stage_row(p, W, r, ring_gs, ring_ge);
+		staged = end;
+		const int yend = (long long) Y + kPlanStrip < H ? Y + kPlanStrip : H;
+		for (int y = Y; y < yend; ++y) plan_row_staged(a, p, W, H, y, staged, ring_gs, ring_ge);
+	}
+	return plan_finish(a, H, max_matrix_mb);
+}
+
+inline TilePlan plan_tile_ondemand(const PlanRows &p, const int W, const int H, const unsigned long long max_matrix_mb) {
+	PlanAcc a = plan_acc_init();
+	for (int y = 0; y < H; ++y) plan_row_ondemand(a, p, W, H, y);
+	return plan_finish(a, H, max_matrix_mb);
+}
+
+inline TilePlan plan_tile_brute(const PlanRows &p, const int W, const int H, const unsigned long long max_matrix_mb) {
+	PlanAcc a = plan_acc_init();
+	bool irregular = false;
+	for (int y = 1; y < H; ++y) {
+		int gs, ge, pgs, pge;
+		plan_row_span(plan_row_at(p, y), W, y, gs, ge);
+		plan_row_span(plan_row_at(p, y - 1), W, y - 1, pgs, pge);
+		if (gs <= pgs || ge < pge) irregular = true;
+	}
+	if (irregular) a.flags |= kPlanIrregular;
+	for (int y = 0; y < H; ++y) {
+		const RowDesc2 ol = plan_row_at(p, y);
+		int gs, ge;
+		plan_row_span(ol, W, y, gs, ge);
+		a.cells += (unsigned long long) (long long) ol.y;
+		a.active += (unsigned long long) (ge - gs);
+		if (ol.y > a.maxlen) a.maxlen = ol.y;
+		if (ge > a.rendmax) a.rendmax = ge;
+		if (gs < a.r0min) a.r0min = gs;
+		const int lim = ge + kSwitchMargin;
+		int first = H;
+		if (!irregular) {
+			for (int yy = y + 1; yy < H; ++yy) {
+				int mgs, mge;
+				plan_row_span(plan_row_at(p, yy), W, yy, mgs, mge);
+				if (mgs >= lim) { first = yy; break; }
+			}
+		} else {
+			first = plan_first_row_at(y, gs, lim, H, [&](const int yy) {
+				int mgs, mge;
+				plan_row_span(plan_row_at(p, yy), W, yy, mgs, mge);
+				return mgs < lim;
+			});
+		}
+		if (first - y + 1 > a.need) a.need = first - y + 1;
+		if (H > 32767) {
+			long long hi_y = (long long) ol.x + (long long) ol.y;
+			const long long lo_y = ol.x > 0 ? ol.x : 0;
+			if (hi_y > W) hi_y = W;
+			if (hi_y < lo_y) hi_y = lo_y;
+			int ext;
+			if (!irregular) {
+				int yy = y + 1;
+				while (yy < H) {
+					const RowDesc2 om = plan_row_at(p, yy);
+					if (!((om.x > 0 ? om.x : 0) < hi_y)) break;
+					++yy;
+				}
+				ext = yy - y;
+			} else {
+				ext = plan_insertion_extent(p, W, H, y);
+			}
+			if (ext > a.maxlen) a.maxlen = ext;
+		}
+	}
+	return plan_finish(a, H, max_matrix_mb);
+}
+#endif
+
+}
+
+#endif
diff --git a/ngmlr_amd/csrc/cvx_rt_align.cpp b/ngmlr_amd/csrc/cvx_rt_align.cpp
--- a/ngmlr_amd/csrc/cvx_rt_align.cpp
+++ b/ngmlr_amd/csrc/cvx_rt_align.cpp
@@ -99,7 +99,7 @@
 	RC_TRY(b->d_plan.ensure(n1));
 	RC_TRY(b->d_trun.ensure(n1));
 	RC_TRY(b->d_tout.ensure(n1));
-	RC_TRY(b->d_dstoff.ensure(n1));
+	RC_TRY(b->d_dstoff.ensure(n1 + 2 * (size_t) finalize_blocks(n)));
 	RC_TRY(b->d_lists.ensure(2 * n1));
 	if (b->d_counters.cap < 64) {
 		RC_TRY(b->d_counters.ensure(64));
@@ -378,7 +378,7 @@
 	if (!sch.per_class) RC_TRY(issue_walk(b, ba, sch.walk, sch.bt_begin, sch.n_walk, st, S_aux[0]));
 	ResultRec *d_rec = reinterpret_cast<ResultRec *>(b->d_res.p);
 	BatchSummary *d_sum = reinterpret_cast<BatchSummary *>(b->d_res.p + (size_t) n * sizeof(ResultRec));
-	HIP_TRY(launch_finalize(b->d_tout.p, b->d_plan.p, b->d_dstoff.p, d_rec, d_sum, b->d_counters.p, n, b->dense_cap, st));
+	HIP_TRY(launch_finalize(b->d_tout.p, b->d_plan.p, b->d_dstoff.p, b->d_dstoff.p + n, d_rec, d_sum, b->d_counters.p, n, b->dense_cap, st));
 	HIP_TRY(launch_compact(b->d_regions.p, b->d_trun.p, b->d_tout.p, b->d_dstoff.p, b->d_dense.p, n, b->dense_cap, st));
 	HIP_TRY(hipEventRecord(b->ev[3], st));
 	HIP_TRY(hipMemcpyAsync(b->h_res.p, b->d_res.p, (size_t) n * sizeof(ResultRec) + sizeof(BatchSummary), hipMemcpyDeviceToHost, st));
@@ -508,6 +508,26 @@
 	ABI_GUARD_BEGIN
 	if (!b || !n_ops || b->state < kFinished) { set_err("cvx_batch_ops_total: batch not run"); return CVX_ERR_ARG; }
 	*n_ops = b->ops_total;
+	return CVX_OK;
+	ABI_GUARD_END
+}
+
+int cvx_batch_summary(cvx_batch b, uint64_t *ops_total, int32_t *n_valid, int32_t *n_redone) {
+	ABI_GUARD_BEGIN
+	if (!b || !ops_total || !n_valid || !n_redone || b->state < kFinished) { set_err("cvx_batch_summary: NULL argument / batch not run"); return CVX_ERR_ARG; }
+	*ops_total = 0; *n_valid = 0; *n_redone = 0;
+	if (b->n == 0) return CVX_OK;
+	const BatchSummary *s = b->summary();
+	*ops_total = s->ops_total; *n_valid = s->n_valid; *n_redone = s->n_redone;
+	return CVX_OK;
+	ABI_GUARD_END
+}
+
+int cvx_batch_plan(cvx_batch b, int32_t first, int32_t count, cvx_tile_plan *out) {
+	ABI_GUARD_BEGIN
+	static_assert(sizeof(cvx_tile_plan) == sizeof(TilePlan), "cvx_tile_plan mirrors TilePlan");
+	if (!b || b->state < kFinished || first < 0 || count < 0 || (int64_t) first + count > b->n || (count > 0 && !out)) { set_err("cvx_batch_plan: bad range / batch not run"); return CVX_ERR_ARG; }
+	if (count) memcpy(out, b->plan() + first, (size_t) count * sizeof(TilePlan));
 	return CVX_OK;
 	ABI_GUARD_END
 }
diff --git a/ngmlr_amd/csrc/cvx_types.h b/ngmlr_amd/csrc/cvx_types.h
--- a/ngmlr_amd/csrc/cvx_types.h
+++ b/ngmlr_amd/csrc/cvx_types.h
@@ -13,8 +13,11 @@
 static const int kLateMinGroups = 128;
 static const int kLateShift = 5;
 static const int kPadRedo = 2;
-static const int kPenEntries = 64;
-static const int kPenClamp = kPenEntries - 8;
+static const int kPenClamp = 56;
+static const int kPenClampSteps = 32;
+static const int kPenEntries = 96;
+static_assert(kPenEntries >= kPenClamp + kPenClampSteps + 1, "the penalty table must cover every run reachable between two clamps");
+static_assert(kPenClamp + kPenClampSteps < 65536, "a gang's boundary record keeps the run in 16 bits");
 static const int kGangDepth = 8;
 static const int kChainChunk = 16;
 
```

Measured after the change: 16340 (median of 6 runs). 1.7% higher.
